# ECP-WarpX/WarpX

Measured on AMD Instinct MI355X. Metric: particle_steps_per_s, higher is better.
Workload: dtype f64; 1 GPU; 3D uniform_plasma 256x256x256, 8 ppc, Yee FDTD, order-3 shape, esirkepov, boris, filter on; cells_per_gpu=16777216, particles_per_gpu=134217728, n_ranks=1, ranks_per_gpu=1, sort_interval=2, single_precision_comms=False, preroll_steps=40, overlap_halo=False, momentum_synchronisation=outside the timed region (the K steps are consecutive steps of one longer run)

## Files before the change

### include/warpx_amd.h

```cpp
#ifndef WARPX_AMD_H_
#define WARPX_AMD_H_

#include <stdint.h>

#ifdef __cplusplus
extern "C" {
#endif

typedef enum wxa_status {
    WXA_OK = 0,
    WXA_ERR_INVALID_ARG = -1,
    WXA_ERR_HIP = -2,
    WXA_ERR_UNSUPPORTED = -3,
    WXA_ERR_NOMEM = -4,
    WXA_ERR_COMM = -5
} wxa_status;

enum { WXA_PUSHER_BORIS = 0, WXA_PUSHER_VAY = 1, WXA_PUSHER_HC = 2,
       WXA_PUSHER_BORIS_RR = 3 };
enum { WXA_DEPOSIT_ESIRKEPOV = 0, WXA_DEPOSIT_DIRECT = 1 };
enum { WXA_DT_FULL = 0, WXA_DT_FIRST_HALF = 1, WXA_DT_SECOND_HALF = 2 };

typedef struct wxa_field_view {
    double* p;
    int32_t lo[3];
    int32_t n[3];
    int32_t ng[3];
    int32_t stag[3];
    int64_t jstride;
    int64_t kstride;
} wxa_field_view;

typedef struct wxa_particle_view {
    double* x; double* y; double* z; double* w;
    double* ux; double* uy; double* uz;
    uint64_t* idcpu;
    int64_t np;
} wxa_particle_view;

typedef struct wxa_grid_geom {
    double xyzmin[3];
    double dinv[3];
    int32_t lo[3];
} wxa_grid_geom;

typedef struct wxa_workspace wxa_workspace;

wxa_status wxa_workspace_create(wxa_workspace** ws);
void       wxa_workspace_destroy(wxa_workspace* ws);
wxa_status wxa_workspace_set_external_particle_fields(wxa_workspace* ws, const double E[3], const double B[3]);
typedef struct wxa_repeated_plasma_lens {
    int32_t n_lenses;
    double  period;
    const double* starts;
    const double* lengths;
    const double* strengths_E;
    const double* strengths_B;
    double  gamma_boost;
    double  dt;
} wxa_repeated_plasma_lens;
wxa_status wxa_workspace_set_repeated_plasma_lens(wxa_workspace* ws, const wxa_repeated_plasma_lens* lens);
wxa_status wxa_workspace_set_time(wxa_workspace* ws, double t);
#define WXA_ACC_FP64 0
#define WXA_ACC_FP32 1
wxa_status wxa_workspace_set_deposit_accumulator(wxa_workspace* ws, int32_t accumulator);
wxa_status wxa_workspace_set_streaming_plasma(wxa_workspace* ws, int32_t on);

const char* wxa_version(void);
const char* wxa_last_error(void);


wxa_status wxa_evolve_b(const wxa_field_view E[3], const wxa_field_view B[3],
                        double dt, const double dinv[3], void* stream);

wxa_status wxa_evolve_e(const wxa_field_view E[3], const wxa_field_view B[3],
                        const wxa_field_view J[3],
                        double dt, const double dinv[3], void* stream);

wxa_status wxa_evolve_b_guard_layer(const wxa_field_view E[3], const wxa_field_view B[3], double dt,
                                    const double inv_dx[3], const int32_t grow[3], void* stream);

void wxa_ckc_stencil_coefficients(const double cell_size[3], double coefs_x[5], double coefs_y[5], double coefs_z[5]);
double wxa_ckc_max_dt(const double cell_size[3]);
wxa_status wxa_evolve_b_ckc(const wxa_field_view E[3], const wxa_field_view B[3], double dt,
                            const double coefs_x[5], const double coefs_y[5], const double coefs_z[5], void* stream);


wxa_status wxa_gather_push(const wxa_particle_view* p,
                           const wxa_field_view E[3], const wxa_field_view B[3],
                           const wxa_grid_geom* geom,
                           double q, double m, double dt,
                           int order, int galerkin, int pusher, void* stream);

wxa_status wxa_push_p(const wxa_particle_view* p,
                      const wxa_field_view E[3], const wxa_field_view B[3],
                      const wxa_grid_geom* geom,
                      double q, double m, double dt,
                      int order, int galerkin, int pusher, void* stream);

wxa_status wxa_gather_push_ws(const wxa_particle_view* p,
                              const wxa_field_view E[3], const wxa_field_view B[3],
                              const wxa_grid_geom* geom,
                              double q, double m, double dt,
                              int order, int galerkin, int pusher, int move,
                              wxa_workspace* ws, void* stream);

enum { WXA_PART_INTERIOR = 1, WXA_PART_REST = 2 };
wxa_status wxa_gather_push_part(const wxa_particle_view* p,
                                const wxa_field_view E[3], const wxa_field_view B[3],
                                const wxa_grid_geom* geom,
                                double q, double m, double dt,
                                int order, int galerkin, int pusher,
                                wxa_workspace* ws, int part, void* stream);

wxa_status wxa_deposit_current(const wxa_particle_view* p,
                               const wxa_field_view J[3],
                               const wxa_grid_geom* geom,
                               double q, double dt, double relative_time,
                               int order, int algo,
                               wxa_workspace* ws, void* stream);

wxa_status wxa_deposit_charge(const wxa_particle_view* p,
                              const wxa_field_view* rho,
                              const wxa_grid_geom* geom,
                              double q, int order, void* stream);

wxa_status wxa_enforce_periodic(const wxa_particle_view* p,
                                const double plo[3], const double phi[3],
                                const int periodic[3], void* stream);
wxa_status wxa_enforce_periodic_sorted(const wxa_particle_view* p, const double plo[3], const double phi[3],
                                       const int periodic[3], wxa_workspace* ws, int32_t steps_since_sort,
                                       void* stream);

wxa_status wxa_sort_particles_by_cell(const wxa_particle_view* src,
                                      const wxa_particle_view* dst,
                                      const double plo[3], const double dinv[3],
                                      const int32_t cell_lo[3], const int32_t ncell[3],
                                      wxa_workspace* ws, void* stream);

enum { WXA_PUSH_SORT_COUNT = 1, WXA_PUSH_SORT_SCATTER = 2 };
wxa_status wxa_push_sort_begin(wxa_workspace* ws, int32_t mode, const wxa_particle_view* p,
                               const wxa_particle_view* dst, const double plo[3], const double dinv[3],
                               const int32_t cell_lo[3], const int32_t ncell[3], const int32_t wrap[3],
                               int32_t check_retired, double predict_dt, void* stream);
wxa_status wxa_push_sort_end(wxa_workspace* ws, int32_t read_live, int64_t* live, int64_t* appended,
                             void* stream);
int32_t wxa_push_sort_pending(const wxa_workspace* ws, const wxa_particle_view* p);

wxa_status wxa_partition_particles(const wxa_particle_view* src, const wxa_particle_view* dst,
                                   int dim, double lo, double hi, int64_t counts[3],
                                   wxa_workspace* ws, void* stream);

#define WXA_IDCPU_RETIRED 0xFFFFFFFFFFFFFFFFull

wxa_status wxa_wrap_and_classify(const wxa_particle_view* p, int64_t first, int64_t count,
                                 const double prob_lo[3], const double prob_hi[3],
                                 const int periodic[3], const double brick_lo[3],
                                 const double brick_hi[3], const int split[3], int32_t* lists,
                                 int64_t capacity, int64_t counts[6], wxa_workspace* ws,
                                 void* stream);

wxa_status wxa_wrap_and_classify_dest(const wxa_particle_view* p, int64_t first, int64_t count,
                                      const double prob_lo[3], const double prob_hi[3],
                                      const int periodic[3], const double brick_lo[3],
                                      const double brick_hi[3], const int split[3], int32_t* lists,
                                      int64_t capacity, int64_t counts[27], wxa_workspace* ws,
                                      void* stream);

wxa_status wxa_pack_leavers(const wxa_particle_view* p, const int32_t* list, int64_t n, void* msg,
                            int64_t row_len, int64_t offset, int retire, const double brick_lo[3],
                            const double brick_hi[3], void* stream);

wxa_status wxa_sort_live_count(wxa_workspace* ws, int64_t* n, void* stream);


#define WXA_BOUNDARY_PERIODIC 0
#define WXA_BOUNDARY_PEC      1

wxa_status wxa_apply_pec_e(const wxa_field_view E[3], const int32_t dom_lo[3],
                           const int32_t dom_hi[3], const int32_t pec_lo[3],
                           const int32_t pec_hi[3], const int32_t ng[3], void* stream);
wxa_status wxa_apply_pec_b(const wxa_field_view B[3], const int32_t dom_lo[3],
                           const int32_t dom_hi[3], const int32_t pec_lo[3],
                           const int32_t pec_hi[3], const int32_t ng[3], void* stream);

#define WXA_PBOUNDARY_DEFAULT    0
#define WXA_PBOUNDARY_ABSORBING  1
#define WXA_PBOUNDARY_REFLECTING 2
#define WXA_PBOUNDARY_PERIODIC   3

wxa_status wxa_apply_particle_boundaries(const wxa_particle_view* p, const double prob_lo[3],
                                         const double prob_hi[3], const int32_t bc_lo[3],
                                         const int32_t bc_hi[3], int64_t* n_lost,
                                         wxa_workspace* ws, void* stream);

wxa_status wxa_apply_pec_j(const wxa_field_view J[3], const int32_t dom_lo[3],
                           const int32_t dom_hi[3], const int32_t pec_lo[3],
                           const int32_t pec_hi[3], void* stream);

wxa_status wxa_apply_pec_rho(const wxa_field_view* rho, const int32_t dom_lo[3],
                             const int32_t dom_hi[3], const int32_t pec_lo[3],
                             const int32_t pec_hi[3], void* stream);


wxa_status wxa_filter_bilinear(const wxa_field_view* src, const wxa_field_view* dst,
                               void* stream);

wxa_status wxa_filter_stencil(const wxa_field_view* src, const wxa_field_view* dst, const double* s0, int32_t n0,
                              const double* s1, int32_t n1, const double* s2, int32_t n2, void* stream);

#define WXA_NCI_EX_EY_BZ 0
#define WXA_NCI_BX_BY_EZ 1
wxa_status wxa_nci_godfrey_stencil(double cdtodz, int32_t nodal_gather, int32_t coeff_set, double stencil_z[5]);

wxa_status wxa_fill_boundary_periodic(const wxa_field_view* f, const int ng[3],
                                      const int periodic[3], void* stream);

wxa_status wxa_fill_boundary_periodic_multi(const wxa_field_view* f, int32_t nf, const int ng[3],
                                            const int periodic[3], void* stream);

wxa_status wxa_sync_nodal_periodic(const wxa_field_view* f, const int periodic[3], void* stream);

wxa_status wxa_sum_boundary_periodic(const wxa_field_view* f, const int src_ng[3],
                                     const int periodic[3], void* stream);

wxa_status wxa_sum_boundary_periodic_multi(const wxa_field_view* f, int32_t nf, const int src_ng[3],
                                           const int periodic[3], void* stream);

wxa_status wxa_pack_box(const wxa_field_view* f, const int32_t blo[3], const int32_t bhi[3],
                        double* buf, void* stream);
wxa_status wxa_unpack_box(const wxa_field_view* f, const int32_t blo[3], const int32_t bhi[3],
                          const double* buf, int mode, void* stream);
wxa_status wxa_pack_box_f32(const wxa_field_view* f, const int32_t blo[3], const int32_t bhi[3],
                            float* buf, void* stream);
wxa_status wxa_unpack_box_f32(const wxa_field_view* f, const int32_t blo[3], const int32_t bhi[3],
                              const float* buf, int mode, void* stream);

wxa_status wxa_field_set_zero(const wxa_field_view* f, void* stream);
wxa_status wxa_field_set_zero_multi(const wxa_field_view* f, int32_t nf, void* stream);

wxa_status wxa_copy_to_host(void* dst_host, const void* src_dev, int64_t bytes);
wxa_status wxa_copy_to_device(void* dst_dev, const void* src_host, int64_t bytes);
wxa_status wxa_device_synchronize(void);


enum { WXA_GRID_STAGGERED = 0, WXA_GRID_COLLOCATED = 1 };
enum { WXA_SOLVER_YEE = 0, WXA_SOLVER_CKC = 1 };

typedef struct wxa_sim_config {
    int32_t n_cell[3];
    double  prob_lo[3];
    double  prob_hi[3];
    double  cfl;
    int32_t nox;
    int32_t galerkin;
    int32_t particle_pusher;
    int32_t current_deposition;
    int32_t use_filter;
    int32_t sort_interval;
    int32_t nbricks[3];
    int32_t coord[3];
    int32_t field_boundary_lo[3];
    int32_t field_boundary_hi[3];
    int32_t particle_boundary_lo[3];
    int32_t particle_boundary_hi[3];
    int32_t overlap_halo;
    int32_t grid_type;
    int32_t maxwell_solver;
    double  gamma_boost;
    int32_t use_fdtd_nci_corr;
} wxa_sim_config;


typedef struct wxa_moving_window {
    int32_t dir;
    double  v;
} wxa_moving_window;

typedef struct wxa_plasma_injector {
    double  density;
    int32_t ppc[3];
    double  lo[3], hi[3];
    double  gamma_boost;
    double  t;
} wxa_plasma_injector;

typedef struct wxa_injected_momentum {
    double   u_mean[3];
    double   u_th[3];
    uint64_t seed;
    double   origin[3];
} wxa_injected_momentum;
wxa_status wxa_add_plasma(const wxa_particle_view* dst, const wxa_plasma_injector* inj,
                          const double corner[3], const int32_t ncells[3], const double dx[3],
                          const double brick_lo[3], const double brick_hi[3],
                          const wxa_injected_momentum* momentum,
                          int64_t* n_added, wxa_workspace* ws, void* stream);

typedef struct wxa_laser_antenna {
    double position[3], direction[3], polarization[3];
    double e_max, wavelength;
    double waist, duration, t_peak, focal_distance;
} wxa_laser_antenna;

#define WXA_WINDOW_KEEP_GUARDS 2
wxa_status wxa_shift_field_window(const wxa_field_view* f, double* tmp, int32_t dir, int32_t num_shift,
                                  const int periodic[3], void* stream);

typedef struct wxa_laser_push_params {
    double position[3], p_X[3], p_Y[3];
    double mobility;
    double e_max, wavelength, waist, duration, t_peak, focal_distance;
    double nvec[3];
    double gamma_boost;
} wxa_laser_push_params;
wxa_status wxa_laser_push(const wxa_particle_view* p, const wxa_laser_push_params* par, double t,
                          double dt, void* stream);

typedef struct wxa_comm {
    void* ctx;
    int32_t rank, nranks;
    int (*exchange)(void* ctx, int nmsg,
                    const int32_t* send_peer, void* const* send_buf, const int64_t* send_bytes,
                    const int32_t* recv_peer, void* const* recv_buf, const int64_t* recv_bytes,
                    void* stream);
    int (*exchange_counts)(void* ctx, int nmsg,
                           const int32_t* send_peer, const int64_t* send_val,
                           const int32_t* recv_peer, int64_t* recv_val);
} wxa_comm;

#define WXA_RCCL_ID_BYTES 128
#define WXA_RCCL_LOOPBACK 1
#define WXA_RCCL_TIMING   2
typedef struct wxa_rccl_stats {
    int64_t n_exchanges, n_messages, bytes_sent, n_count_exchanges, timed_exchanges;
    double timed_ms;
} wxa_rccl_stats;
wxa_status wxa_rccl_unique_id(char id[WXA_RCCL_ID_BYTES]);
wxa_status wxa_rccl_comm_set_timing(wxa_comm* comm, int32_t on);
wxa_status wxa_rccl_comm_create(const char id[WXA_RCCL_ID_BYTES], int32_t rank, int32_t nranks, int32_t flags,
                                wxa_comm* out);
void       wxa_rccl_comm_destroy(wxa_comm* comm);
wxa_status wxa_rccl_comm_stats(wxa_comm* comm, wxa_rccl_stats* out, int32_t reset);

typedef struct wxa_sim wxa_sim;

wxa_status wxa_sim_create(const wxa_sim_config* cfg, const wxa_comm* comm, wxa_sim** out);
void       wxa_sim_destroy(wxa_sim* s);
wxa_status wxa_sim_add_species(wxa_sim* s, double charge, double mass,
                               const wxa_particle_view* init, int32_t* species_id);
wxa_status wxa_sim_evolve(wxa_sim* s, int32_t numsteps);
wxa_status wxa_sim_set_synchronize_at_end(wxa_sim* s, int32_t on);
wxa_status wxa_sim_synchronize(wxa_sim* s);
wxa_status wxa_sim_set_safe_guard_cells(wxa_sim* s, int32_t on);
wxa_status wxa_sim_set_single_precision_comms(wxa_sim* s, int32_t on);
wxa_status wxa_sim_set_external_particle_fields(wxa_sim* s, int32_t id, const double E[3], const double B[3]);
wxa_status wxa_sim_set_deposit_accumulator(wxa_sim* s, int32_t id, int32_t accumulator);
wxa_status wxa_sim_set_radiation_reaction(wxa_sim* s, int32_t id, int32_t on);
wxa_status wxa_sim_create_from_inputs(const char* inputs_path, int32_t n_overrides,
                                      const char* const* overrides, const wxa_comm* comm,
                                      const int32_t* nbricks, const int32_t* coord, wxa_sim** out);
int32_t     wxa_sim_max_step(const wxa_sim* s);
int32_t     wxa_sim_num_species(const wxa_sim* s);
const char* wxa_sim_species_name(const wxa_sim* s, int32_t id);
int64_t     wxa_sim_checksum_json(wxa_sim* s, char* buf, int64_t capacity);
wxa_status  wxa_sim_write_plotfile(wxa_sim* s, const char* dir);
wxa_status  wxa_sim_add_full_diag(wxa_sim* s, const char* name, const char* intervals, const char* file_prefix,
                                  int32_t file_min_digits, const char* fields, int32_t write_species,
                                  int32_t dump_last_timestep);
wxa_status  wxa_sim_flush_diags_last_timestep(wxa_sim* s);
wxa_status  wxa_sim_btd_write_plotfile(wxa_sim* s, int32_t i, const char* dir);
wxa_status  wxa_sim_btd_set_flush(wxa_sim* s, const char* file_prefix, int32_t file_min_digits);
wxa_status  wxa_sim_btd_flush(wxa_sim* s);
wxa_status  wxa_sim_btd_box(wxa_sim* s, int32_t i, int32_t lo[3], int32_t hi[3]);
wxa_status  wxa_parser_eval(const char* expr, int32_t nvars, const char* const* names,
                            const double* values, double* out);

int32_t wxa_sim_halo_overlap(const wxa_sim* s);

wxa_status wxa_sim_compute_rho(wxa_sim* s);
double     wxa_sim_dt(const wxa_sim* s);
int64_t    wxa_sim_istep(const wxa_sim* s);
wxa_status wxa_sim_get_field(wxa_sim* s, const char* name, wxa_field_view* out);
wxa_status wxa_sim_get_particles(wxa_sim* s, int32_t species_id, wxa_particle_view* out);
wxa_status wxa_btd_select_particles(const wxa_particle_view* p, const double* const old6[6], double z_boost,
                                    double z_boost_old, double t_boost, double dt, double t_lab, double gamma_boost,
                                    double* out, int64_t capacity, int64_t* n_selected, void* stream);
wxa_status wxa_sim_add_btd(wxa_sim* s, int32_t num_snapshots, double dt_snapshots_lab, int32_t buffer_size,
                           int32_t write_species);
wxa_status wxa_sim_btd_num_particles(wxa_sim* s, int32_t i, int32_t id, int64_t* n);
wxa_status wxa_sim_btd_particles(wxa_sim* s, int32_t i, int32_t id, double* out);
wxa_status wxa_sim_btd_info(wxa_sim* s, int32_t i, int32_t n[3], double z_lab[2], double* t_lab, int32_t* slices,
                            int32_t* full);
wxa_status wxa_sim_btd_data(wxa_sim* s, int32_t i, int32_t comp, double* out);

wxa_status wxa_sim_get_timers(wxa_sim* s, double ms[8], int64_t counts[8], int reset);
wxa_status wxa_sim_dry_comm(wxa_sim* s, int32_t reps, double ms[4]);
wxa_status wxa_sim_enable_timers(wxa_sim* s, int enable);

wxa_status wxa_reduce_field(const wxa_field_view* f, const int32_t lo[3], const int32_t hi[3], double* sum_sq,
                            double* max_abs, void* stream);
wxa_status wxa_reduce_particles(const wxa_particle_view* p, double mass, int32_t photon, double out[6], void* stream);
wxa_status wxa_sim_add_reduced_diag(wxa_sim* s, const char* name, const char* type, const char* intervals,
                                    const char* path);
wxa_status wxa_sim_reduced_diag_data(wxa_sim* s, const char* name, int32_t compute_now, double* out, int32_t capacity,
                                     int32_t* n);

#ifdef __cplusplus
}
#endif
#endif
```

### warpx_amd/_capi.py

```python
from __future__ import annotations

import ctypes as C
import os

_HERE = os.path.dirname(os.path.abspath(__file__))
PRODUCT_LIB = os.path.join(_HERE, "libwarpx_amd.so")


class FieldView(C.Structure):
    _fields_ = [
        ("p", C.c_void_p),
        ("lo", C.c_int32 * 3),
        ("n", C.c_int32 * 3),
        ("ng", C.c_int32 * 3),
        ("stag", C.c_int32 * 3),
        ("jstride", C.c_int64),
        ("kstride", C.c_int64),
    ]


class ParticleView(C.Structure):
    _fields_ = [
        ("x", C.c_void_p), ("y", C.c_void_p), ("z", C.c_void_p), ("w", C.c_void_p),
        ("ux", C.c_void_p), ("uy", C.c_void_p), ("uz", C.c_void_p),
# ... 14 lines not shown
SOLVER_YEE, SOLVER_CKC = 0, 1
PART_INTERIOR, PART_REST = 1, 2


class SimConfig(C.Structure):
    _fields_ = [
        ("n_cell", C.c_int32 * 3),
        ("prob_lo", C.c_double * 3),
        ("prob_hi", C.c_double * 3),
        ("cfl", C.c_double),
        ("nox", C.c_int32),
        ("galerkin", C.c_int32),
        ("particle_pusher", C.c_int32),
        ("current_deposition", C.c_int32),
        ("use_filter", C.c_int32),
        ("sort_interval", C.c_int32),
        ("nbricks", C.c_int32 * 3),
        ("coord", C.c_int32 * 3),
        ("field_boundary_lo", C.c_int32 * 3),
        ("field_boundary_hi", C.c_int32 * 3),
        ("particle_boundary_lo", C.c_int32 * 3),
        ("particle_boundary_hi", C.c_int32 * 3),
        ("overlap_halo", C.c_int32),
        ("grid_type", C.c_int32),
        ("maxwell_solver", C.c_int32),
        ("gamma_boost", C.c_double),
        ("use_fdtd_nci_corr", C.c_int32),
    ]


class MovingWindow(C.Structure):
    _fields_ = [("dir", C.c_int32), ("v", C.c_double)]


class PlasmaInjector(C.Structure):
    _fields_ = [("density", C.c_double), ("ppc", C.c_int32 * 3), ("lo", C.c_double * 3), ("hi", C.c_double * 3),
                ("gamma_boost", C.c_double), ("t", C.c_double)]


class RepeatedPlasmaLens(C.Structure):
    _fields_ = [("n_lenses", C.c_int32), ("period", C.c_double), ("starts", C.POINTER(C.c_double)),
                ("lengths", C.POINTER(C.c_double)), ("strengths_E", C.POINTER(C.c_double)),
                ("strengths_B", C.POINTER(C.c_double)), ("gamma_boost", C.c_double), ("dt", C.c_double)]

    @classmethod
    def make(cls, period, starts, lengths, strengths_E, strengths_B, gamma_boost, dt):
        n = len(starts)
        arrays = [(C.c_double * n)(*map(float, a)) for a in (starts, lengths, strengths_E, strengths_B)]
        lens = cls(n, float(period), *[C.cast(a, C.POINTER(C.c_double)) for a in arrays], float(gamma_boost), float(dt))
        lens._keep = arrays
        return lens


class InjectedMomentum(C.Structure):
    _fields_ = [("u_mean", C.c_double * 3), ("u_th", C.c_double * 3), ("seed", C.c_uint64), ("origin", C.c_double * 3)]


class LaserAntenna(C.Structure):
    _fields_ = [("position", C.c_double * 3), ("direction", C.c_double * 3), ("polarization", C.c_double * 3),
                ("e_max", C.c_double), ("wavelength", C.c_double), ("waist", C.c_double), ("duration", C.c_double),
                ("t_peak", C.c_double), ("focal_distance", C.c_double)]


class LaserPushParams(C.Structure):
    _fields_ = [("position", C.c_double * 3), ("p_X", C.c_double * 3), ("p_Y", C.c_double * 3),
                ("mobility", C.c_double), ("e_max", C.c_double), ("wavelength", C.c_double), ("waist", C.c_double),
                ("duration", C.c_double), ("t_peak", C.c_double), ("focal_distance", C.c_double),
                ("nvec", C.c_double * 3), ("gamma_boost", C.c_double)]


EXCHANGE_FN = C.CFUNCTYPE(
    C.c_int, C.c_void_p, C.c_int,
    C.POINTER(C.c_int32), C.POINTER(C.c_void_p), C.POINTER(C.c_int64),
    C.POINTER(C.c_int32), C.POINTER(C.c_void_p), C.POINTER(C.c_int64),
    C.c_void_p)
EXCHANGE_COUNTS_FN = C.CFUNCTYPE(
    C.c_int, C.c_void_p, C.c_int,
    C.POINTER(C.c_int32), C.POINTER(C.c_int64),
    C.POINTER(C.c_int32), C.POINTER(C.c_int64))


class Comm(C.Structure):
    _fields_ = [
        ("ctx", C.c_void_p),
        ("rank", C.c_int32),
        ("nranks", C.c_int32),
        ("exchange", EXCHANGE_FN),
        ("exchange_counts", EXCHANGE_COUNTS_FN),
    ]


class RcclStats(C.Structure):
    _fields_ = [("n_exchanges", C.c_int64), ("n_messages", C.c_int64), ("bytes_sent", C.c_int64),
                ("n_count_exchanges", C.c_int64), ("timed_exchanges", C.c_int64), ("timed_ms", C.c_double)]


RCCL_LOOPBACK, RCCL_TIMING = 1, 2
PUSHER_BORIS, PUSHER_VAY, PUSHER_HC, PUSHER_BORIS_RR = 0, 1, 2, 3
DEPOSIT_ESIRKEPOV, DEPOSIT_DIRECT = 0, 1
BOUNDARY_PERIODIC, BOUNDARY_PEC = 0, 1
PBOUNDARY_DEFAULT, PBOUNDARY_ABSORBING, PBOUNDARY_REFLECTING, PBOUNDARY_PERIODIC = 0, 1, 2, 3

_FV3 = FieldView * 3
_D3 = C.c_double * 3
_I3 = C.c_int * 3
_I32_3 = C.c_int32 * 3
_PFV = C.POINTER(FieldView)
_PPV = C.POINTER(ParticleView)
_PGG = C.POINTER(GridGeom)

_KERNEL_SIGS = {
    "evolve_b": (C.c_int, [_FV3, _FV3, C.c_double, _D3, C.c_void_p]),
    "evolve_e": (C.c_int, [_FV3, _FV3, _FV3, C.c_double, _D3, C.c_void_p]),
    "gather_push": (C.c_int, [_PPV, _FV3, _FV3, _PGG, C.c_double, C.c_double, C.c_double,
                              C.c_int, C.c_int, C.c_int, C.c_void_p]),
    "push_p": (C.c_int, [_PPV, _FV3, _FV3, _PGG, C.c_double, C.c_double, C.c_double,
                         C.c_int, C.c_int, C.c_int, C.c_void_p]),
    "deposit_current": (C.c_int, [_PPV, _FV3, _PGG, C.c_double, C.c_double, C.c_double,
                                  C.c_int, C.c_int, C.c_void_p, C.c_void_p]),
    "deposit_charge": (C.c_int, [_PPV, _PFV, _PGG, C.c_double, C.c_int, C.c_void_p]),
    "btd_select_particles": (C.c_int, [_PPV, C.POINTER(C.c_void_p), C.c_double, C.c_double, C.c_double, C.c_double,
                                       C.c_double, C.c_double, C.c_void_p, C.c_int64, C.POINTER(C.c_int64), C.c_void_p]),
    "reduce_field": (C.c_int, [_PFV, _I32_3, _I32_3, C.POINTER(C.c_double), C.POINTER(C.c_double), C.c_void_p]),
    "reduce_particles": (C.c_int, [_PPV, C.c_double, C.c_int32, C.c_double * 6, C.c_void_p]),
    "enforce_periodic": (C.c_int, [_PPV, _D3, _D3, _I3, C.c_void_p]),
    "apply_pec_e": (C.c_int, [_FV3, _I32_3, _I32_3, _I32_3, _I32_3, _I32_3, C.c_void_p]),
    "apply_pec_b": (C.c_int, [_FV3, _I32_3, _I32_3, _I32_3, _I32_3, _I32_3, C.c_void_p]),
    "apply_pec_j": (C.c_int, [_FV3, _I32_3, _I32_3, _I32_3, _I32_3, C.c_void_p]),
    "apply_particle_boundaries": (C.c_int, [_PPV, _D3, _D3, _I32_3, _I32_3, C.POINTER(C.c_int64), C.c_void_p,
                                            C.c_void_p]),
    "evolve_b_guard_layer": (C.c_int, [_FV3, _FV3, C.c_double, _D3, _I32_3, C.c_void_p]),
    "evolve_b_ckc": (C.c_int, [_FV3, _FV3, C.c_double, C.c_double * 5, C.c_double * 5, C.c_double * 5, C.c_void_p]),
    "ckc_stencil_coefficients": (None, [_D3, C.c_double * 5, C.c_double * 5, C.c_double * 5]),
    "ckc_max_dt": (C.c_double, [_D3]),
    "apply_pec_rho": (C.c_int, [_PFV, _I32_3, _I32_3, _I32_3, _I32_3, C.c_void_p]),
    "shift_field_window": (C.c_int, [_PFV, C.c_void_p, C.c_int32, C.c_int32, _I3, C.c_void_p]),
    "laser_push": (C.c_int, [_PPV, C.POINTER(LaserPushParams), C.c_double, C.c_double, C.c_void_p]),
    "filter_bilinear": (C.c_int, [_PFV, _PFV, C.c_void_p]),
    "filter_stencil": (C.c_int, [_PFV, _PFV, C.POINTER(C.c_double), C.c_int32, C.POINTER(C.c_double), C.c_int32,
                                 C.POINTER(C.c_double), C.c_int32, C.c_void_p]),
    "nci_godfrey_stencil": (C.c_int, [C.c_double, C.c_int32, C.c_int32, C.POINTER(C.c_double)]),
    "fill_boundary_periodic": (C.c_int, [_PFV, _I3, _I3, C.c_void_p]),
    "sum_boundary_periodic": (C.c_int, [_PFV, _I3, _I3, C.c_void_p]),
    "sync_nodal_periodic": (C.c_int, [_PFV, _I3, C.c_void_p]),
    "field_set_zero": (C.c_int, [_PFV, C.c_void_p]),
    "version": (C.c_char_p, []),
}

_INPUTS_SIGS = {
    "sim_dry_comm": (C.c_int, [C.c_void_p, C.c_int32, C.c_double * 4]),
    "sim_create_from_inputs": (C.c_int, [C.c_char_p, C.c_int32, C.POINTER(C.c_char_p), C.POINTER(Comm),
                                        C.POINTER(C.c_int32), C.POINTER(C.c_int32), C.POINTER(C.c_void_p)]),
    "sim_max_step": (C.c_int32, [C.c_void_p]),
    "sim_num_species": (C.c_int32, [C.c_void_p]),
    "sim_species_name": (C.c_char_p, [C.c_void_p, C.c_int32]),
    "sim_checksum_json": (C.c_int64, [C.c_void_p, C.c_char_p, C.c_int64]),
    "sim_write_plotfile": (C.c_int, [C.c_void_p, C.c_char_p]),
    "sim_add_full_diag": (C.c_int, [C.c_void_p, C.c_char_p, C.c_char_p, C.c_char_p, C.c_int32, C.c_char_p, C.c_int32,
                                   C.c_int32]),
    "sim_flush_diags_last_timestep": (C.c_int, [C.c_void_p]),
    "sim_btd_write_plotfile": (C.c_int, [C.c_void_p, C.c_int32, C.c_char_p]),
    "sim_btd_set_flush": (C.c_int, [C.c_void_p, C.c_char_p, C.c_int32]),
    "sim_btd_flush": (C.c_int, [C.c_void_p]),
    "sim_btd_box": (C.c_int, [C.c_void_p, C.c_int32, C.POINTER(C.c_int32), C.POINTER(C.c_int32)]),
    "sim_set_synchronize_at_end": (C.c_int, [C.c_void_p, C.c_int32]),
    "sim_synchronize": (C.c_int, [C.c_void_p]),
    "sim_set_safe_guard_cells": (C.c_int, [C.c_void_p, C.c_int32]),
    "sim_set_single_precision_comms": (C.c_int, [C.c_void_p, C.c_int32]),
    "parser_eval": (C.c_int, [C.c_char_p, C.c_int32, C.POINTER(C.c_char_p), C.POINTER(C.c_double),
                              C.POINTER(C.c_double)]),
    "last_error": (C.c_char_p, []),
}

_SIM_SIGS = {
    "sim_create": (C.c_int, [C.POINTER(SimConfig), C.c_void_p, C.POINTER(C.c_void_p)]),
    "sim_destroy": (None, [C.c_void_p]),
    "sim_add_species": (C.c_int, [C.c_void_p, C.c_double, C.c_double, _PPV, C.POINTER(C.c_int32)]),
    "sim_evolve": (C.c_int, [C.c_void_p, C.c_int32]),
    "sim_dt": (C.c_double, [C.c_void_p]),
    "sim_istep": (C.c_int64, [C.c_void_p]),
    "sim_get_field": (C.c_int, [C.c_void_p, C.c_char_p, _PFV]),
    "sim_get_particles": (C.c_int, [C.c_void_p, C.c_int32, _PPV]),
    "sim_get_timers": (C.c_int, [C.c_void_p, C.c_double * 8, C.c_int64 * 8, C.c_int]),
    "sim_enable_timers": (C.c_int, [C.c_void_p, C.c_int]),
    "sim_compute_rho": (C.c_int, [C.c_void_p]),
    "sim_halo_overlap": (C.c_int32, [C.c_void_p]),
    "sim_set_moving_window": (C.c_int, [C.c_void_p, C.POINTER(MovingWindow)]),
    "sim_set_injection": (C.c_int, [C.c_void_p, C.c_int32, C.POINTER(PlasmaInjector), C.c_int, C.c_int]),
    "sim_set_external_particle_fields": (C.c_int, [C.c_void_p, C.c_int32, _D3, _D3]),
    "sim_set_radiation_reaction": (C.c_int, [C.c_void_p, C.c_int32, C.c_int32]),
    "sim_add_laser": (C.c_int, [C.c_void_p, C.POINTER(LaserAntenna)]),
    "sim_add_btd": (C.c_int, [C.c_void_p, C.c_int32, C.c_double, C.c_int32, C.c_int32]),
    "sim_btd_num_particles": (C.c_int, [C.c_void_p, C.c_int32, C.c_int32, C.POINTER(C.c_int64)]),
    "sim_btd_particles": (C.c_int, [C.c_void_p, C.c_int32, C.c_int32, C.POINTER(C.c_double)]),
    "sim_btd_info": (C.c_int, [C.c_void_p, C.c_int32, C.POINTER(C.c_int32), C.POINTER(C.c_double), C.POINTER(C.c_double),
                              C.POINTER(C.c_int32), C.POINTER(C.c_int32)]),
    "sim_btd_data": (C.c_int, [C.c_void_p, C.c_int32, C.c_int32, C.POINTER(C.c_double)]),
    "sim_add_reduced_diag": (C.c_int, [C.c_void_p, C.c_char_p, C.c_char_p, C.c_char_p, C.c_char_p]),
    "sim_reduced_diag_data": (C.c_int, [C.c_void_p, C.c_char_p, C.c_int32, C.POINTER(C.c_double), C.c_int32,
                                       C.POINTER(C.c_int32)]),
}

_PRODUCT_SIGS = {
    "fill_boundary_periodic_multi": (C.c_int, [_PFV, C.c_int32, _I3, _I3, C.c_void_p]),
    "sum_boundary_periodic_multi": (C.c_int, [_PFV, C.c_int32, _I3, _I3, C.c_void_p]),
    "workspace_set_external_particle_fields": (C.c_int, [C.c_void_p, _D3, _D3]),
    "workspace_set_repeated_plasma_lens": (C.c_int, [C.c_void_p, C.POINTER(RepeatedPlasmaLens)]),
    "workspace_set_time": (C.c_int, [C.c_void_p, C.c_double]),
    "workspace_create": (C.c_int, [C.POINTER(C.c_void_p)]),
    "workspace_destroy": (None, [C.c_void_p]),
    "last_error": (C.c_char_p, []),
    "sort_particles_by_cell": (C.c_int, [_PPV, _PPV, _D3, _D3, _I32_3, _I32_3, C.c_void_p, C.c_void_p]),
    "gather_push_ws": (C.c_int, [_PPV, _FV3, _FV3, _PGG, C.c_double, C.c_double, C.c_double,
                                 C.c_int, C.c_int, C.c_int, C.c_int, C.c_void_p, C.c_void_p]),
    "add_plasma": (C.c_int, [_PPV, C.POINTER(PlasmaInjector), _D3, _I32_3, _D3, _D3, _D3,
                             C.POINTER(InjectedMomentum), C.POINTER(C.c_int64), C.c_void_p, C.c_void_p]),
    "gather_push_part": (C.c_int, [_PPV, _FV3, _FV3, _PGG, C.c_double, C.c_double, C.c_double, C.c_int, C.c_int,
                                   C.c_int, C.c_void_p, C.c_int, C.c_void_p]),
    "partition_particles": (C.c_int, [_PPV, _PPV, C.c_int, C.c_double, C.c_double,
                                      C.POINTER(C.c_int64), C.c_void_p, C.c_void_p]),
    "wrap_and_classify": (C.c_int, [_PPV, C.c_int64, C.c_int64, _D3, _D3, _I3, _D3, _D3, _I3, C.c_void_p,
                                    C.c_int64, C.POINTER(C.c_int64), C.c_void_p, C.c_void_p]),
    "wrap_and_classify_dest": (C.c_int, [_PPV, C.c_int64, C.c_int64, _D3, _D3, _I3, _D3, _D3, _I3, C.c_void_p,
                                         C.c_int64, C.POINTER(C.c_int64), C.c_void_p, C.c_void_p]),
    "pack_leavers": (C.c_int, [_PPV, C.c_void_p, C.c_int64, C.c_void_p, C.c_int64, C.c_int64, C.c_int, _D3, _D3,
                               C.c_void_p]),
    "sort_live_count": (C.c_int, [C.c_void_p, C.POINTER(C.c_int64), C.c_void_p]),
    "push_sort_begin": (C.c_int, [C.c_void_p, C.c_int32, _PPV, _PPV, _D3, _D3, _I32_3, _I32_3, _I32_3, C.c_int32, C.c_double, C.c_void_p]),
    "push_sort_end": (C.c_int, [C.c_void_p, C.c_int32, C.POINTER(C.c_int64), C.POINTER(C.c_int64), C.c_void_p]),
    "push_sort_pending": (C.c_int32, [C.c_void_p, _PPV]),
    "pack_box": (C.c_int, [_PFV, _I32_3, _I32_3, C.c_void_p, C.c_void_p]),
    "unpack_box": (C.c_int, [_PFV, _I32_3, _I32_3, C.c_void_p, C.c_int, C.c_void_p]),
    "pack_box_f32": (C.c_int, [_PFV, _I32_3, _I32_3, C.c_void_p, C.c_void_p]),
    "unpack_box_f32": (C.c_int, [_PFV, _I32_3, _I32_3, C.c_void_p, C.c_int, C.c_void_p]),
    "field_set_zero_multi": (C.c_int, [_PFV, C.c_int32, C.c_void_p]),
    "copy_to_host": (C.c_int, [C.c_void_p, C.c_void_p, C.c_int64]),
    "copy_to_device": (C.c_int, [C.c_void_p, C.c_void_p, C.c_int64]),
    "device_synchronize": (C.c_int, []),
    "enforce_periodic_sorted": (C.c_int, [_PPV, _D3, _D3, _I3, C.c_void_p, C.c_int32, C.c_void_p]),
    "workspace_set_deposit_accumulator": (C.c_int, [C.c_void_p, C.c_int32]),
    "workspace_set_streaming_plasma": (C.c_int, [C.c_void_p, C.c_int32]),
    "sim_set_deposit_accumulator": (C.c_int, [C.c_void_p, C.c_int32, C.c_int32]),
}
ACC_FP64, ACC_FP32 = 0, 1
PUSH_SORT_COUNT, PUSH_SORT_SCATTER = 1, 2

_TRANSPORT_SIGS = {
    "rccl_unique_id": (C.c_int, [C.c_char * 128]),
    "rccl_comm_create": (C.c_int, [C.c_char * 128, C.c_int32, C.c_int32, C.c_int32, C.POINTER(Comm)]),
    "rccl_comm_destroy": (None, [C.POINTER(Comm)]),
    "rccl_comm_stats": (C.c_int, [C.POINTER(Comm), C.POINTER(RcclStats), C.c_int32]),
    "rccl_comm_set_timing": (C.c_int, [C.POINTER(Comm), C.c_int32]),
}

_ORACLE_SIGS = {
    "sum_sq_unique": (C.c_double, [_PFV]),
    "field_energy": (None, [_FV3, _FV3, _D3, C.c_double * 3]),
    "particle_energy": (C.c_double, [_PPV, C.c_double]),
    "particle_momentum": (None, [_PPV, C.c_double, C.c_double * 3]),
    "cell_centered_abs_sum": (C.c_double, [_PFV]),
    "abs_sum": (C.c_double, [C.c_void_p, C.c_int64, C.c_double]),

    "pack_box_f32": (C.c_int, [_PFV, _I32_3, _I32_3, C.c_void_p, C.c_void_p]),
    "unpack_box_f32": (C.c_int, [_PFV, _I32_3, _I32_3, C.c_void_p, C.c_int, C.c_void_p]),
    "num_threads": (C.c_int, []),
    "set_num_threads": (C.c_int, [C.c_int]),
    "add_plasma": (C.c_int, [_PPV, C.POINTER(PlasmaInjector), _D3, _I32_3, _D3, _D3, _D3,
                             C.POINTER(InjectedMomentum), C.POINTER(C.c_int64), C.c_void_p, C.c_void_p]),
    "sort_particles_by_cell": (C.c_int, [_PPV, _PPV, _D3, _D3, _I32_3, _I32_3, C.c_void_p, C.c_void_p]),
    "wrap_and_classify": (C.c_int, [_PPV, C.c_int64, C.c_int64, _D3, _D3, _I3, _D3, _D3, _I3, C.c_void_p,
                                    C.c_int64, C.POINTER(C.c_int64), C.c_void_p, C.c_void_p]),
    "wrap_and_classify_dest": (C.c_int, [_PPV, C.c_int64, C.c_int64, _D3, _D3, _I3, _D3, _D3, _I3, C.c_void_p,
                                         C.c_int64, C.POINTER(C.c_int64), C.c_void_p, C.c_void_p]),
    "pack_leavers": (C.c_int, [_PPV, C.c_void_p, C.c_int64, C.c_void_p, C.c_int64, C.c_int64, C.c_int, _D3, _D3,
                               C.c_void_p]),
}


class WxaError(RuntimeError):
    pass


_RETURNS_A_VALUE = {"sim_max_step", "sim_num_species", "num_threads", "set_num_threads", "sim_halo_overlap", "push_sort_pending"}


class CLib:

    def __init__(self, path: str, prefix: str, extra_sigs: dict | None = None, kernels: bool = True,
                 memory: str | None = None):
        self.memory = memory or ("cuda" if prefix == "wxa_" else "cpu")
        if not os.path.exists(path):
            raise WxaError(
                f"{path} not found: build it first (python -c 'import __graft_entry__ as g; g.build()')")
        self.path = path
        self.prefix = prefix
        self._dll = C.CDLL(path, mode=C.RTLD_GLOBAL if prefix == "wxa_" else C.RTLD_LOCAL)
        sigs = dict(_KERNEL_SIGS) if kernels else {}
        sigs.update(_SIM_SIGS)
        if extra_sigs:
            sigs.update(extra_sigs)
        self.names = []
        for name, (res, args) in sigs.items():
            fn = getattr(self._dll, prefix + name)
            fn.restype = res
            fn.argtypes = args
            setattr(self, "_" + name, fn)
            self.names.append(prefix + name)

    def __getattr__(self, name):
        raw = object.__getattribute__(self, "_" + name)
        if raw.restype is C.c_int and name not in _RETURNS_A_VALUE:
            def checked(*a):
                rc = raw(*a)
                if rc != 0:
                    msg = ""
                    if hasattr(self, "_last_error"):
                        try:
                            msg = (self._last_error() or b"").decode()
                        except Exception:
                            pass
                    raise WxaError(f"{self.prefix}{name} failed with status {rc} {msg}")
                return rc
            return checked
        return raw


_product = None


def load_product() -> CLib:
    global _product
    if _product is None:
        _product = CLib(os.environ.get("WXA_PRODUCT_LIB", PRODUCT_LIB), "wxa_",
                       {**_PRODUCT_SIGS, **_INPUTS_SIGS, **_TRANSPORT_SIGS})
    return _product


def declared_symbols(header_path: str) -> list[str]:
    import re
    text = open(header_path).read()
    text = re.sub(r"/\*.*?\*/", "", text, flags=re.S)
    return sorted(set(re.findall(r"\b(wxa_[a-z0-9_]+)\s*\(", text)))
```

### warpx_amd/csrc/fields.hip

```cpp
#include "common.hpp"

#include <algorithm>
#include <climits>
#include <cstdlib>

namespace wxa {

template <int TW_, int TJ_, int KC_, int NT_, int BATCH_ = 0>
struct StencilCfg {
    static constexpr int TW = TW_, TI = 64 * TW_, TJ = TJ_, KC = KC_, NT = NT_, BATCH = BATCH_;
};

struct TileGrid {
    int nti, ntj, ntk;
    long ntiles;
};

template <class CFG>
static TileGrid make_tiles_cfg(const Box3& ub) {
    TileGrid t;
    t.nti = (ub.hi[0] - ub.lo[0] + CFG::TI - 1) / CFG::TI;
    t.ntj = (ub.hi[1] - ub.lo[1] + CFG::TJ - 1) / CFG::TJ;
    t.ntk = (ub.hi[2] - ub.lo[2] + CFG::KC - 1) / CFG::KC;
    t.ntiles = (long)t.nti * t.ntj * t.ntk;
    return t;
}

__device__ inline bool in_ij(const Box3& b, int i, int j) {
    return i >= b.lo[0] && i < b.hi[0] && j >= b.lo[1] && j < b.hi[1];
}

template <int NT>
__device__ __forceinline__ double ld_shared(const double* p) {
    if constexpr (NT >= 2) return __builtin_nontemporal_load(p);
    else return *p;
}
template <int NT>
__device__ __forceinline__ double ld_once(const double* p) {
    if constexpr (NT) return __builtin_nontemporal_load(p);
    else return *p;
}
template <int NT>
__device__ __forceinline__ void st_once(double* p, double v) {
    if constexpr (NT) __builtin_nontemporal_store(v, p);
    else *p = v;
}

template <class CFG>
__global__ void __launch_bounds__(CFG::TI* CFG::TJ)
evolve_b_kernel(DevF Ex, DevF Ey, DevF Ez, DevF Bx, DevF By, DevF Bz, Box3 ub, Box3 bbx, Box3 bby,
                Box3 bbz, TileGrid tg, double dt, double idx, double idy, double idz) {
    constexpr int KC = CFG::KC, NT = CFG::NT;
    const long tile = xcd_tile_id(blockIdx.x, tg.ntiles);
    if (tile >= tg.ntiles) return;
    const int ti = (int)(tile % tg.nti);
    const int tj = (int)((tile / tg.nti) % tg.ntj);
    const int tk = (int)(tile / ((long)tg.nti * tg.ntj));
    const int i = ub.lo[0] + ti * CFG::TI + (int)threadIdx.x;
    const int j = ub.lo[1] + tj * CFG::TJ + (int)threadIdx.y;
    if (i >= ub.hi[0] || j >= ub.hi[1]) return;
    const int k0 = ub.lo[2] + tk * KC;
    const int k1 = min(k0 + KC, ub.hi[2]);
    const bool px = in_ij(bbx, i, j), py = in_ij(bby, i, j), pz = in_ij(bbz, i, j);

    const double* __restrict__ ex = Ex.p + Ex.off(i, j, k0);
    const double* __restrict__ ey = Ey.p + Ey.off(i, j, k0);
    const double* __restrict__ ez = Ez.p + Ez.off(i, j, k0);
    double* __restrict__ bx = Bx.p + Bx.off(i, j, k0);
    double* __restrict__ by = By.p + By.off(i, j, k0);
    double* __restrict__ bz = Bz.p + Bz.off(i, j, k0);

    if constexpr (CFG::BATCH != 0) {
        double exv[KC + 1], eyv[KC + 1], ezc[KC], ezj[KC], ezi[KC], exj[KC], eyi[KC], b0[KC], b1[KC], b2[KC];
        bool d0[KC], d1[KC], d2[KC];
        exv[0] = ld_shared<NT>(ex); eyv[0] = ld_shared<NT>(ey);
#pragma unroll
        for (int n = 0; n < KC; ++n) {
            const int k = k0 + n;
            const bool in = k < k1;
            d0[n] = in && px && k >= bbx.lo[2] && k < bbx.hi[2];
            d1[n] = in && py && k >= bby.lo[2] && k < bby.hi[2];
            d2[n] = in && pz && k >= bbz.lo[2] && k < bbz.hi[2];
            exv[n + 1] = eyv[n + 1] = ezc[n] = ezj[n] = ezi[n] = exj[n] = eyi[n] = b0[n] = b1[n] = b2[n] = 0.0;
            if (in) {
                exv[n + 1] = ld_shared<NT>(ex + (n + 1) * Ex.ks); eyv[n + 1] = ld_shared<NT>(ey + (n + 1) * Ey.ks);
                ezc[n] = ld_shared<NT>(ez + n * Ez.ks); ezj[n] = ld_shared<NT>(ez + n * Ez.ks + Ez.js);
                ezi[n] = ld_shared<NT>(ez + n * Ez.ks + 1);
                exj[n] = ld_shared<NT>(ex + n * Ex.ks + Ex.js); eyi[n] = ld_shared<NT>(ey + n * Ey.ks + 1);
            }
            if (d0[n]) b0[n] = ld_once<NT>(bx + n * Bx.ks);
            if (d1[n]) b1[n] = ld_once<NT>(by + n * By.ks);
            if (d2[n]) b2[n] = ld_once<NT>(bz + n * Bz.ks);
        }
        asm volatile("" : "+v"(exv[0]), "+v"(eyv[0]));
#pragma unroll
        for (int n = 0; n < KC; ++n)
            asm volatile("" : "+v"(exv[n + 1]), "+v"(eyv[n + 1]), "+v"(ezc[n]), "+v"(ezj[n]), "+v"(ezi[n]), "+v"(exj[n]),
                              "+v"(eyi[n]), "+v"(b0[n]), "+v"(b1[n]), "+v"(b2[n]));
#pragma unroll
        for (int n = 0; n < KC; ++n) {
            if (d0[n]) st_once<NT>(bx + n * Bx.ks, b0[n] + (dt * (idz * (eyv[n + 1] - eyv[n])) - dt * (idy * (ezj[n] - ezc[n]))));
            if (d1[n]) st_once<NT>(by + n * By.ks, b1[n] + (dt * (idx * (ezi[n] - ezc[n])) - dt * (idz * (exv[n + 1] - exv[n]))));
            if (d2[n]) st_once<NT>(bz + n * Bz.ks, b2[n] + (dt * (idy * (exj[n] - exv[n])) - dt * (idx * (eyi[n] - eyv[n]))));
        }
        return;
    }
    double ex_k = ld_shared<NT>(ex), ey_k = ld_shared<NT>(ey);
#pragma unroll 4
    for (int k = k0; k < k1; ++k) {
        const double ex_k1 = ld_shared<NT>(ex + Ex.ks), ey_k1 = ld_shared<NT>(ey + Ey.ks);
        const double ez_c = ld_shared<NT>(ez), ez_j1 = ld_shared<NT>(ez + Ez.js), ez_i1 = ld_shared<NT>(ez + 1);
        const double ex_j1 = ld_shared<NT>(ex + Ex.js), ey_i1 = ld_shared<NT>(ey + 1);
        if (px && k >= bbx.lo[2] && k < bbx.hi[2])
            st_once<NT>(bx, ld_once<NT>(bx) + (dt * (idz * (ey_k1 - ey_k)) - dt * (idy * (ez_j1 - ez_c))));
        if (py && k >= bby.lo[2] && k < bby.hi[2])
            st_once<NT>(by, ld_once<NT>(by) + (dt * (idx * (ez_i1 - ez_c)) - dt * (idz * (ex_k1 - ex_k))));
        if (pz && k >= bbz.lo[2] && k < bbz.hi[2])
            st_once<NT>(bz, ld_once<NT>(bz) + (dt * (idy * (ex_j1 - ex_k)) - dt * (idx * (ey_i1 - ey_k))));
        ex_k = ex_k1; ey_k = ey_k1;
        ex += Ex.ks; ey += Ey.ks; ez += Ez.ks; bx += Bx.ks; by += By.ks; bz += Bz.ks;
    }
}

template <class CFG>
__global__ void __launch_bounds__(CFG::TI* CFG::TJ)
evolve_e_kernel(DevF Ex, DevF Ey, DevF Ez, DevF Bx, DevF By, DevF Bz, DevF Jx, DevF Jy, DevF Jz,
                Box3 ub, Box3 bex, Box3 bey, Box3 bez, TileGrid tg, double dt, double idx, double idy,
                double idz) {
    constexpr int KC = CFG::KC, NT = CFG::NT;
    const long tile = xcd_tile_id(blockIdx.x, tg.ntiles);
    if (tile >= tg.ntiles) return;
    const int ti = (int)(tile % tg.nti);
    const int tj = (int)((tile / tg.nti) % tg.ntj);
    const int tk = (int)(tile / ((long)tg.nti * tg.ntj));
    const int i = ub.lo[0] + ti * CFG::TI + (int)threadIdx.x;
    const int j = ub.lo[1] + tj * CFG::TJ + (int)threadIdx.y;
    if (i >= ub.hi[0] || j >= ub.hi[1]) return;
    const int k0 = ub.lo[2] + tk * KC;
    const int k1 = min(k0 + KC, ub.hi[2]);
    const bool px = in_ij(bex, i, j), py = in_ij(bey, i, j), pz = in_ij(bez, i, j);
    constexpr double c2 = PhysConst::c * PhysConst::c;
    constexpr double mu0 = PhysConst::mu0;

    double* __restrict__ ex = Ex.p + Ex.off(i, j, k0);
    double* __restrict__ ey = Ey.p + Ey.off(i, j, k0);
    double* __restrict__ ez = Ez.p + Ez.off(i, j, k0);
    const double* __restrict__ bx = Bx.p + Bx.off(i, j, k0);
    const double* __restrict__ by = By.p + By.off(i, j, k0);
    const double* __restrict__ bz = Bz.p + Bz.off(i, j, k0);
    const double* __restrict__ jx = Jx.p + Jx.off(i, j, k0);
    const double* __restrict__ jy = Jy.p + Jy.off(i, j, k0);
    const double* __restrict__ jz = Jz.p + Jz.off(i, j, k0);

    if constexpr (CFG::BATCH != 0) {
        double bxv[KC + 1], byv[KC + 1], bzc[KC], bzj[KC], bzi[KC], bxj[KC], byi[KC], e0[KC], e1[KC], e2[KC], j0[KC], j1[KC], j2[KC];
        bool d0[KC], d1[KC], d2[KC];
        bxv[0] = ld_shared<NT>(bx - Bx.ks); byv[0] = ld_shared<NT>(by - By.ks);
#pragma unroll
        for (int n = 0; n < KC; ++n) {
            const int k = k0 + n;
            const bool in = k < k1;
            d0[n] = in && px && k >= bex.lo[2] && k < bex.hi[2];
            d1[n] = in && py && k >= bey.lo[2] && k < bey.hi[2];
            d2[n] = in && pz && k >= bez.lo[2] && k < bez.hi[2];
            bxv[n + 1] = byv[n + 1] = bzc[n] = bzj[n] = bzi[n] = bxj[n] = byi[n] = 0.0;
            e0[n] = e1[n] = e2[n] = j0[n] = j1[n] = j2[n] = 0.0;
            if (in) {
                bxv[n + 1] = ld_shared<NT>(bx + n * Bx.ks); byv[n + 1] = ld_shared<NT>(by + n * By.ks);
                bzc[n] = ld_shared<NT>(bz + n * Bz.ks);
                bzj[n] = ld_shared<NT>(bz + n * Bz.ks - Bz.js); bzi[n] = ld_shared<NT>(bz + n * Bz.ks - 1);
                bxj[n] = ld_shared<NT>(bx + n * Bx.ks - Bx.js); byi[n] = ld_shared<NT>(by + n * By.ks - 1);
            }
            if (d0[n]) { e0[n] = ld_once<NT>(ex + n * Ex.ks); j0[n] = ld_once<NT>(jx + n * Jx.ks); }
            if (d1[n]) { e1[n] = ld_once<NT>(ey + n * Ey.ks); j1[n] = ld_once<NT>(jy + n * Jy.ks); }
            if (d2[n]) { e2[n] = ld_once<NT>(ez + n * Ez.ks); j2[n] = ld_once<NT>(jz + n * Jz.ks); }
        }
        asm volatile("" : "+v"(bxv[0]), "+v"(byv[0]));
#pragma unroll
        for (int n = 0; n < KC; ++n)
            asm volatile("" : "+v"(bxv[n + 1]), "+v"(byv[n + 1]), "+v"(bzc[n]), "+v"(bzj[n]), "+v"(bzi[n]), "+v"(bxj[n]),
                              "+v"(byi[n]), "+v"(e0[n]), "+v"(e1[n]), "+v"(e2[n]), "+v"(j0[n]), "+v"(j1[n]), "+v"(j2[n]));
#pragma unroll
        for (int n = 0; n < KC; ++n) {
            if (d0[n]) st_once<NT>(ex + n * Ex.ks, e0[n] + c2 * dt * (-(idz * (byv[n + 1] - byv[n])) + (idy * (bzc[n] - bzj[n])) - mu0 * j0[n]));
            if (d1[n]) st_once<NT>(ey + n * Ey.ks, e1[n] + c2 * dt * (-(idx * (bzc[n] - bzi[n])) + (idz * (bxv[n + 1] - bxv[n])) - mu0 * j1[n]));
            if (d2[n]) st_once<NT>(ez + n * Ez.ks, e2[n] + c2 * dt * (-(idy * (bxv[n + 1] - bxj[n])) + (idx * (byv[n + 1] - byi[n])) - mu0 * j2[n]));
        }
        return;
    }
    double bx_km = ld_shared<NT>(bx - Bx.ks), by_km = ld_shared<NT>(by - By.ks);
#pragma unroll 4
    for (int k = k0; k < k1; ++k) {
        const double bx_c = ld_shared<NT>(bx), by_c = ld_shared<NT>(by), bz_c = ld_shared<NT>(bz);
        const double bz_jm = ld_shared<NT>(bz - Bz.js), bz_im = ld_shared<NT>(bz - 1);
        const double bx_jm = ld_shared<NT>(bx - Bx.js), by_im = ld_shared<NT>(by - 1);
        if (px && k >= bex.lo[2] && k < bex.hi[2])
            st_once<NT>(ex, ld_once<NT>(ex) + c2 * dt * (-(idz * (by_c - by_km)) + (idy * (bz_c - bz_jm)) - mu0 * ld_once<NT>(jx)));
        if (py && k >= bey.lo[2] && k < bey.hi[2])
            st_once<NT>(ey, ld_once<NT>(ey) + c2 * dt * (-(idx * (bz_c - bz_im)) + (idz * (bx_c - bx_km)) - mu0 * ld_once<NT>(jy)));
        if (pz && k >= bez.lo[2] && k < bez.hi[2])
            st_once<NT>(ez, ld_once<NT>(ez) + c2 * dt * (-(idy * (bx_c - bx_jm)) + (idx * (by_c - by_im)) - mu0 * ld_once<NT>(jz)));
        bx_km = bx_c; by_km = by_c;
        ex += Ex.ks; ey += Ey.ks; ez += Ez.ks; bx += Bx.ks; by += By.ks; bz += Bz.ks;
        jx += Jx.ks; jy += Jy.ks; jz += Jz.ks;
    }
}

using StProduction = StencilCfg<1, 1, 3, 1, 1>;

struct FaceBoxes {
    int n;
    Box3 b[12];
    int comp[12];
    long first[13];
};
__global__ void __launch_bounds__(256)
evolve_b_faces_kernel(DevF Ex, DevF Ey, DevF Ez, DevF Bx, DevF By, DevF Bz, FaceBoxes fb, double dt, double idx, double idy,
                      double idz) {
    long t = (long)blockIdx.x * 256 + threadIdx.x;
    if (t >= fb.first[fb.n]) return;
    int f = 0;
    while (t >= fb.first[f + 1]) ++f;
    t -= fb.first[f];
    const Box3 b = fb.b[f];
    const int n0 = b.hi[0] - b.lo[0], n1 = b.hi[1] - b.lo[1];
    const int i = b.lo[0] + (int)(t % n0), j = b.lo[1] + (int)((t / n0) % n1), k = b.lo[2] + (int)(t / ((long)n0 * n1));
    const int c = fb.comp[f];
    if (c == 0) {
        const double* ey = Ey.p + Ey.off(i, j, k);
        const double* ez = Ez.p + Ez.off(i, j, k);
        double* bx = Bx.p + Bx.off(i, j, k);
        *bx = *bx + (dt * (idz * (ey[Ey.ks] - ey[0])) - dt * (idy * (ez[Ez.js] - ez[0])));
    } else if (c == 1) {
        const double* ex = Ex.p + Ex.off(i, j, k);
        const double* ez = Ez.p + Ez.off(i, j, k);
        double* by = By.p + By.off(i, j, k);
        *by = *by + (dt * (idx * (ez[1] - ez[0])) - dt * (idz * (ex[Ex.ks] - ex[0])));
    } else {
        const double* ex = Ex.p + Ex.off(i, j, k);
        const double* ey = Ey.p + Ey.off(i, j, k);
        double* bz = Bz.p + Bz.off(i, j, k);
        *bz = *bz + (dt * (idy * (ex[Ex.js] - ex[0])) - dt * (idx * (ey[1] - ey[0])));
    }
}

struct BoxN {
    int lo[3];
    int n[3];
};

__global__ void __launch_bounds__(256)
shift_copy_kernel(DevF f, BoxN box, int s0, int s1, int s2) {
    const long total = (long)box.n[0] * box.n[1] * box.n[2];
    for (long t = (long)blockIdx.x * blockDim.x + threadIdx.x; t < total; t += (long)gridDim.x * blockDim.x) {
        const int a = (int)(t % box.n[0]);
        const int b = (int)((t / box.n[0]) % box.n[1]);
        const int c = (int)(t / ((long)box.n[0] * box.n[1]));
        const int i = box.lo[0] + a, j = box.lo[1] + b, k = box.lo[2] + c;
        f.p[f.off(i, j, k)] = f.p[f.off(i + s0, j + s1, k + s2)];
    }
}

struct PecGeom {
    int dom_lo[3], dom_hi[3];
    int pec_lo[3], pec_hi[3];
    int nodal[3];
};

template <bool IS_E>
__global__ void __launch_bounds__(256)
apply_pec_kernel(DevF f, int icomp, BoxN box, PecGeom pg) {
    const long total = (long)box.n[0] * box.n[1] * box.n[2];
    for (long t = (long)blockIdx.x * blockDim.x + threadIdx.x; t < total; t += (long)gridDim.x * blockDim.x) {
        int ijk[3];
        ijk[0] = box.lo[0] + (int)(t % box.n[0]);
        ijk[1] = box.lo[1] + (int)((t / box.n[0]) % box.n[1]);
        ijk[2] = box.lo[2] + (int)(t / ((long)box.n[0] * box.n[1]));
        int mirror[3] = {ijk[0], ijk[1], ijk[2]};
        bool on_face = false, guard = false;
        double sign = 1.0;
#pragma unroll
        for (int idim = 0; idim < 3; ++idim) {
#pragma unroll
            for (int iside = 0; iside < 2; ++iside) {
                if (!(iside == 0 ? pg.pec_lo[idim] : pg.pec_hi[idim])) continue;
                const bool flagged = IS_E ? (icomp != idim) : (icomp == idim);
                const int ig = iside == 0 ? pg.dom_lo[idim] - ijk[idim]
                                          : ijk[idim] - (pg.dom_hi[idim] + pg.nodal[idim]);
                if (ig == 0) {
                    if (flagged && pg.nodal[idim] == 1) on_face = true;
                } else if (ig > 0) {
                    mirror[idim] = iside == 0 ? pg.dom_lo[idim] + ig - (1 - pg.nodal[idim]) : pg.dom_hi[idim] + 1 - ig;
                    guard = true;
                    if (flagged) sign = -sign;
                }
            }
        }
        if (on_face) f(ijk[0], ijk[1], ijk[2]) = 0.0;
        else if (guard) f(ijk[0], ijk[1], ijk[2]) = sign * f(mirror[0], mirror[1], mirror[2]);
    }
}

__global__ void __launch_bounds__(256)
apply_pec_j_kernel(DevF f, int icomp, Box3 vb, PecGeom pg) {
    const int n0 = vb.hi[0] - vb.lo[0], n1 = vb.hi[1] - vb.lo[1], n2 = vb.hi[2] - vb.lo[2];
    const long total = (long)n0 * n1 * n2;
    for (long t = (long)blockIdx.x * blockDim.x + threadIdx.x; t < total; t += (long)gridDim.x * blockDim.x) {
        int ijk[3];
        ijk[0] = vb.lo[0] + (int)(t % n0);
        ijk[1] = vb.lo[1] + (int)((t / n0) % n1);
        ijk[2] = vb.lo[2] + (int)(t / ((long)n0 * n1));
        const int flo[3] = {f.lo0, f.lo1, f.lo2}, fn[3] = {f.n0, f.n1, f.n2};
        int mir[3][2];
        bool any = false;
#pragma unroll
        for (int d = 0; d < 3; ++d) {
#pragma unroll
            for (int s = 0; s < 2; ++s) {
                mir[d][s] = INT_MIN;
                if (!(s == 0 ? pg.pec_lo[d] : pg.pec_hi[d])) continue;
                const int fac = (s == 0 ? 2 * pg.dom_lo[d] : 2 * (pg.dom_hi[d] + 1)) - (1 - pg.nodal[d]);
                const int m = fac - ijk[d];
                if (m == ijk[d] || (m >= flo[d] && m < flo[d] + fn[d])) { mir[d][s] = m; any = true; }
            }
        }
        if (!any) continue;
        double v = f(ijk[0], ijk[1], ijk[2]);
#pragma unroll
        for (int d = 0; d < 3; ++d) {
#pragma unroll
            for (int s = 0; s < 2; ++s) {
                const int m = mir[d][s];
                if (m == INT_MIN) continue;
                if (m == ijk[d]) { v = 0.0; continue; }
                int q[3] = {ijk[0], ijk[1], ijk[2]};
                q[d] = m;
                v += (icomp != d ? -1.0 : 1.0) * f(q[0], q[1], q[2]);
            }
        }
        f(ijk[0], ijk[1], ijk[2]) = v;
#pragma unroll
        for (int d = 0; d < 3; ++d) {
#pragma unroll
            for (int s = 0; s < 2; ++s) {
                const int m = mir[d][s];
                if (m == INT_MIN || m == ijk[d]) continue;
                int q[3] = {ijk[0], ijk[1], ijk[2]};
                q[d] = m;
                f(q[0], q[1], q[2]) = icomp != d ? -v : v;
            }
        }
    }
}

__global__ void __launch_bounds__(256)
set_box_kernel(DevF f, BoxN box, double value) {
    const long total = (long)box.n[0] * box.n[1] * box.n[2];
    for (long t = (long)blockIdx.x * blockDim.x + threadIdx.x; t < total; t += (long)gridDim.x * blockDim.x) {
        const int i = box.lo[0] + (int)(t % box.n[0]);
        const int j = box.lo[1] + (int)((t / box.n[0]) % box.n[1]);
        const int k = box.lo[2] + (int)(t / ((long)box.n[0] * box.n[1]));
        f.p[f.off(i, j, k)] = value;
    }
}

__global__ void __launch_bounds__(256)
shifted_copy_kernel(DevF dst, DevF src, BoxN box, int s0, int s1, int s2) {
    const long total = (long)box.n[0] * box.n[1] * box.n[2];
    for (long t = (long)blockIdx.x * blockDim.x + threadIdx.x; t < total; t += (long)gridDim.x * blockDim.x) {
        const int i = box.lo[0] + (int)(t % box.n[0]);
        const int j = box.lo[1] + (int)((t / box.n[0]) % box.n[1]);
        const int k = box.lo[2] + (int)(t / ((long)box.n[0] * box.n[1]));
        dst.p[dst.off(i, j, k)] = src.p[src.off(i + s0, j + s1, k + s2)];
    }
}

__global__ void __launch_bounds__(256)
shift_copy_sides_kernel(DevF f, BoxN box_lo, BoxN box_hi, int s0, int s1, int s2) {
    const long half = (long)box_lo.n[0] * box_lo.n[1] * box_lo.n[2];
    for (long t = (long)blockIdx.x * blockDim.x + threadIdx.x; t < 2 * half; t += (long)gridDim.x * blockDim.x) {
        const bool hi = t >= half;
        const long u = hi ? t - half : t;
        const BoxN& box = hi ? box_hi : box_lo;
        const int sg = hi ? -1 : 1;
        const int a = (int)(u % box.n[0]);
        const int b = (int)((u / box.n[0]) % box.n[1]);
        const int c = (int)(u / ((long)box.n[0] * box.n[1]));
        const int i = box.lo[0] + a, j = box.lo[1] + b, k = box.lo[2] + c;
        f.p[f.off(i, j, k)] = f.p[f.off(i + sg * s0, j + sg * s1, k + sg * s2)];
    }
}

__global__ void __launch_bounds__(256)
sum_periodic_kernel(DevF f, int d, int nc, int s0, int s1) {
    const int lo[3] = {f.lo0, f.lo1, f.lo2};
// ... 269 lines not shown
using CkcProduction = CkcCfg<4, 16, 2>;
using FilterCfg = CkcCfg<8, 16, 1>;

struct FilterStencils {
    static constexpr int MAXLEN = 8;
    double s[3][MAXLEN];
    int n[3];
};
__global__ void __launch_bounds__(256)
filter_stencil_kernel(DevF src, DevF dst, FilterStencils fs) {
    const long total = (long)src.n0 * src.n1 * src.n2;
    for (long t = (long)blockIdx.x * blockDim.x + threadIdx.x; t < total; t += (long)gridDim.x * blockDim.x) {
        const int i = src.lo0 + (int)(t % src.n0);
        const int j = src.lo1 + (int)((t / src.n0) % src.n1);
        const int k = src.lo2 + (int)(t / ((long)src.n0 * src.n1));
        auto zp = [&](int ii, int jj, int kk) -> double {
            return (ii >= src.lo0 && ii < src.lo0 + src.n0 && jj >= src.lo1 && jj < src.lo1 + src.n1 && kk >= src.lo2 &&
                    kk < src.lo2 + src.n2) ? src.p[src.off(ii, jj, kk)] : 0.0;
        };
        double d = 0.0;
        for (int i2 = 0; i2 < fs.n[2]; ++i2)
            for (int i1 = 0; i1 < fs.n[1]; ++i1)
                for (int i0 = 0; i0 < fs.n[0]; ++i0) {
                    const double sss = fs.s[0][i0] * fs.s[1][i1] * fs.s[2][i2];
                    d += sss * (zp(i - i0, j - i1, k - i2) + zp(i + i0, j - i1, k - i2) + zp(i - i0, j + i1, k - i2) +
                                zp(i + i0, j + i1, k - i2) + zp(i - i0, j - i1, k + i2) + zp(i + i0, j - i1, k + i2) +
                                zp(i - i0, j + i1, k + i2) + zp(i + i0, j + i1, k + i2));
                }
        dst.p[dst.off(i, j, k)] = d;
    }
}

template <int N2, int KC>
__global__ void __launch_bounds__(256)
filter_stencil_z_kernel(DevF src, DevF dst, FilterStencils fs) {
    const long columns = (long)src.n0 * src.n1;
    const int nseg = (src.n2 + KC - 1) / KC;
    const long t = (long)blockIdx.x * blockDim.x + threadIdx.x;
    if (t >= columns * nseg) return;
    const int i = src.lo0 + (int)(t % src.n0);
    const int j = src.lo1 + (int)((t / src.n0) % src.n1);
    const int k0 = src.lo2 + (int)(t / columns) * KC, k1 = min(k0 + KC, src.lo2 + src.n2);
    auto zp = [&](int kk) -> double { return (kk >= src.lo2 && kk < src.lo2 + src.n2) ? src.p[src.off(i, j, kk)] : 0.0; };
    double w[2 * N2 - 1];
#pragma unroll
    for (int m = 0; m < 2 * N2 - 1; ++m) w[m] = zp(k0 - (N2 - 1) + m);
    double sss[N2];
#pragma unroll
    for (int i2 = 0; i2 < N2; ++i2) sss[i2] = fs.s[0][0] * fs.s[1][0] * fs.s[2][i2];
    for (int k = k0; k < k1; ++k) {
        const double next = zp(k + N2);
        double d = 0.0;
#pragma unroll
        for (int i2 = 0; i2 < N2; ++i2) {
            const double a = w[N2 - 1 - i2], b = w[N2 - 1 + i2];
            d += sss[i2] * (a + a + a + a + b + b + b + b);
        }
        dst.p[dst.off(i, j, k)] = d;
#pragma unroll
        for (int m = 0; m + 1 < 2 * N2 - 1; ++m) w[m] = w[m + 1];
        w[2 * N2 - 2] = next;
    }
}

template <class CFG>
__global__ void __launch_bounds__(CFG::NT)
filter_bilinear_kernel(DevF src, DevF dst, TileGrid tg) {
    constexpr int PLANE = CFG::PLANE;
    __shared__ double ring[4 * PLANE];
    const long tile = xcd_tile_id(blockIdx.x, tg.ntiles);
    if (tile >= tg.ntiles) return;
    const int ti = (int)(tile % tg.nti), tj = (int)((tile / tg.nti) % tg.ntj), tk = (int)(tile / ((long)tg.nti * tg.ntj));
    const int i0 = src.lo0 + ti * CFG::TI, j0 = src.lo1 + tj * CFG::TJ, k0 = src.lo2 + tk * CFG::KC;
    const int hi0 = src.lo0 + src.n0, hi1 = src.lo1 + src.n1, hi2 = src.lo2 + src.n2;
    const int k1 = min(k0 + CFG::KC, hi2);
    const int tid = (int)(threadIdx.y * CFG::TI + threadIdx.x);
    const int i = i0 + (int)threadIdx.x, j = j0 + (int)threadIdx.y;
    double r[CFG::PER];
    for (int k = k0 - 1; k <= k0 + 1; ++k) {
        ckc_fetch_plane<CFG>(r, src, i0, j0, k, tid);
        ckc_put_plane<CFG>(ring + (k & 3) * PLANE, r, tid);
    }
    const CkcRing<CFG> in{ring, i0, j0};
    const bool active = i < hi0 && j < hi1;
    for (int k = k0; k < k1; ++k) {
        __syncthreads();
        const bool more = k + 2 <= k1;
        if (more) ckc_fetch_plane<CFG>(r, src, i0, j0, k + 2, tid);
        if (active) {
            auto tap = [&](int di, int dj, int dk) -> double { return in(i + di, j + dj, k + dk); };
            double d = 0.0;
#pragma unroll
            for (int i2 = 0; i2 < 2; ++i2)
#pragma unroll
                for (int i1 = 0; i1 < 2; ++i1)
#pragma unroll
                    for (int i0_ = 0; i0_ < 2; ++i0_) {
                        const double sss = 0.25 * 0.25 * 0.25;
                        d += sss * (tap(-i0_, -i1, -i2) + tap(+i0_, -i1, -i2) + tap(-i0_, +i1, -i2) +
                                    tap(+i0_, +i1, -i2) + tap(-i0_, -i1, +i2) + tap(+i0_, -i1, +i2) +
                                    tap(-i0_, +i1, +i2) + tap(+i0_, +i1, +i2));
                    }
            dst.p[dst.off(i, j, k)] = d;
        }
        if (more) ckc_put_plane<CFG>(ring + ((k + 2) & 3) * PLANE, r, tid);
    }
}

static inline int grid_for(long total, int block = 256, int cap = 256 * 16) {
    long g = (total + block - 1) / block;
    if (g < 1) g = 1;
    if (g > cap) g = cap;
    return (int)g;
}

static bool box_inside(const wxa_field_view& v, const int32_t blo[3], const int32_t bhi[3]) {
    for (int d = 0; d < 3; ++d)
        if (blo[d] < v.lo[d] || bhi[d] > v.lo[d] + v.n[d] || bhi[d] < blo[d]) return false;
    return true;
}

}

using namespace wxa;

extern "C" {

wxa_status wxa_evolve_b(const wxa_field_view E[3], const wxa_field_view B[3], double dt,
                        const double dinv[3], void* stream) {
    WXA_REQUIRE(E && B && dinv, "null argument");
    for (int c = 0; c < 3; ++c) WXA_REQUIRE(view_ok(E[c]) && view_ok(B[c]), "bad field view");
    if (!yee_E(E) || !yee_B(B)) {
        set_last_error("wxa_evolve_b: only the Yee staggering is supported");
        return WXA_ERR_UNSUPPORTED;
    }
    for (int c = 0; c < 3; ++c)
        for (int d = 0; d < 3; ++d) WXA_REQUIRE(E[c].ng[d] >= 1, "EvolveB needs >= 1 guard point on E");
    const Box3 bx = valid_box(B[0]), by = valid_box(B[1]), bz = valid_box(B[2]);
    Box3 ub;
    for (int d = 0; d < 3; ++d) {
        ub.lo[d] = std::min(bx.lo[d], std::min(by.lo[d], bz.lo[d]));
        ub.hi[d] = std::max(bx.hi[d], std::max(by.hi[d], bz.hi[d]));
    }
    using CFG = StProduction;
    const TileGrid tg = make_tiles_cfg<CFG>(ub);
    if (tg.ntiles > 0)
        hipLaunchKernelGGL((evolve_b_kernel<CFG>), dim3((unsigned)xcd_grid_size(tg.ntiles)), dim3(CFG::TI, CFG::TJ), 0,
                           (hipStream_t)stream, make_devf(E[0]), make_devf(E[1]), make_devf(E[2]), make_devf(B[0]),
                           make_devf(B[1]), make_devf(B[2]), ub, bx, by, bz, tg, dt, dinv[0], dinv[1], dinv[2]);
    WXA_LAUNCH_CHECK();
    return WXA_OK;
}

wxa_status wxa_evolve_b_guard_layer(const wxa_field_view E[3], const wxa_field_view B[3], double dt,
                                    const double dinv[3], const int32_t grow[3], void* stream) {
    WXA_REQUIRE(E && B && dinv && grow, "null argument");
    for (int c = 0; c < 3; ++c) WXA_REQUIRE(view_ok(E[c]) && view_ok(B[c]), "bad field view");
    if (!yee_E(E) || !yee_B(B)) {
        set_last_error("wxa_evolve_b_guard_layer: only the Yee staggering is supported");
        return WXA_ERR_UNSUPPORTED;
    }
    for (int c = 0; c < 3; ++c)
        for (int d = 0; d < 3; ++d)
            WXA_REQUIRE(!grow[d] || (E[c].ng[d] >= 2 && B[c].ng[d] >= 1), "guard layer update needs 2 guard points on E, 1 on B");
    FaceBoxes fb;
    fb.n = 0;
    fb.first[0] = 0;
    for (int d = 0; d < 3; ++d) {
        if (!grow[d]) continue;
        for (int side = 0; side < 2; ++side)
            for (int c = 0; c < 3; ++c) {
                if (B[c].stag[d]) continue;
                Box3 b = valid_box(B[c]);
                const int layer = side == 0 ? b.lo[d] - 1 : b.hi[d];
                b.lo[d] = layer; b.hi[d] = layer + 1;
                const long pts = (long)(b.hi[0] - b.lo[0]) * (b.hi[1] - b.lo[1]) * (b.hi[2] - b.lo[2]);
                if (pts <= 0) continue;
                fb.b[fb.n] = b; fb.comp[fb.n] = c;
                fb.first[fb.n + 1] = fb.first[fb.n] + pts;
                ++fb.n;
            }
    }
    if (fb.n > 0 && fb.first[fb.n] > 0)
        hipLaunchKernelGGL(evolve_b_faces_kernel, dim3((unsigned)((fb.first[fb.n] + 255) / 256)), dim3(256), 0, (hipStream_t)stream,
                           make_devf(E[0]), make_devf(E[1]), make_devf(E[2]), make_devf(B[0]), make_devf(B[1]), make_devf(B[2]),
                           fb, dt, dinv[0], dinv[1], dinv[2]);
    WXA_LAUNCH_CHECK();
    return WXA_OK;
}

void wxa_ckc_stencil_coefficients(const double cell_size[3], double cx[5], double cy[5], double cz[5]) {
    const double inv_dx = 1. / cell_size[0], inv_dy = 1. / cell_size[1], inv_dz = 1. / cell_size[2];
    const double delta = std::max({inv_dx, inv_dy, inv_dz});
    const double rx = (inv_dx / delta) * (inv_dx / delta);
    const double ry = (inv_dy / delta) * (inv_dy / delta);
    const double rz = (inv_dz / delta) * (inv_dz / delta);
    const double beta = 0.125 * (1. - rx * ry * rz / (ry * rz + rz * rx + rx * ry));
    const double betaxy = ry * beta * inv_dx, betaxz = rz * beta * inv_dx;
    const double betayx = rx * beta * inv_dy, betayz = rz * beta * inv_dy;
    const double betazx = rx * beta * inv_dz, betazy = ry * beta * inv_dz;
    const double inv_r_fac = (1. / (ry * rz + rz * rx + rx * ry));
    const double gammax = ry * rz * (0.0625 - 0.125 * ry * rz * inv_r_fac);
    const double gammay = rx * rz * (0.0625 - 0.125 * rx * rz * inv_r_fac);
    const double gammaz = rx * ry * (0.0625 - 0.125 * rx * ry * inv_r_fac);
    const double alphax = (1. - 2. * ry * beta - 2. * rz * beta - 4. * gammax) * inv_dx;
    const double alphay = (1. - 2. * rx * beta - 2. * rz * beta - 4. * gammay) * inv_dy;
    const double alphaz = (1. - 2. * rx * beta - 2. * ry * beta - 4. * gammaz) * inv_dz;
    cx[0] = inv_dx; cx[1] = alphax; cx[2] = betaxy; cx[3] = betaxz; cx[4] = gammax * inv_dx;
    cy[0] = inv_dy; cy[1] = alphay; cy[2] = betayz; cy[3] = betayx; cy[4] = gammay * inv_dy;
    cz[0] = inv_dz; cz[1] = alphaz; cz[2] = betazx; cz[3] = betazy; cz[4] = gammaz * inv_dz;
}

double wxa_ckc_max_dt(const double cell_size[3]) {
    return std::min(cell_size[0], std::min(cell_size[1], cell_size[2])) / PhysConst::c;
}

wxa_status wxa_evolve_b_ckc(const wxa_field_view E[3], const wxa_field_view B[3], double dt, const double cx[5],
                            const double cy[5], const double cz[5], void* stream) {
    WXA_REQUIRE(E && B && cx && cy && cz, "null argument");
    for (int c = 0; c < 3; ++c) WXA_REQUIRE(view_ok(E[c]) && view_ok(B[c]), "bad field view");
    if (!yee_E(E) || !yee_B(B)) {
        set_last_error("wxa_evolve_b_ckc: only the Yee staggering is supported");
        return WXA_ERR_UNSUPPORTED;
    }
    for (int c = 0; c < 3; ++c)
        for (int d = 0; d < 3; ++d) WXA_REQUIRE(E[c].ng[d] >= 1, "the CKC update of B needs >= 1 guard point on E");
    const Box3 bx = valid_box(B[0]), by = valid_box(B[1]), bz = valid_box(B[2]);
    Box3 ub;
    for (int d = 0; d < 3; ++d) {
        ub.lo[d] = std::min(bx.lo[d], std::min(by.lo[d], bz.lo[d]));
        ub.hi[d] = std::max(bx.hi[d], std::max(by.hi[d], bz.hi[d]));
        if (ub.hi[d] <= ub.lo[d]) return WXA_OK;
    }
    CkcCoefs cc;
    for (int n = 0; n < 5; ++n) { cc.x[n] = cx[n]; cc.y[n] = cy[n]; cc.z[n] = cz[n]; }
    using CFG = CkcProduction;
    const TileGrid tg = make_tiles_cfg<StencilCfg<1, CFG::TJ, CFG::KC, 1>>(ub);
    hipLaunchKernelGGL(evolve_b_ckc_tiled_kernel<CFG>, dim3((unsigned)xcd_grid_size(tg.ntiles)), dim3(CFG::TI, CFG::TJ), 0,
                       (hipStream_t)stream, make_devf(E[0]), make_devf(E[1]), make_devf(E[2]), make_devf(B[0]), make_devf(B[1]),
                       make_devf(B[2]), ub, bx, by, bz, tg, dt, cc);
    WXA_LAUNCH_CHECK();
    return WXA_OK;
}

wxa_status wxa_evolve_e(const wxa_field_view E[3], const wxa_field_view B[3], const wxa_field_view J[3],
                        double dt, const double dinv[3], void* stream) {
    WXA_REQUIRE(E && B && J && dinv, "null argument");
    for (int c = 0; c < 3; ++c) WXA_REQUIRE(view_ok(E[c]) && view_ok(B[c]) && view_ok(J[c]), "bad field view");
    if (!yee_E(E) || !yee_B(B) || !yee_E(J)) {
        set_last_error("wxa_evolve_e: only the Yee staggering is supported");
        return WXA_ERR_UNSUPPORTED;
    }
    for (int c = 0; c < 3; ++c)
        for (int d = 0; d < 3; ++d) WXA_REQUIRE(B[c].ng[d] >= 1, "EvolveE needs >= 1 guard point on B");
    const Box3 bx = valid_box(E[0]), by = valid_box(E[1]), bz = valid_box(E[2]);
    for (int c = 0; c < 3; ++c) {
        const Box3 bj = valid_box(J[c]);
        const Box3 be = valid_box(E[c]);
        for (int d = 0; d < 3; ++d)
            WXA_REQUIRE(bj.lo[d] == be.lo[d] && bj.hi[d] == be.hi[d], "J and E valid boxes differ");
    }
    Box3 ub;
    for (int d = 0; d < 3; ++d) {
        ub.lo[d] = std::min(bx.lo[d], std::min(by.lo[d], bz.lo[d]));
        ub.hi[d] = std::max(bx.hi[d], std::max(by.hi[d], bz.hi[d]));
    }
    using CFG = StProduction;
    const TileGrid tg = make_tiles_cfg<CFG>(ub);
    if (tg.ntiles > 0)
        hipLaunchKernelGGL((evolve_e_kernel<CFG>), dim3((unsigned)xcd_grid_size(tg.ntiles)), dim3(CFG::TI, CFG::TJ), 0,
                           (hipStream_t)stream, make_devf(E[0]), make_devf(E[1]), make_devf(E[2]), make_devf(B[0]),
                           make_devf(B[1]), make_devf(B[2]), make_devf(J[0]), make_devf(J[1]), make_devf(J[2]), ub, bx, by, bz,
                           tg, dt, dinv[0], dinv[1], dinv[2]);
    WXA_LAUNCH_CHECK();
    return WXA_OK;
}

wxa_status wxa_filter_bilinear(const wxa_field_view* src, const wxa_field_view* dst, void* stream) {
    WXA_REQUIRE(src && dst && view_ok(*src) && view_ok(*dst), "bad field view");
    WXA_REQUIRE(src->p != dst->p, "src and dst must not alias");
    for (int d = 0; d < 3; ++d)
        WXA_REQUIRE(src->lo[d] == dst->lo[d] && src->n[d] == dst->n[d], "src/dst boxes differ");
    TileGrid tg;
    tg.nti = (src->n[0] + FilterCfg::TI - 1) / FilterCfg::TI;
    tg.ntj = (src->n[1] + FilterCfg::TJ - 1) / FilterCfg::TJ;
    tg.ntk = (src->n[2] + FilterCfg::KC - 1) / FilterCfg::KC;
    tg.ntiles = (long)tg.nti * tg.ntj * tg.ntk;
    hipLaunchKernelGGL(filter_bilinear_kernel<FilterCfg>, dim3((unsigned)xcd_grid_size(tg.ntiles)),
                       dim3(FilterCfg::TI, FilterCfg::TJ), 0, (hipStream_t)stream, make_devf(*src), make_devf(*dst), tg);
    WXA_LAUNCH_CHECK();
    return WXA_OK;
}

wxa_status wxa_filter_stencil(const wxa_field_view* src, const wxa_field_view* dst, const double* s0, int32_t n0,
                              const double* s1, int32_t n1, const double* s2, int32_t n2, void* stream) {
    WXA_REQUIRE(src && dst && view_ok(*src) && view_ok(*dst) && s0 && s1 && s2, "bad argument");
    WXA_REQUIRE(src->p != dst->p, "src and dst must not alias");
    WXA_REQUIRE(n0 >= 1 && n0 <= FilterStencils::MAXLEN && n1 >= 1 && n1 <= FilterStencils::MAXLEN && n2 >= 1 &&
                n2 <= FilterStencils::MAXLEN, "stencil length");
    for (int d = 0; d < 3; ++d)
        WXA_REQUIRE(src->lo[d] == dst->lo[d] && src->n[d] == dst->n[d], "src/dst boxes differ");
    FilterStencils fs;
    fs.n[0] = n0; fs.n[1] = n1; fs.n[2] = n2;
    for (int a = 0; a < FilterStencils::MAXLEN; ++a) {
        fs.s[0][a] = a < n0 ? s0[a] : 0.0; fs.s[1][a] = a < n1 ? s1[a] : 0.0; fs.s[2][a] = a < n2 ? s2[a] : 0.0;
    }
    const long total = (long)src->n[0] * src->n[1] * src->n[2];
    if (total == 0) return WXA_OK;
    if (n0 == 1 && n1 == 1 && n2 == 5) {
        constexpr int KC = 32;
        const long lanes = (long)src->n[0] * src->n[1] * ((src->n[2] + KC - 1) / KC);
        hipLaunchKernelGGL((filter_stencil_z_kernel<5, KC>), dim3((unsigned)((lanes + 255) / 256)), dim3(256), 0,
                           (hipStream_t)stream, make_devf(*src), make_devf(*dst), fs);
        WXA_LAUNCH_CHECK();
        return WXA_OK;
    }
    hipLaunchKernelGGL(filter_stencil_kernel, dim3(grid_for(total)), dim3(256), 0, (hipStream_t)stream, make_devf(*src),
                       make_devf(*dst), fs);
    WXA_LAUNCH_CHECK();
    return WXA_OK;
}

wxa_status wxa_fill_boundary_periodic(const wxa_field_view* f, const int ng[3], const int periodic[3],
                                      void* stream) {
    WXA_REQUIRE(f && view_ok(*f) && ng && periodic, "bad argument");
    const DevF df = make_devf(*f);
    int lo[3], hi[3];
    for (int d = 0; d < 3; ++d) {
        WXA_REQUIRE(ng[d] <= f->ng[d], "ng exceeds allocated guards");
        lo[d] = f->lo[d] + f->ng[d];
        hi[d] = f->lo[d] + f->n[d] - f->ng[d];
    }
    for (int d = 0; d < 3; ++d) {
        if (!periodic[d] || ng[d] <= 0) continue;
        const int nc = f->n[d] - 2 * f->ng[d] - f->stag[d];
        WXA_REQUIRE(ng[d] <= nc, "guard depth exceeds the period");
        const int v0 = f->lo[d] + f->ng[d], v1 = f->lo[d] + f->n[d] - f->ng[d];
        BoxN blo, bhi;
        for (int e = 0; e < 3; ++e) { blo.lo[e] = bhi.lo[e] = lo[e]; blo.n[e] = bhi.n[e] = hi[e] - lo[e]; }
// ... 353 lines not shown
```

### warpx_amd/csrc/host/WarpX.hpp

```cpp
#ifndef WXA_HOST_WARPX_HPP_
#define WXA_HOST_WARPX_HPP_

#include <chrono>
#include <functional>

#include "BTDiagnostics.hpp"
#include "NCIGodfreyFilter.hpp"
#include "ReducedDiags.hpp"
#include "WarpXParticleContainer.hpp"

namespace wxa::host {

struct guardCellManager {
    amrex::IntVect ng_alloc_EB, ng_alloc_J, ng_depos_J, ng_FieldSolver, ng_FieldGather, ng_UpdateAux;

    void Init(const amrex::Real dt, const std::array<amrex::Real, 3>& dx, const int nox, const bool use_filter,
              const amrex::IntVect& bilinear_filter_stencil_length, const bool do_fdtd_nci_corr = false,
              const int nci_corr_stencil = 0, const bool safe_guard_cells = false) {
        constexpr double c = 299'792'458.;
        for (int d = 0; d < 3; ++d) {
            const int ng_tmp = nox;
            ng_alloc_EB[d] = (ng_tmp % 2) ? ng_tmp + 1 : ng_tmp;
            if (d == 2 && do_fdtd_nci_corr) {
                const int ng = ng_tmp + nci_corr_stencil;
                ng_alloc_EB[d] = (ng % 2) ? ng + 1 : ng;
            }
            int ngJ = ng_tmp;
            ngJ += static_cast<int>(std::ceil(c * 0.5 * dt / dx[d]));
            ng_depos_J[d] = ngJ;
            ng_alloc_J[d] = ngJ + (use_filter ? bilinear_filter_stencil_length[d] - 1 : 0);
            ng_FieldSolver[d] = 1;
            ng_FieldGather[d] = (nox + 1) / 2;
            ng_UpdateAux[d] = 0;
        }
        {
            const amrex::IntVect no_nci(std::min(ng_FieldGather[0], nox % 2 ? nox + 1 : nox),
                                        std::min(ng_FieldGather[1], nox % 2 ? nox + 1 : nox),
                                        std::min(ng_FieldGather[2], nox % 2 ? nox + 1 : nox));
            ng_FieldGather = no_nci;
            if (do_fdtd_nci_corr) ng_FieldGather[2] += nci_corr_stencil;
        }
        ng_FieldGather = amrex::min(ng_FieldGather, ng_alloc_EB);
        for (int d = 0; d < 3; ++d) ng_FieldGather[d] = std::max(ng_FieldGather[d], ng_FieldSolver[d]);
        if (safe_guard_cells) {
            ng_FieldSolver = ng_alloc_EB;
            ng_FieldGather = ng_alloc_EB;
            ng_UpdateAux = ng_alloc_EB;
        }
    }
};

class FiniteDifferenceSolver {
public:
    FiniteDifferenceSolver(WarpXContext* ctx, int fdtd_algo, const std::array<amrex::Real, 3>& cell_size)
        : m_ctx(ctx), m_fdtd_algo(fdtd_algo) {
        for (int d = 0; d < 3; ++d) m_stencil_coefs[d] = 1.0 / cell_size[d];
        if (m_fdtd_algo == WXA_SOLVER_CKC) {
            if (!ctx->be->evolve_b_ckc) throw std::runtime_error("algo.maxwell_solver = ckc: not in this backend");
            ctx->be->ckc_stencil_coefficients(cell_size.data(), m_ckc_x.data(), m_ckc_y.data(), m_ckc_z.data());
        } else if (m_fdtd_algo != WXA_SOLVER_YEE) {
            throw std::runtime_error("algo.maxwell_solver: yee or ckc");
        }
    }
    void EvolveB(ablastr::fields::MultiFabRegister& fields, int lev, PatchType patch_type, amrex::Real dt) {
        using warpx::fields::FieldType;
        if (patch_type != PatchType::fine) throw std::runtime_error("single level: fine patch only");
        auto E = fields.get_alldirs(FieldType::Efield_fp, lev);
        auto B = fields.get_alldirs(FieldType::Bfield_fp, lev);
        const wxa_field_view Ev[3] = {E[0]->view(), E[1]->view(), E[2]->view()};
        const wxa_field_view Bv[3] = {B[0]->view(), B[1]->view(), B[2]->view()};
        if (m_fdtd_algo == WXA_SOLVER_CKC)
            check(m_ctx->be->evolve_b_ckc(Ev, Bv, dt, m_ckc_x.data(), m_ckc_y.data(), m_ckc_z.data(), m_ctx->stream),
                  "evolve_b_ckc");
        else
            check(m_ctx->be->evolve_b(Ev, Bv, dt, m_stencil_coefs.data(), m_ctx->stream), "evolve_b");
    }
    void EvolveE(ablastr::fields::MultiFabRegister& fields, int lev, PatchType patch_type,
                 const ablastr::fields::VectorField& Efield, amrex::Real dt) {
        using warpx::fields::FieldType;
        if (patch_type != PatchType::fine) throw std::runtime_error("single level: fine patch only");
        auto B = fields.get_alldirs(FieldType::Bfield_fp, lev);
        auto J = fields.get_alldirs(FieldType::current_fp, lev);
        const wxa_field_view Ev[3] = {Efield[0]->view(), Efield[1]->view(), Efield[2]->view()};
        const wxa_field_view Bv[3] = {B[0]->view(), B[1]->view(), B[2]->view()};
        const wxa_field_view Jv[3] = {J[0]->view(), J[1]->view(), J[2]->view()};
        check(m_ctx->be->evolve_e(Ev, Bv, Jv, dt, m_stencil_coefs.data(), m_ctx->stream), "evolve_e");
    }
    void EvolveBGuardLayer(ablastr::fields::MultiFabRegister& fields, int lev, amrex::Real dt, const int32_t grow[3]) {
        using warpx::fields::FieldType;
        auto E = fields.get_alldirs(FieldType::Efield_fp, lev);
        auto B = fields.get_alldirs(FieldType::Bfield_fp, lev);
        const wxa_field_view Ev[3] = {E[0]->view(), E[1]->view(), E[2]->view()};
        const wxa_field_view Bv[3] = {B[0]->view(), B[1]->view(), B[2]->view()};
        check(m_ctx->be->evolve_b_guard_layer(Ev, Bv, dt, m_stencil_coefs.data(), grow, m_ctx->stream), "evolve_b_guard_layer");
    }

private:
    WarpXContext* m_ctx;
    int m_fdtd_algo = WXA_SOLVER_YEE;
    std::array<amrex::Real, 3> m_stencil_coefs{};
    std::array<amrex::Real, 5> m_ckc_x{}, m_ckc_y{}, m_ckc_z{};
};

class WarpX {
public:
    static constexpr bool sync_nodal_points = true;

    WarpX(const Backend* be, const wxa_sim_config& cfg, const wxa_comm* comm)
        : m_be(be), m_cfg(cfg), m_fields(be), mypc(std::make_unique<MultiParticleContainer>(&m_ctx)) {
        using warpx::fields::FieldType;
        using ablastr::fields::Direction;
        if (cfg.nox < 1 || cfg.nox > 4) throw std::runtime_error("algo.particle_shape must be 1..4");
        m_env_no_guard_layer = std::getenv("WXA_NO_GUARD_LAYER") != nullptr;
        if (const char* e = std::getenv("WXA_PEC_RHO_FOLD_GUARD_COLUMNS")) m_env_fold_rho_guard_columns = std::atoi(e) != 0;
        m_ctx.be = be;
        m_ctx.nox = cfg.nox;
        m_ctx.galerkin_interpolation = cfg.galerkin != 0;
        m_ctx.particle_pusher_algo = (ParticlePusherAlgo)cfg.particle_pusher;
        m_ctx.current_deposition_algo = (CurrentDepositionAlgo)cfg.current_deposition;
        if (cfg.gamma_boost > 1.0) {
            m_ctx.gamma_boost = cfg.gamma_boost;
            m_ctx.beta_boost = std::sqrt(1.0 - 1.0 / std::pow(cfg.gamma_boost, 2.0));
        }
        amrex::IntVect blo, bhi;
        for (int d = 0; d < 3; ++d) {
            if (cfg.nbricks[d] < 1 || cfg.coord[d] < 0 || cfg.coord[d] >= cfg.nbricks[d])
                throw std::runtime_error("bad brick decomposition");
            if (cfg.n_cell[d] % cfg.nbricks[d] != 0) throw std::runtime_error("n_cell must divide evenly into bricks");
            m_ctx.prob_lo[d] = cfg.prob_lo[d];
            m_ctx.prob_hi[d] = cfg.prob_hi[d];
            m_ctx.dx[d] = (cfg.prob_hi[d] - cfg.prob_lo[d]) / cfg.n_cell[d];
            m_ctx.dinv[d] = 1.0 / m_ctx.dx[d];
            const int nb = cfg.n_cell[d] / cfg.nbricks[d];
            blo[d] = cfg.coord[d] * nb;
            bhi[d] = blo[d] + nb - 1;
            m_ctx.brick_plo[d] = cfg.prob_lo[d] + blo[d] * m_ctx.dx[d];
            m_ctx.brick_phi[d] = (cfg.coord[d] == cfg.nbricks[d] - 1) ? cfg.prob_hi[d]
                                                                       : cfg.prob_lo[d] + (bhi[d] + 1) * m_ctx.dx[d];
        }
        m_ctx.brick_box = amrex::Box(blo, bhi);
        if (cfg.grid_type != WXA_GRID_STAGGERED)
            throw std::runtime_error("warpx.grid_type: only the staggered (Yee) grid is on this path");
        ComputeDt();
        use_filter = cfg.use_filter != 0;
        guard_cells.Init(dt[0], m_ctx.dx, cfg.nox, use_filter, amrex::IntVect(2), cfg.use_fdtd_nci_corr != 0,
                         NCIGodfreyFilter::m_stencil_width);
        m_ctx.ng_alloc_EB = guard_cells.ng_alloc_EB;
        m_ctx.ng_depos_J = guard_cells.ng_depos_J;
        for (int d = 0; d < 3; ++d)
            if (m_ctx.brick_box.length(d) < guard_cells.ng_alloc_J[d] + 1)
                throw std::runtime_error("brick thinner than the guard depth");
        m_comm = std::make_unique<BrickComm>(be, comm, cfg.nbricks, cfg.coord);
        int periodic[3];
        for (int d = 0; d < 3; ++d) {
            const int lo = cfg.field_boundary_lo[d], hi = cfg.field_boundary_hi[d];
            const bool ok = (lo == WXA_BOUNDARY_PERIODIC || lo == WXA_BOUNDARY_PEC) &&
                            (hi == WXA_BOUNDARY_PERIODIC || hi == WXA_BOUNDARY_PEC) &&
                            ((lo == WXA_BOUNDARY_PERIODIC) == (hi == WXA_BOUNDARY_PERIODIC));
            if (!ok) throw std::runtime_error("field boundary: a direction is periodic on both sides or on neither");
            periodic[d] = lo == WXA_BOUNDARY_PERIODIC;
            m_pec_lo[d] = lo == WXA_BOUNDARY_PEC && cfg.coord[d] == 0;
            m_pec_hi[d] = hi == WXA_BOUNDARY_PEC && cfg.coord[d] == cfg.nbricks[d] - 1;
            m_any_pec = m_any_pec || lo == WXA_BOUNDARY_PEC || hi == WXA_BOUNDARY_PEC;
            m_pec_here = m_pec_here || m_pec_lo[d] || m_pec_hi[d];
            m_dom_lo[d] = 0;
            m_dom_hi[d] = cfg.n_cell[d] - 1;
        }
        m_comm->set_periodic(periodic);
        SetUpHaloOverlap(cfg.overlap_halo != 0);
        for (int d = 0; d < 3; ++d)
            for (int side = 0; side < 2; ++side) {
                int32_t want = side == 0 ? cfg.particle_boundary_lo[d] : cfg.particle_boundary_hi[d];
                const bool fper = periodic[d] != 0;
                if (want == WXA_PBOUNDARY_DEFAULT) want = fper ? WXA_PBOUNDARY_PERIODIC : WXA_PBOUNDARY_ABSORBING;
                const bool ok = (want == WXA_PBOUNDARY_PERIODIC) == fper &&
                                (want == WXA_PBOUNDARY_PERIODIC || want == WXA_PBOUNDARY_ABSORBING ||
                                 want == WXA_PBOUNDARY_REFLECTING);
                if (!ok) throw std::runtime_error("particle boundary: periodic if and only if the field boundary is");
                (side == 0 ? m_ctx.particle_bc_lo[d] : m_ctx.particle_bc_hi[d]) = want;
                m_ctx.any_particle_wall = m_ctx.any_particle_wall || want != WXA_PBOUNDARY_PERIODIC;
                m_any_reflecting_wall = m_any_reflecting_wall || want == WXA_PBOUNDARY_REFLECTING;
            }

        const amrex::IntVect Etype[3] = {{0, 1, 1}, {1, 0, 1}, {1, 1, 0}};
        const amrex::IntVect Btype[3] = {{1, 0, 0}, {0, 1, 0}, {0, 0, 1}};
        for (int d = 0; d < 3; ++d) {
            m_fields.alloc_init(FieldType::Efield_fp, Direction{d}, 0, m_ctx.brick_box, Etype[d], guard_cells.ng_alloc_EB);
            m_fields.alloc_init(FieldType::Bfield_fp, Direction{d}, 0, m_ctx.brick_box, Btype[d], guard_cells.ng_alloc_EB);
            m_fields.alloc_init(FieldType::current_fp, Direction{d}, 0, m_ctx.brick_box, Etype[d], guard_cells.ng_alloc_J);
            m_fields.alias_init(FieldType::Efield_aux, FieldType::Efield_fp, Direction{d}, 0);
            m_fields.alias_init(FieldType::Bfield_aux, FieldType::Bfield_fp, Direction{d}, 0);
        }
        if (use_filter)
            for (int d = 0; d < 3; ++d)
                m_filter_tmp[d] = std::make_unique<amrex::MultiFab>(be, m_ctx.brick_box, Etype[d], guard_cells.ng_alloc_J);
        for (int d = 0; d < 3; ++d)
            if (cfg.nbricks[d] == 1 && m_comm->periodic(d) &&
                m_ctx.brick_box.length(d) < 2 * guard_cells.ng_alloc_J[d] + 1)
                throw std::runtime_error("periodic direction shorter than twice the guard depth");
        if (cfg.use_fdtd_nci_corr) InitNCICorrector(Etype, Btype);
        {
            std::vector<amrex::MultiFab*> eb, jj;
            for (int d = 0; d < 3; ++d) {
                eb.push_back(m_fields.get(FieldType::Efield_fp, Direction{d}, 0));
                eb.push_back(m_fields.get(FieldType::Bfield_fp, Direction{d}, 0));
                jj.push_back(m_fields.get(FieldType::current_fp, Direction{d}, 0));
            }
            m_comm->presize(eb, guard_cells.ng_alloc_EB);
            m_comm->presize(jj, guard_cells.ng_alloc_J);
        }
        m_fdtd_solver_fp = std::make_unique<FiniteDifferenceSolver>(&m_ctx, cfg.maxwell_solver, m_ctx.dx);
        sort_intervals = cfg.sort_interval;
        m_ctx.sort_intervals_on = sort_intervals > 0;
        const char* fold = std::getenv("WXA_SORT_IN_PUSH");
        m_ctx.sort_in_push = sort_intervals > 0 && !(fold && std::atoi(fold) == 0);
        if (const char* e = std::getenv("WXA_SORT_BEHIND_SHIFT")) m_ctx.skip_sort_behind_a_window_shift = std::atoi(e) == 0;
        for (int d = 0; d < 3; ++d) m_ctx.sort_wrap[d] = m_comm->periodic(d) && m_comm->self_periodic(d) ? 1 : 0;
        const char* predict = std::getenv("WXA_SORT_PREDICT");
        m_ctx.sort_predict_dt = predict && std::atoi(predict) == 0 ? 0.0 : dt[0];
        const char* merged = std::getenv("WXA_SORT_MERGED");
        m_ctx.sort_merged = m_ctx.sort_in_push && !(merged && std::atoi(merged) == 0);
        m_ctx.sort_interval_steps = (int32_t)sort_intervals;
        m_ctx.step_dt = dt[0];
    }

    void InitNCICorrector(const amrex::IntVect (&Etype)[3], const amrex::IntVect (&Btype)[3]) {
        constexpr double c = 299'792'458.;
        const double cdtodz = c * dt[0] / m_ctx.dx[2];
        const bool nodal_gather = !m_ctx.galerkin_interpolation;
        nci_godfrey_filter_exeybz = std::make_unique<NCIGodfreyFilter>(godfrey_coeff_set::Ex_Ey_Bz, cdtodz, nodal_gather);
        nci_godfrey_filter_bxbyez = std::make_unique<NCIGodfreyFilter>(godfrey_coeff_set::Bx_By_Ez, cdtodz, nodal_gather);
        nci_godfrey_filter_exeybz->ComputeStencils();
        nci_godfrey_filter_bxbyez->ComputeStencils();
        for (int i = 0; i < 5; ++i) {
            m_ctx.nci_stencil_exeybz[i] = nci_godfrey_filter_exeybz->stencil_z[i];
            m_ctx.nci_stencil_bxbyez[i] = nci_godfrey_filter_bxbyez->stencil_z[i];
        }
        for (int d = 0; d < 3; ++d) {
            m_nci_E[d] = std::make_unique<amrex::MultiFab>(m_be, m_ctx.brick_box, Etype[d], guard_cells.ng_alloc_EB);
            m_nci_B[d] = std::make_unique<amrex::MultiFab>(m_be, m_ctx.brick_box, Btype[d], guard_cells.ng_alloc_EB);
            m_ctx.nci_E[d] = m_nci_E[d].get();
            m_ctx.nci_B[d] = m_nci_B[d].get();
        }
        m_ctx.use_fdtd_nci_corr = true;
    }

    void ComputeDt() {
        constexpr double c = 299'792'458.;
        const auto& dx = m_ctx.dx;
        amrex::Real deltat;
        if (m_cfg.maxwell_solver == WXA_SOLVER_CKC) {
            if (!m_be->ckc_max_dt) throw std::runtime_error("algo.maxwell_solver = ckc: not in this backend");
            deltat = m_cfg.cfl * m_be->ckc_max_dt(dx.data());
        } else {
            deltat = m_cfg.cfl * 1.0 / (std::sqrt(1.0 / (dx[0] * dx[0]) + 1.0 / (dx[1] * dx[1]) + 1.0 / (dx[2] * dx[2])) * c);
        }
        dt.assign(1, deltat);
    }

    void Evolve(int numsteps) {
        const int numsteps_max = numsteps;
        if (!m_switches_verified) {
            m_switches_verified = true;
            m_comm->VerifySwitchesAgree((safe_guard_cells ? 1 : 0) | (m_env_no_guard_layer ? 2 : 0) |
                                        (m_env_fold_rho_guard_columns ? 4 : 0) | (m_overlap ? 8 : 0));
        }
        if (!m_reduced_diags_started) {
            m_reduced_diags_started = true;
            if (diag_hook) diag_hook((int)istep - 1, kDiagFlush);
            reduced_diags.ComputeAndWrite(*this, (int)istep - 1);
        }
        for (int step = 0; step < numsteps_max; ++step) {
            if (diag_hook) diag_hook((int)istep, kDiagNewIteration);
            ExplicitFillBoundaryEBUpdateAux();
            m_ctx.sort_now = sort_intervals > 0 && (istep % sort_intervals == 0);
            m_ctx.count_now = sort_intervals > 0 && ((istep + 1) % sort_intervals == 0);
            m_ctx.steps_to_next_sort = sort_intervals > 0 ? (int32_t)(sort_intervals - istep % sort_intervals) : 0;
            OneStep_nosub(cur_time);
            if (step == numsteps_max - 1 && synchronize_at_end) Synchronize();
            ++istep;
            cur_time += dt[0];
            m_ctx.t_new = cur_time;
            if (m_btd) m_btd->ComputeAndPack(*this);
            const bool move_j = is_synchronized;
            const int num_moved = MoveWindow(istep, move_j);
            HandleParticlesAtBoundaries(step, cur_time, num_moved);
            reduced_diags.ComputeAndWrite(*this, (int)istep - 1);
            if (diag_hook) diag_hook((int)istep - 1, kDiagFlush);
        }
        m_be->stream_sync(m_ctx.stream);
        if (max_step >= 0 && istep == max_step) FlushDiagsLastTimestep();
    }
    void FlushDiagsLastTimestep() {
        if (diag_hook) diag_hook((int)istep, kDiagLastTimestep);
        if (m_btd) m_btd->FlushLast(*this);
    }
    static constexpr int kDiagNewIteration = 0, kDiagFlush = 1, kDiagLastTimestep = 2;
    std::function<void(int step, int what)> diag_hook;
    int64_t max_step = -1;

    void AddBTDiagnostics(int num_snapshots, amrex::Real dt_snapshots_lab, int buffer_size, bool write_species) {
        m_btd = std::make_unique<BTDiagnostics>(num_snapshots, dt_snapshots_lab, buffer_size);
        m_btd->Init(*this);
        m_btd_write_species = write_species;
        HookBTDSpecies();
    }
    void HookBTDSpecies() {
        if (!m_btd || !m_btd_write_species) return;
        m_ctx.btd = m_btd.get();
        for (int i = 0; i < mypc->nSpecies(); ++i) mypc->GetParticleContainer(i).btd_species_id = i;
    }
    BTDiagnostics* btd() const { return m_btd.get(); }

    MultiReducedDiags reduced_diags;
    void owned_points(const wxa_field_view& f, int32_t lo[3], int32_t hi[3]) const {
        for (int d = 0; d < 3; ++d) {
            lo[d] = f.lo[d] + f.ng[d];
            hi[d] = f.lo[d] + f.n[d] - f.ng[d];
            const bool top_wall = !m_comm->periodic(d) && m_comm->coord()[d] == m_comm->nbricks()[d] - 1;
            if (f.stag[d] && !top_wall) hi[d] -= 1;
        }
    }
    amrex::Real getdt() const { return dt[0]; }
    void sync_stream() { m_be->stream_sync(m_ctx.stream); }

    void SetMovingWindow(int dir, amrex::Real v_over_c) {
        if (dir < 0 || dir > 2 || !(v_over_c > 0.0)) throw std::runtime_error("moving window: direction 0..2, v > 0");
        if (m_comm->periodic(dir)) throw std::runtime_error("the moving window direction cannot be periodic");
        do_moving_window = true;
        moving_window_dir = dir;
        moving_window_v = v_over_c * 299'792'458.;
        moving_window_x = m_ctx.prob_lo[dir];
        const char* merged = std::getenv("WXA_SORT_MERGED");
        if (!(merged && std::atoi(merged) != 0)) m_ctx.sort_merged = false;
    }

    int MoveWindow(int , bool move_j) {
        if (!do_moving_window) return 0;
        using warpx::fields::FieldType;
        using ablastr::fields::Direction;
        for (int i = 0; i < mypc->nContainers(); ++i) {
            WarpXParticleContainer& pc = mypc->GetParticleContainer(i);
            if (std::isnan(pc.m_current_injection_position)) pc.m_current_injection_position = m_ctx.prob_hi[moving_window_dir];
        }
        const amrex::Real c = 299'792'458.;
        moving_window_x += (moving_window_v - m_ctx.beta_boost * c) / (1 - moving_window_v * m_ctx.beta_boost / c) * dt[0];
        const int dir = moving_window_dir;
        UpdateInjectionPosition(dt[0]);
        const amrex::Real cdx = m_ctx.dx[dir];
        const int num_shift_base = static_cast<int>((moving_window_x - m_ctx.prob_lo[dir]) / cdx);
        if (num_shift_base == 0) return 0;
        m_ctx.prob_lo[dir] += num_shift_base * cdx;
        m_ctx.prob_hi[dir] += num_shift_base * cdx;
        m_ctx.brick_plo[dir] = m_ctx.prob_lo[dir] + (m_ctx.brick_box.lo[dir] - m_dom_lo[dir]) * cdx;
        m_ctx.brick_phi[dir] = m_ctx.prob_lo[dir] + (m_ctx.brick_box.lo[dir] - m_dom_lo[dir] + m_ctx.brick_box.length(dir)) * cdx;
        for (int dim = 0; dim < 3; ++dim) {
            shiftMF(*m_fields.get(FieldType::Bfield_fp, Direction{dim}, 0), num_shift_base, dir);
            shiftMF(*m_fields.get(FieldType::Efield_fp, Direction{dim}, 0), num_shift_base, dir);
            if (move_j) shiftMF(*m_fields.get(FieldType::current_fp, Direction{dim}, 0), num_shift_base, dir);
        }
        for (int i = 0; i < mypc->nContainers(); ++i) {
            WarpXParticleContainer& pc = mypc->GetParticleContainer(i);
            if (!pc.doContinuousInjection()) continue;
            const amrex::Real new_injection_position =
                pc.m_current_injection_position + std::floor((m_ctx.prob_hi[dir] - pc.m_current_injection_position) / cdx) * cdx;
            double blo[3] = {m_ctx.prob_lo[0], m_ctx.prob_lo[1], m_ctx.prob_lo[2]};
            double bhi[3] = {m_ctx.prob_hi[0], m_ctx.prob_hi[1], m_ctx.prob_hi[2]};
            blo[dir] = pc.m_current_injection_position;
            bhi[dir] = new_injection_position;
            if (bhi[dir] > blo[dir] && pc.m_current_injection_position != new_injection_position) {
                pc.ContinuousInjection(blo, bhi);
                pc.m_current_injection_position = new_injection_position;
            }
        }
        if (sort_intervals > 0) {
            mypc->SortParticlesByBin(amrex::IntVect(1));
            for (int i = 0; i < mypc->nContainers(); ++i) mypc->GetParticleContainer(i).m_sorted_by_window_shift = true;
        }
        return num_shift_base;
    }

    void UpdateInjectionPosition(amrex::Real a_dt) {
        const amrex::Real c = 299'792'458.;
        const int dir = moving_window_dir;
        for (int i = 0; i < mypc->nContainers(); ++i) {
            WarpXParticleContainer& pc = mypc->GetParticleContainer(i);
            if (!pc.doContinuousInjection()) continue;
            const amrex::Real u_bulk = pc.BulkMomentum(dir);
            amrex::Real v_shift = c * u_bulk / std::sqrt(1.0 + u_bulk * u_bulk);
            if (m_ctx.gamma_boost > 1.0) {
                v_shift = (v_shift - c * m_ctx.beta_boost) / (1.0 - v_shift * m_ctx.beta_boost / c);
                v_shift *= (dir == 2) ? 1.0 : 0.0;
            }
            pc.m_current_injection_position += v_shift * a_dt;
        }
    }

    void shiftMF(amrex::MultiFab& mf, int num_shift, int dir) {
        const wxa_field_view& v = mf.view();
        if (num_shift > v.ng[dir]) throw std::runtime_error("shiftMF: shift exceeds the guard depth");
        m_shift_tmp.be = m_be;
        m_shift_tmp.reserve(sizeof(double) * (size_t)v.kstride * (size_t)v.n[2]);
        int periodic[3] = {m_comm->periodic(0) ? 1 : 0, m_comm->periodic(1) ? 1 : 0, m_comm->periodic(2) ? 1 : 0};
        if (m_comm->exchanges(dir)) {
            amrex::IntVect ng(0);
            ng[dir] = num_shift;
            m_comm->FillBoundary(mf, ng, false, m_ctx.stream);
            if (m_comm->has_neighbor(dir, 1)) periodic[dir] = WXA_WINDOW_KEEP_GUARDS;
        }
        if (m_be->shift_field_window(&v, static_cast<double*>(m_shift_tmp.p), dir, num_shift, periodic, m_ctx.stream) != 0)
            throw std::runtime_error("shift_field_window failed");
    }

    void OneStep_nosub(amrex::Real a_cur_time) {
        PushParticlesandDeposit(a_cur_time);
        SyncCurrentAndRho();
        EvolveB(0.5 * dt[0], DtType::FirstHalf);
        if (!m_grown_b) FillBoundaryB(guard_cells.ng_FieldSolver, WarpX::sync_nodal_points);
        if (m_overlap) order_streams(m_ctx.stream, 1, m_comm_stream);
        EvolveE(dt[0]);
        if (m_cfg.maxwell_solver == WXA_SOLVER_CKC || safe_guard_cells)
            FillBoundaryE(guard_cells.ng_FieldSolver, WarpX::sync_nodal_points);
        EvolveB(0.5 * dt[0], DtType::SecondHalf);
        if (safe_guard_cells) FillBoundaryB(guard_cells.ng_alloc_EB);
    }

    void SetSafeGuardCells(bool on) {
        if (istep != 0 && on != safe_guard_cells) throw std::runtime_error("warpx.safe_guard_cells: before the first step");
        safe_guard_cells = on;
        guard_cells.Init(dt[0], m_ctx.dx, m_cfg.nox, use_filter, amrex::IntVect(2), m_cfg.use_fdtd_nci_corr != 0,
                         NCIGodfreyFilter::m_stencil_width, safe_guard_cells);
        if (on && m_overlap) throw std::runtime_error("warpx.safe_guard_cells with overlap_halo: the overlapped schedule relies on the "
                                                      "guard-layer update the safe mode switches off");
        if (on) m_grown_b = false;
    }
    void SetSinglePrecisionComms(bool on) { m_comm->set_single_precision_comms(on); }
    bool do_single_precision_comms() const { return m_comm->single_precision_comms(); }

    void SetUpHaloOverlap(bool want) {
        m_grown_b = !m_any_pec && m_be->evolve_b_guard_layer != nullptr && m_cfg.maxwell_solver == WXA_SOLVER_YEE &&
                    !m_env_no_guard_layer;
        m_overlap = false;
        bool any_split = false;
        for (int d = 0; d < 3; ++d) any_split = any_split || !m_comm->self_periodic(d);
        if (want && !(m_cfg.sort_interval > 0 && m_cfg.sort_interval <= 4))
            throw std::runtime_error("overlap_halo needs 0 < warpx.sort_intervals <= 4 (interior tiles must stay clear of the guards)");
        if (!want || !m_grown_b || !any_split || !m_be->stream_create || m_cfg.use_fdtd_nci_corr) return;
        m_comm_stream = m_be->stream_create();
        if (!m_comm_stream) return;
        if (m_be->event_create)
            for (auto& e : m_halo_events) e = m_be->event_create();
        m_overlap = true;
    }
    bool halo_overlap() const { return m_overlap; }
    void order_streams(void* waiting_stream, int ev, void* recorded_stream) {
        if (!m_halo_events[ev]) return;
        m_be->event_record(m_halo_events[ev], recorded_stream);
        m_be->stream_wait_event(waiting_stream, m_halo_events[ev]);
    }

    void PushParticlesandDeposit(amrex::Real a_cur_time, bool skip_current = false,
                                 PushType push_type = PushType::Explicit) {
        if (m_eb_fill_in_flight) {
            mypc->PushInterior(m_fields, dt[0]);
            order_streams(m_ctx.stream, 3, m_comm_stream);
            m_eb_fill_in_flight = false;
        }
        mypc->Evolve(m_fields, 0, "current_fp", a_cur_time, dt[0], DtType::Full, skip_current, push_type);
    }

    void SyncCurrentAndRho() {
        PhaseTimer t(&m_ctx, kSyncCurrent);
        using warpx::fields::FieldType;
        auto J = m_fields.get_alldirs(FieldType::current_fp, 0);
        if (use_filter)
            for (int idim = 0; idim < 3; ++idim) ApplyFilterJ(J, 0, idim);
        if (m_overlap) {
            order_streams(m_comm_stream, 0, m_ctx.stream);
            SumBoundaryJ(J, 0, m_comm_stream);
            return;
        }
        SumBoundaryJ(J, 0);
        ApplyJfieldBoundary(0, J[0], J[1], J[2], PatchType::fine);
    }

    void ApplyJfieldBoundary(int , amrex::MultiFab* Jx, amrex::MultiFab* Jy, amrex::MultiFab* Jz,
                             PatchType ) {
        if (!m_pec_here) return;
        const wxa_field_view Jv[3] = {Jx->view(), Jy->view(), Jz->view()};
        if (m_be->apply_pec_j(Jv, m_dom_lo, m_dom_hi, m_pec_lo, m_pec_hi, m_ctx.stream) != 0)
            throw std::runtime_error("apply_pec_j failed");
    }

    amrex::MultiFab& ComputeRho() {
        if (!m_rho) {
            amrex::IntVect ng_rho;
            for (int d = 0; d < 3; ++d)
                ng_rho[d] = m_ctx.nox + 1 + static_cast<int>(std::ceil(299'792'458. * dt[0] / m_ctx.dx[d]));
            m_rho = std::make_unique<amrex::MultiFab>(m_be, m_ctx.brick_box, amrex::IntVect(1), ng_rho);
            if (use_filter) m_rho_tmp = std::make_unique<amrex::MultiFab>(m_be, m_ctx.brick_box, amrex::IntVect(1), ng_rho);
        }
        amrex::MultiFab& rho = *m_rho;
        rho.setVal(0.0, m_ctx.stream);
        for (int i = 0; i < mypc->nContainers(); ++i) mypc->GetParticleContainer(i).DepositCharge(&rho);
        if (m_pec_here) ApplyRhofieldBoundary(rho);
        if (use_filter) {
            check(m_be->filter_bilinear(&rho.view(), &m_rho_tmp->view(), m_ctx.stream), "filter_bilinear");
            rho.swap_storage(*m_rho_tmp);
        }
        m_comm->SumBoundary(rho, rho.nGrowVect(), false, m_ctx.stream);
        m_be->stream_sync(m_ctx.stream);
        return rho;
    }
    amrex::MultiFab* rho() { return m_rho.get(); }

    void ApplyRhofieldBoundary(amrex::MultiFab& rho) {
        const wxa_field_view& v = rho.view();
        const bool fold_columns = m_env_fold_rho_guard_columns;
        struct Slab { int32_t lo[3], hi[3]; size_t at; };
        std::vector<Slab> slabs;
        size_t total = 0;
        if (!fold_columns) {
            for (int d = 0; d < 3; ++d) {
                if (m_pec_lo[d] || m_pec_hi[d] || v.ng[d] == 0) continue;
                for (int side = 0; side < 2; ++side) {
                    if (!m_comm->domain_face(d, side)) continue;
                    Slab sl;
                    for (int e = 0; e < 3; ++e) { sl.lo[e] = v.lo[e]; sl.hi[e] = v.lo[e] + v.n[e]; }
                    if (side == 0) sl.hi[d] = v.lo[d] + v.ng[d];
                    else sl.lo[d] = v.lo[d] + v.n[d] - v.ng[d];
                    sl.at = total;
                    total += (size_t)(sl.hi[0] - sl.lo[0]) * (size_t)(sl.hi[1] - sl.lo[1]) * (size_t)(sl.hi[2] - sl.lo[2]);
                    slabs.push_back(sl);
                }
            }
        }
        if (total) {
            m_pec_rho_keep.be = m_be;
            m_pec_rho_keep.reserve(sizeof(double) * total);
            for (const Slab& sl : slabs)
                check(m_be->pack_box(&v, sl.lo, sl.hi, static_cast<double*>(m_pec_rho_keep.p) + sl.at, m_ctx.stream), "pack_box");
        }
        if (m_be->apply_pec_rho(&v, m_dom_lo, m_dom_hi, m_pec_lo, m_pec_hi, m_ctx.stream) != 0)
            throw std::runtime_error("apply_pec_rho failed");
        for (const Slab& sl : slabs)
            check(m_be->unpack_box(&v, sl.lo, sl.hi, static_cast<const double*>(m_pec_rho_keep.p) + sl.at,  0,
                                   m_ctx.stream), "unpack_box");
    }

    void ApplyFilterJ(const ablastr::fields::VectorField& current, int , int idim) {
        amrex::MultiFab& J = *current[idim];
        amrex::MultiFab& tmp = *m_filter_tmp[idim];
        check(m_be->filter_bilinear(&J.view(), &tmp.view(), m_ctx.stream), "filter_bilinear");
        J.swap_storage(tmp);
    }

    void SumBoundaryJ(const ablastr::fields::VectorField& current, int lev) { SumBoundaryJ(current, lev, m_ctx.stream); }
    void SumBoundaryJ(const ablastr::fields::VectorField& current, int , void* stream) {
        amrex::IntVect ng_depos_J = guard_cells.ng_depos_J;
        if (use_filter) ng_depos_J = ng_depos_J + amrex::IntVect(2) - amrex::IntVect(1);
        ng_depos_J = amrex::min(ng_depos_J, current[0]->nGrowVect());
        m_comm->SumBoundary({current[0], current[1], current[2]}, ng_depos_J, safe_guard_cells,
                            stream);
    }

    void DryComm(int reps, double ms[4]) {
        using warpx::fields::FieldType;
        reps = std::min(std::max(reps, 1), 64);
        auto J = m_fields.get_alldirs(FieldType::current_fp, 0);
        DeviceBuffer saved[3];
        for (int c = 0; c < 3; ++c) {
            const wxa_field_view v = J[c]->view();
            const size_t bytes = sizeof(double) * (size_t)v.kstride * (size_t)v.n[2];
            saved[c].be = m_be;
            saved[c].reserve(bytes);
            m_be->memcpy_async(saved[c].p, v.p, bytes, m_ctx.stream);
        }
        auto timed = [&](auto&& f) {
// ... 18 lines not shown
    }

    void EvolveB(amrex::Real a_dt, DtType a_dt_type) {
        {
            PhaseTimer t(&m_ctx, kEvolveB);
            m_fdtd_solver_fp->EvolveB(m_fields, 0, PatchType::fine, a_dt);
        }
        if (a_dt_type == DtType::FirstHalf && m_grown_b) {
            PhaseTimer t(&m_ctx, kFillBoundary);
            const int32_t grow[3] = {1, 1, 1};
            m_fdtd_solver_fp->EvolveBGuardLayer(m_fields, 0, a_dt, grow);
        }
        ApplyBfieldBoundary(0, PatchType::fine);
    }
    void EvolveE(amrex::Real a_dt) {
        PhaseTimer t(&m_ctx, kEvolveE);
        using warpx::fields::FieldType;
        m_fdtd_solver_fp->EvolveE(m_fields, 0, PatchType::fine, m_fields.get_alldirs(FieldType::Efield_fp, 0), a_dt);
        ApplyEfieldBoundary(0, PatchType::fine);
    }

    void ApplyEfieldBoundary(int , PatchType ) {
        if (!m_pec_here) return;
        auto E = m_fields.get_alldirs(warpx::fields::FieldType::Efield_fp, 0);
        const wxa_field_view Ev[3] = {E[0]->view(), E[1]->view(), E[2]->view()};
        const int32_t ng[3] = {guard_cells.ng_FieldGather[0], guard_cells.ng_FieldGather[1], guard_cells.ng_FieldGather[2]};
        if (m_be->apply_pec_e(Ev, m_dom_lo, m_dom_hi, m_pec_lo, m_pec_hi, ng, m_ctx.stream) != 0)
            throw std::runtime_error("apply_pec_e failed");
    }
    void ApplyBfieldBoundary(int , PatchType ) {
        if (!m_pec_here) return;
        auto B = m_fields.get_alldirs(warpx::fields::FieldType::Bfield_fp, 0);
        const wxa_field_view Bv[3] = {B[0]->view(), B[1]->view(), B[2]->view()};
        const int32_t ng[3] = {guard_cells.ng_FieldGather[0], guard_cells.ng_FieldGather[1], guard_cells.ng_FieldGather[2]};
        if (m_be->apply_pec_b(Bv, m_dom_lo, m_dom_hi, m_pec_lo, m_pec_hi, ng, m_ctx.stream) != 0)
            throw std::runtime_error("apply_pec_b failed");
    }

    void FillBoundaryE(const amrex::IntVect& ng, std::optional<bool> nodal_sync = std::nullopt) {
        FillBoundaryVector(warpx::fields::FieldType::Efield_fp, ng, nodal_sync.value_or(false));
    }
    void FillBoundaryB(const amrex::IntVect& ng, std::optional<bool> nodal_sync = std::nullopt) {
        FillBoundaryVector(warpx::fields::FieldType::Bfield_fp, ng, nodal_sync.value_or(false));
    }
    void FillBoundaryAux(const amrex::IntVect& ) {}
    void UpdateAuxilaryData() {}

    void ExplicitFillBoundaryEBUpdateAux() {
        using warpx::fields::FieldType;
        if (is_synchronized) {
            FillBoundaryEB(guard_cells.ng_alloc_EB);
            UpdateAuxilaryData();
            FillBoundaryAux(guard_cells.ng_UpdateAux);
            auto E = m_fields.get_alldirs(FieldType::Efield_aux, 0);
            auto B = m_fields.get_alldirs(FieldType::Bfield_aux, 0);
            mypc->PushP(0, -0.5 * dt[0], *E[0], *E[1], *E[2], *B[0], *B[1], *B[2]);
            is_synchronized = false;
        } else {
            if (m_overlap) {
                order_streams(m_comm_stream, 2, m_ctx.stream);
                FillBoundaryEB(guard_cells.ng_FieldGather, m_comm_stream);
                m_eb_fill_in_flight = true;
            } else {
                FillBoundaryEB(guard_cells.ng_FieldGather);
            }
            UpdateAuxilaryData();
            FillBoundaryAux(guard_cells.ng_UpdateAux);
        }
    }

    void Synchronize() {
        using warpx::fields::FieldType;
        FillBoundaryEB(guard_cells.ng_FieldGather);
        UpdateAuxilaryData();
        FillBoundaryAux(guard_cells.ng_UpdateAux);
        auto E = m_fields.get_alldirs(FieldType::Efield_aux, 0);
        auto B = m_fields.get_alldirs(FieldType::Bfield_aux, 0);
        mypc->PushP(0, 0.5 * dt[0], *E[0], *E[1], *E[2], *B[0], *B[1], *B[2]);
        is_synchronized = true;
    }

    void HandleParticlesAtBoundaries(int step, amrex::Real , int num_moved) {
        PhaseTimer t(&m_ctx, kRedistribute);
        mypc->ApplyBoundaryConditions();
        mypc->RedistributeLocal(num_moved + 1, *m_comm);
        (void)step;
    }

    ablastr::fields::MultiFabRegister& fields() { return m_fields; }
    MultiParticleContainer& GetPartContainer() { return *mypc; }
    WarpXContext& context() { return m_ctx; }
    amrex::Real getdt(int lev) const { return dt[lev]; }
    int64_t getistep() const { return istep; }
    amrex::Real gett_new() const { return cur_time; }
    BrickComm& comm() { return *m_comm; }
    bool any_reflecting_wall() const { return m_any_reflecting_wall; }

    guardCellManager guard_cells;
    bool use_filter = true;
    bool safe_guard_cells = false;
    bool is_synchronized = true;
    bool synchronize_at_end = true;
    void SynchronizeNow() {
        if (!is_synchronized) Synchronize();
        m_be->stream_sync(m_ctx.stream);
    }
    int sort_intervals = -1;
    int32_t m_pec_lo[3] = {0, 0, 0}, m_pec_hi[3] = {0, 0, 0}, m_dom_lo[3] = {0, 0, 0}, m_dom_hi[3] = {0, 0, 0};
    bool m_any_pec = false;
    bool m_pec_here = false;
    bool m_any_reflecting_wall = false;
    bool do_moving_window = false;
    int moving_window_dir = 2;
    amrex::Real moving_window_v = 0.0, moving_window_x = 0.0;
    DeviceBuffer m_shift_tmp;

private:
    void FillBoundaryVector(warpx::fields::FieldType ft, const amrex::IntVect& ng, bool nodal_sync, void* stream) {
        auto F = m_fields.get_alldirs(ft, 0);
        m_comm->FillBoundary({F[0], F[1], F[2]}, ng, nodal_sync, stream);
    }
    void FillBoundaryVector(warpx::fields::FieldType ft, const amrex::IntVect& ng, bool nodal_sync) {
        PhaseTimer t(&m_ctx, kFillBoundary);
        auto F = m_fields.get_alldirs(ft, 0);
        for (int d = 0; d < 3; ++d)
            if (!ng.allLE(F[d]->nGrowVect()))
                throw std::runtime_error("Error: in FillBoundary, requested more guard cells than allocated");
        m_comm->FillBoundary({F[0], F[1], F[2]}, ng, nodal_sync, m_ctx.stream);
    }
    void FillBoundaryEB(const amrex::IntVect& ng) {
        PhaseTimer t(&m_ctx, kFillBoundary);
        FillBoundaryEB(ng, m_ctx.stream);
    }
    void FillBoundaryEB(const amrex::IntVect& ng, void* stream) {
        using warpx::fields::FieldType;
        auto E = m_fields.get_alldirs(FieldType::Efield_fp, 0);
        auto B = m_fields.get_alldirs(FieldType::Bfield_fp, 0);
        for (int d = 0; d < 3; ++d)
            if (!ng.allLE(E[d]->nGrowVect()) || !ng.allLE(B[d]->nGrowVect()))
                throw std::runtime_error("Error: in FillBoundary, requested more guard cells than allocated");
        m_comm->FillBoundary({E[0], E[1], E[2], B[0], B[1], B[2]}, ng, false, stream);
    }

    const Backend* m_be;
    wxa_sim_config m_cfg;
    WarpXContext m_ctx;
    ablastr::fields::MultiFabRegister m_fields;
    std::unique_ptr<MultiParticleContainer> mypc;
    std::unique_ptr<FiniteDifferenceSolver> m_fdtd_solver_fp;
    std::unique_ptr<BrickComm> m_comm;
    std::unique_ptr<NCIGodfreyFilter> nci_godfrey_filter_exeybz, nci_godfrey_filter_bxbyez;
    std::unique_ptr<amrex::MultiFab> m_nci_E[3], m_nci_B[3];
    std::unique_ptr<amrex::MultiFab> m_filter_tmp[3];
    std::unique_ptr<amrex::MultiFab> m_rho, m_rho_tmp;
    DeviceBuffer m_pec_rho_keep;
    std::unique_ptr<BTDiagnostics> m_btd;
    bool m_btd_write_species = false;
    bool m_reduced_diags_started = false;
    bool m_grown_b = false, m_overlap = false;
    bool m_env_no_guard_layer = false, m_env_fold_rho_guard_columns = false, m_switches_verified = false;
    void* m_comm_stream = nullptr;
    void* m_halo_events[4] = {nullptr, nullptr, nullptr, nullptr};
    bool m_eb_fill_in_flight = false;
    std::vector<amrex::Real> dt;
    amrex::Real cur_time = 0.0;
    int64_t istep = 0;
};

}
#endif
```

### warpx_amd/csrc/host/backend.hpp

```cpp
#ifndef WXA_HOST_BACKEND_HPP_
#define WXA_HOST_BACKEND_HPP_

#include <cstddef>
#include <cstdint>

#include "../../../include/warpx_amd.h"

namespace wxa::host {

struct Backend {
    const char* name;
    int (*evolve_b)(const wxa_field_view*, const wxa_field_view*, double, const double*, void*);
    int (*evolve_e)(const wxa_field_view*, const wxa_field_view*, const wxa_field_view*, double,
                    const double*, void*);
    int (*evolve_b_guard_layer)(const wxa_field_view*, const wxa_field_view*, double, const double*, const int32_t* grow,
                                void*);
    void (*ckc_stencil_coefficients)(const double* cell_size, double* cx, double* cy, double* cz);
    double (*ckc_max_dt)(const double* cell_size);
    int (*evolve_b_ckc)(const wxa_field_view*, const wxa_field_view*, double, const double* cx, const double* cy,
                        const double* cz, void*);
    int (*ws_set_external_eb)(void* ws, const double* E, const double* B);
    int (*ws_set_repeated_plasma_lens)(void* ws, const wxa_repeated_plasma_lens*) = nullptr;
    int (*ws_set_time)(void* ws, double t) = nullptr;
    int (*ws_set_deposit_accumulator)(void* ws, int32_t acc) = nullptr;
    int (*ws_set_streaming_plasma)(void* ws, int32_t on) = nullptr;
    int (*gather_push)(const wxa_particle_view*, const wxa_field_view*, const wxa_field_view*,
                       const wxa_grid_geom*, double, double, double, int, int, int, int move, void* ws, void*);
    int (*gather_push_part)(const wxa_particle_view*, const wxa_field_view*, const wxa_field_view*,
                            const wxa_grid_geom*, double, double, double, int, int, int, void* ws, int part, void*);
    int (*deposit_current)(const wxa_particle_view*, const wxa_field_view*, const wxa_grid_geom*, double,
                           double, double, int, int, void* ws, void*);
    int (*add_plasma)(const wxa_particle_view* dst, const wxa_plasma_injector*, const double* corner, const int32_t* ncells,
                      const double* dx, const double* brick_lo, const double* brick_hi, const wxa_injected_momentum* momentum,
                      int64_t* n_added,
                      void* ws, void*);
    int (*deposit_charge)(const wxa_particle_view*, const wxa_field_view*, const wxa_grid_geom*, double, int, void*);
    int (*apply_pec_e)(const wxa_field_view*, const int32_t* dom_lo, const int32_t* dom_hi, const int32_t* pec_lo,
                       const int32_t* pec_hi, const int32_t* ng, void*);
    int (*apply_pec_b)(const wxa_field_view*, const int32_t* dom_lo, const int32_t* dom_hi, const int32_t* pec_lo,
                       const int32_t* pec_hi, const int32_t* ng, void*);
    int (*apply_pec_j)(const wxa_field_view*, const int32_t* dom_lo, const int32_t* dom_hi, const int32_t* pec_lo,
                       const int32_t* pec_hi, void*);
    int (*apply_pec_rho)(const wxa_field_view*, const int32_t* dom_lo, const int32_t* dom_hi, const int32_t* pec_lo,
                         const int32_t* pec_hi, void*);
    int (*shift_field_window)(const wxa_field_view*, double* tmp, int32_t dir, int32_t num_shift, const int* periodic,
                              void*);
    int (*laser_push)(const wxa_particle_view*, const wxa_laser_push_params*, double t, double dt, void*);
    int (*filter_bilinear)(const wxa_field_view*, const wxa_field_view*, void*);
    int (*btd_select_particles)(const wxa_particle_view*, const double* const old6[6], double z_boost, double z_boost_old,
                                double t_boost, double dt, double t_lab, double gamma_boost, double* out, int64_t capacity,
                                int64_t* n_selected, void* stream) = nullptr;
    int (*reduce_field)(const wxa_field_view*, const int32_t* lo, const int32_t* hi, double* sum_sq, double* max_abs,
                        void* stream) = nullptr;
    int (*reduce_particles)(const wxa_particle_view*, double mass, int32_t photon, double* out6, void* stream) = nullptr;
    int (*filter_stencil)(const wxa_field_view*, const wxa_field_view*, const double* s0, int32_t n0, const double* s1,
                          int32_t n1, const double* s2, int32_t n2, void*) = nullptr;
    int (*fill_boundary_periodic)(const wxa_field_view*, const int*, const int*, void*);
    int (*sync_nodal_periodic)(const wxa_field_view*, const int*, void*);
    int (*sum_boundary_periodic)(const wxa_field_view*, const int*, const int*, void*);
    int (*fill_boundary_periodic_multi)(const wxa_field_view*, int32_t, const int*, const int*, void*) = nullptr;
    int (*sum_boundary_periodic_multi)(const wxa_field_view*, int32_t, const int*, const int*, void*) = nullptr;
    int (*pack_box)(const wxa_field_view*, const int32_t*, const int32_t*, double*, void*);
    int (*unpack_box)(const wxa_field_view*, const int32_t*, const int32_t*, const double*, int, void*);
    int (*pack_box_f32)(const wxa_field_view*, const int32_t*, const int32_t*, float*, void*) = nullptr;
    int (*unpack_box_f32)(const wxa_field_view*, const int32_t*, const int32_t*, const float*, int, void*) = nullptr;
    int (*field_set_zero)(const wxa_field_view*, void*);
    int (*field_set_zero_multi)(const wxa_field_view*, int32_t, void*) = nullptr;
    int (*enforce_periodic)(const wxa_particle_view*, const double*, const double*, const int*, void*);
    int (*enforce_periodic_sorted)(const wxa_particle_view*, const double*, const double*, const int*, void* ws, int32_t,
                                   void*) = nullptr;
    int (*sort_particles_by_cell)(const wxa_particle_view*, const wxa_particle_view*, const double*,
                                  const double*, const int32_t*, const int32_t*, void* ws, void*);
    int (*partition_particles)(const wxa_particle_view*, const wxa_particle_view*, int dim, double lo,
                               double hi, int64_t* counts, void* ws, void*);
    int (*wrap_and_classify)(const wxa_particle_view*, int64_t first, int64_t count, const double* prob_lo,
                             const double* prob_hi, const int* periodic, const double* brick_lo,
                             const double* brick_hi, const int* split, int32_t* lists, int64_t capacity,
                             int64_t* counts, void* ws, void*);
    int (*wrap_and_classify_dest)(const wxa_particle_view*, int64_t first, int64_t count, const double* prob_lo,
                                  const double* prob_hi, const int* periodic, const double* brick_lo,
                                  const double* brick_hi, const int* split, int32_t* lists, int64_t capacity,
                                  int64_t* counts27, void* ws, void*);
    int (*pack_leavers)(const wxa_particle_view*, const int32_t* list, int64_t n, void* msg, int64_t row_len,
                        int64_t offset, int retire, const double* brick_lo, const double* brick_hi, void*);
    int (*sort_live_count)(void* ws, int64_t* n, void*);
    int (*push_sort_begin)(void* ws, int32_t mode, const wxa_particle_view* p, const wxa_particle_view* dst, const double* plo,
                           const double* dinv, const int32_t* cell_lo, const int32_t* ncell, const int32_t* wrap,
                           int32_t check_retired, double predict_dt, void*) = nullptr;
    int (*push_sort_end)(void* ws, int32_t read_live, int64_t* live, int64_t* appended, void*) = nullptr;
    int (*push_sort_pending)(const void* ws, const wxa_particle_view* p) = nullptr;
    int (*apply_particle_boundaries)(const wxa_particle_view*, const double* prob_lo, const double* prob_hi,
                                     const int32_t* bc_lo, const int32_t* bc_hi, int64_t* n_lost, void* ws, void*);
    int (*workspace_create)(void** ws);
    void (*workspace_destroy)(void* ws);
    void* (*dmalloc)(size_t bytes);
    void (*dfree)(void* p);
    int (*memset_async)(void* p, int value, size_t bytes, void* stream);
    int (*memcpy_async)(void* dst, const void* src, size_t bytes, void* stream);
    int (*memcpy_h2d)(void* dst, const void* src, size_t bytes);
    int (*memcpy_d2h)(void* dst, const void* src, size_t bytes);
    int (*stream_sync)(void* stream);
    void* (*stream_create)();
    void (*stream_destroy)(void* stream);
    void (*stream_wait_event)(void* stream, void* ev);
    void* (*event_create)();
    void (*event_destroy)(void* ev);
    void (*event_record)(void* ev, void* stream);
    float (*event_elapsed_ms)(void* start, void* stop);
};

}
#endif
```

### warpx_amd/csrc/host/sim_capi.hpp

```cpp
#ifndef WXA_HOST_SIM_CAPI_HPP_
#define WXA_HOST_SIM_CAPI_HPP_

#include <cstring>

#include "WarpX.hpp"

namespace wxa::host {

struct SimHandle {
    std::unique_ptr<WarpX> warpx;
    std::string error;
    int max_step = -1;
    std::vector<std::string> species_names;
    std::shared_ptr<void> multi_diags;
};

inline int sim_create(const Backend* be, const wxa_sim_config* cfg, const wxa_comm* comm, SimHandle** out,
                      std::string& err) {
    if (!cfg || !out) return WXA_ERR_INVALID_ARG;
    try {
        auto h = std::make_unique<SimHandle>();
        h->warpx = std::make_unique<WarpX>(be, *cfg, comm);
        *out = h.release();
        return WXA_OK;
// ... 136 lines not shown
    return WXA_OK;
}

inline int sim_compute_rho(SimHandle* h) {
    if (!h) return WXA_ERR_INVALID_ARG;
    try {
        h->warpx->ComputeRho();
        return WXA_OK;
    } catch (const std::exception& e) {
        h->error = e.what();
        return WXA_ERR_HIP;
    }
}

inline int sim_add_btd(SimHandle* h, int32_t num_snapshots, double dt_snapshots_lab, int32_t buffer_size,
                       int32_t write_species) {
    if (!h) return WXA_ERR_INVALID_ARG;
    try {
        h->warpx->AddBTDiagnostics(num_snapshots, dt_snapshots_lab, buffer_size, write_species != 0);
        return WXA_OK;
    } catch (const std::exception& e) {
        h->error = e.what();
        return WXA_ERR_INVALID_ARG;
    }
}

inline int sim_btd_info(SimHandle* h, int32_t i, int32_t n[3], double z_lab[2], double* t_lab, int32_t* filled,
                        int32_t* full) {
    if (!h || !h->warpx->btd() || i < 0 || i >= h->warpx->btd()->num_snapshots()) return WXA_ERR_INVALID_ARG;
    const auto& s = h->warpx->btd()->snapshot(i);
    if (n) for (int d = 0; d < 3; ++d) n[d] = s.n[d];
    if (z_lab) { z_lab[0] = s.zlo_lab; z_lab[1] = s.zhi_lab; }
    if (t_lab) *t_lab = s.t_lab;
    if (filled) *filled = s.counter;
    if (full) *full = s.full;
    return WXA_OK;
}

inline int sim_btd_data(SimHandle* h, int32_t i, int32_t comp, double* out) {
    if (!h || !out || !h->warpx->btd() || i < 0 || i >= h->warpx->btd()->num_snapshots() || comp < 0 ||
        comp >= BTDiagnostics::NCOMP)
        return WXA_ERR_INVALID_ARG;
    const auto& s = h->warpx->btd()->snapshot(i);
    const size_t n = (size_t)s.n[0] * s.n[1] * s.n[2];
    if (s.data.size() != (size_t)BTDiagnostics::NCOMP * n) return WXA_ERR_INVALID_ARG;
    std::memcpy(out, s.data.data() + (size_t)comp * n, sizeof(double) * n);
    return WXA_OK;
}

inline int sim_btd_num_particles(SimHandle* h, int32_t i, int32_t id, int64_t* n) {
    if (!h || !n || !h->warpx->btd() || i < 0 || i >= h->warpx->btd()->num_snapshots() || id < 0) return WXA_ERR_INVALID_ARG;
    const auto& s = h->warpx->btd()->snapshot(i);
    *n = id < (int32_t)s.particles.size() ? (int64_t)s.particles[(size_t)id][0].size() : 0;
    return WXA_OK;
}
inline int sim_btd_particles(SimHandle* h, int32_t i, int32_t id, double* out) {
    int64_t n = 0;
    const int rc = sim_btd_num_particles(h, i, id, &n);
    if (rc != WXA_OK || !out) return rc != WXA_OK ? rc : WXA_ERR_INVALID_ARG;
    if (n == 0) return WXA_OK;
    const auto& rows = h->warpx->btd()->snapshot(i).particles[(size_t)id];
    for (int c = 0; c < 7; ++c) std::memcpy(out + (size_t)c * (size_t)n, rows[(size_t)c].data(), sizeof(double) * (size_t)n);
    return WXA_OK;
}

inline int sim_add_reduced_diag(SimHandle* h, const char* name, const char* type, const char* intervals, const char* path) {
    if (!h || !name || !*name || !type) return WXA_ERR_INVALID_ARG;
    try {
        h->warpx->reduced_diags.Add(name, type, intervals ? intervals : "", path);
        h->warpx->reduced_diags.SetSpeciesNames(h->species_names);
        return WXA_OK;
    } catch (const std::exception& e) {
        h->error = e.what();
        return WXA_ERR_INVALID_ARG;
    }
}
inline int sim_reduced_diag_data(SimHandle* h, const char* name, int32_t compute_now, double* out, int32_t capacity,
                                 int32_t* n) {
    if (!h || !name || !n || capacity < 0 || (capacity > 0 && !out)) return WXA_ERR_INVALID_ARG;
    try {
        const std::vector<double>& d = h->warpx->reduced_diags.Data(*h->warpx, name, compute_now != 0);
        *n = (int32_t)d.size();
        for (int32_t i = 0; i < std::min(*n, capacity); ++i) out[i] = d[(size_t)i];
        return WXA_OK;
    } catch (const std::exception& e) {
        h->error = e.what();
        return WXA_ERR_INVALID_ARG;
    }
}

inline int sim_get_particles(SimHandle* h, int32_t id, wxa_particle_view* out) {
    if (!h || !out || id < 0 || id >= h->warpx->GetPartContainer().nSpecies()) return WXA_ERR_INVALID_ARG;
    *out = h->warpx->GetPartContainer().GetParticleContainer(id).tile().view();
    return WXA_OK;
}

inline int sim_dry_comm(SimHandle* h, int32_t reps, double ms[4]) {
    if (!h || !ms) return WXA_ERR_INVALID_ARG;
    try {
        h->warpx->DryComm(reps, ms);
        return WXA_OK;
    } catch (const std::exception& e) {
        h->error = e.what();
        return WXA_ERR_HIP;
    }
}

inline int sim_get_timers(SimHandle* h, double ms[8], int64_t counts[8], int reset) {
    if (!h) return WXA_ERR_INVALID_ARG;
    WarpXContext& c = h->warpx->context();
    c.resolve_timers();
    for (int i = 0; i < 8; ++i) { ms[i] = c.ms[i]; counts[i] = c.counts[i]; }
    if (reset) for (int i = 0; i < 8; ++i) { c.ms[i] = 0; c.counts[i] = 0; }
    return WXA_OK;
}

}

#define WXA_SIM_CAPI(PFX, RET, SIMTYPE, BACKEND_GETTER, SET_ERROR)                                          \
    extern "C" {                                                                                       \
    RET PFX##sim_create(const wxa_sim_config* cfg, const wxa_comm* comm, SIMTYPE** out) {              \
        std::string err;                                                                               \
        wxa::host::SimHandle* h = nullptr;                                                             \
        int rc = wxa::host::sim_create(BACKEND_GETTER(), cfg, comm, &h, err);                          \
        if (rc != 0) { SET_ERROR(err.c_str()); return (RET)rc; }                                            \
        *out = reinterpret_cast<SIMTYPE*>(h);                                                          \
        return (RET)0;                                                                                   \
    }                                                                                                  \
    void PFX##sim_destroy(SIMTYPE* s) { delete reinterpret_cast<wxa::host::SimHandle*>(s); }           \
    RET PFX##sim_add_species(SIMTYPE* s, double q, double m, const wxa_particle_view* init, int32_t* id) { \
        auto* h = reinterpret_cast<wxa::host::SimHandle*>(s);                                          \
        int rc = wxa::host::sim_add_species(h, q, m, init, id);                                        \
        if (rc != 0 && h) SET_ERROR(h->error.c_str());                                                 \
        return (RET)rc;                                                                                     \
    }                                                                                                  \
    RET PFX##sim_evolve(SIMTYPE* s, int32_t n) {                                                       \
        auto* h = reinterpret_cast<wxa::host::SimHandle*>(s);                                          \
        int rc = wxa::host::sim_evolve(h, n);                                                          \
        if (rc != 0 && h) SET_ERROR(h->error.c_str());                                                 \
        return (RET)rc;                                                                                     \
    }                                                                                                  \
    double PFX##sim_dt(const SIMTYPE* s) {                                                             \
        return reinterpret_cast<const wxa::host::SimHandle*>(s)->warpx->getdt(0);                      \
    }                                                                                                  \
    int64_t PFX##sim_istep(const SIMTYPE* s) {                                                         \
        return reinterpret_cast<const wxa::host::SimHandle*>(s)->warpx->getistep();                    \
    }                                                                                                  \
    RET PFX##sim_get_field(SIMTYPE* s, const char* name, wxa_field_view* out) {                        \
        return (RET)wxa::host::sim_get_field(reinterpret_cast<wxa::host::SimHandle*>(s), name, out);        \
    }                                                                                                  \
    int32_t PFX##sim_halo_overlap(const SIMTYPE* s) {                                                  \
        return s && reinterpret_cast<const wxa::host::SimHandle*>(s)->warpx->halo_overlap() ? 1 : 0;     \
    }                                                                                                  \
    RET PFX##sim_compute_rho(SIMTYPE* s) {                                                             \
        auto* h = reinterpret_cast<wxa::host::SimHandle*>(s);                                          \
        int rc = wxa::host::sim_compute_rho(h);                                                        \
        if (rc != 0 && h) SET_ERROR(h->error.c_str());                                                 \
        return (RET)rc;                                                                                \
    }                                                                                                  \
    RET PFX##sim_set_moving_window(SIMTYPE* s, const wxa_moving_window* mw) {                          \
        return (RET)wxa::host::sim_set_moving_window(reinterpret_cast<wxa::host::SimHandle*>(s), mw);    \
    }                                                                                                  \
    RET PFX##sim_set_injection(SIMTYPE* s, int32_t id, const wxa_plasma_injector* inj, int add_initial, \
                               int continuous) {                                                       \
        return (RET)wxa::host::sim_set_injection(reinterpret_cast<wxa::host::SimHandle*>(s), id, inj,    \
                                                 add_initial, continuous);                             \
    }                                                                                                  \
    RET PFX##sim_set_external_particle_fields(SIMTYPE* s, int32_t id, const double E[3], const double B[3]) { \
        return (RET)wxa::host::sim_set_external_particle_fields(reinterpret_cast<wxa::host::SimHandle*>(s), id, E, B); \
    }                                                                                                  \
    RET PFX##sim_set_deposit_accumulator(SIMTYPE* s, int32_t id, int32_t acc) {                        \
        return (RET)wxa::host::sim_set_deposit_accumulator(reinterpret_cast<wxa::host::SimHandle*>(s), id, acc); \
    }                                                                                                  \
    RET PFX##sim_set_radiation_reaction(SIMTYPE* s, int32_t id, int32_t on) {                          \
        return (RET)wxa::host::sim_set_radiation_reaction(reinterpret_cast<wxa::host::SimHandle*>(s), id, on); \
    }                                                                                                  \
    RET PFX##sim_add_laser(SIMTYPE* s, const wxa_laser_antenna* la) {                                  \
        return (RET)wxa::host::sim_add_laser(reinterpret_cast<wxa::host::SimHandle*>(s), la);            \
    }                                                                                                  \
    RET PFX##sim_add_btd(SIMTYPE* s, int32_t num_snapshots, double dt_snapshots_lab, int32_t buffer_size, \
                         int32_t write_species) {                                                      \
        auto* h = reinterpret_cast<wxa::host::SimHandle*>(s);                                          \
        int rc = wxa::host::sim_add_btd(h, num_snapshots, dt_snapshots_lab, buffer_size, write_species); \
        if (rc != 0 && h) SET_ERROR(h->error.c_str());                                                 \
        return (RET)rc;                                                                                \
    }                                                                                                  \
    RET PFX##sim_btd_info(SIMTYPE* s, int32_t i, int32_t n[3], double z_lab[2], double* t_lab, int32_t* filled, \
                          int32_t* full) {                                                             \
        return (RET)wxa::host::sim_btd_info(reinterpret_cast<wxa::host::SimHandle*>(s), i, n, z_lab, t_lab, filled, full); \
    }                                                                                                  \
    RET PFX##sim_btd_data(SIMTYPE* s, int32_t i, int32_t comp, double* out) {                          \
        return (RET)wxa::host::sim_btd_data(reinterpret_cast<wxa::host::SimHandle*>(s), i, comp, out); \
    }                                                                                                  \
    RET PFX##sim_btd_num_particles(SIMTYPE* s, int32_t i, int32_t id, int64_t* n) {                    \
        return (RET)wxa::host::sim_btd_num_particles(reinterpret_cast<wxa::host::SimHandle*>(s), i, id, n); \
    }                                                                                                  \
    RET PFX##sim_btd_particles(SIMTYPE* s, int32_t i, int32_t id, double* out) {                       \
        return (RET)wxa::host::sim_btd_particles(reinterpret_cast<wxa::host::SimHandle*>(s), i, id, out); \
    }                                                                                                  \
    RET PFX##sim_add_reduced_diag(SIMTYPE* s, const char* name, const char* type, const char* intervals, \
                                  const char* path) {                                                  \
        auto* h = reinterpret_cast<wxa::host::SimHandle*>(s);                                          \
        int rc = wxa::host::sim_add_reduced_diag(h, name, type, intervals, path);                      \
        if (rc != 0 && h) SET_ERROR(h->error.c_str());                                                 \
        return (RET)rc;                                                                                \
    }                                                                                                  \
    RET PFX##sim_reduced_diag_data(SIMTYPE* s, const char* name, int32_t compute_now, double* out,     \
                                   int32_t capacity, int32_t* n) {                                     \
        auto* h = reinterpret_cast<wxa::host::SimHandle*>(s);                                          \
        int rc = wxa::host::sim_reduced_diag_data(h, name, compute_now, out, capacity, n);             \
        if (rc != 0 && h) SET_ERROR(h->error.c_str());                                                 \
        return (RET)rc;                                                                                \
    }                                                                                                  \
    RET PFX##sim_get_particles(SIMTYPE* s, int32_t id, wxa_particle_view* out) {                       \
        return (RET)wxa::host::sim_get_particles(reinterpret_cast<wxa::host::SimHandle*>(s), id, out);      \
    }                                                                                                  \
    RET PFX##sim_get_timers(SIMTYPE* s, double ms[8], int64_t counts[8], int reset) {                  \
        return (RET)wxa::host::sim_get_timers(reinterpret_cast<wxa::host::SimHandle*>(s), ms, counts, reset); \
    }                                                                                                  \
    RET PFX##sim_dry_comm(SIMTYPE* s, int32_t reps, double ms[4]) {                                    \
        auto* h = reinterpret_cast<wxa::host::SimHandle*>(s);                                          \
        int rc = wxa::host::sim_dry_comm(h, reps, ms);                                                 \
        if (rc != 0 && h) SET_ERROR(h->error.c_str());                                                 \
        return (RET)rc;                                                                                \
    }                                                                                                  \
    RET PFX##sim_enable_timers(SIMTYPE* s, int enable) {                                               \
        if (!s) return (RET)-1;                                                                            \
        reinterpret_cast<wxa::host::SimHandle*>(s)->warpx->context().timers_on = enable != 0;          \
        return (RET)0;                                                                                   \
    }                                                                                                  \
    }
#endif
```

### warpx_amd/csrc/host/warpx_host.hip

```cpp
#include <hip/hip_runtime.h>

#include "../common.hpp"
#include "WarpXInputs.hpp"

namespace {

using wxa::host::Backend;

void* hip_dmalloc(size_t bytes) {
    void* p = nullptr;
    if (hipMalloc(&p, bytes ? bytes : 8) != hipSuccess) {
        wxa::set_last_error("hipMalloc of %zu bytes failed", bytes);
        return nullptr;
    }
    return p;
}
void hip_dfree(void* p) { if (p) (void)hipFree(p); }
int hip_memset_async(void* p, int v, size_t n, void* st) {
    return hipMemsetAsync(p, v, n, (hipStream_t)st) == hipSuccess ? 0 : WXA_ERR_HIP;
}
int hip_memcpy_async(void* d, const void* s, size_t n, void* st) {
    if (n == 0) return 0;
    return hipMemcpyAsync(d, s, n, hipMemcpyDeviceToDevice, (hipStream_t)st) == hipSuccess ? 0 : WXA_ERR_HIP;
}
// ... 23 lines not shown
    (void)hipEventElapsedTime(&ms, (hipEvent_t)a, (hipEvent_t)b);
    return ms;
}

int ws_create(void** ws) { return wxa_workspace_create(reinterpret_cast<wxa_workspace**>(ws)); }
void ws_destroy(void* ws) { wxa_workspace_destroy(static_cast<wxa_workspace*>(ws)); }
int k_deposit(const wxa_particle_view* p, const wxa_field_view* J, const wxa_grid_geom* g, double q, double dt,
              double rel, int order, int algo, void* ws, void* st) {
    return wxa_deposit_current(p, J, g, q, dt, rel, order, algo, static_cast<wxa_workspace*>(ws), st);
}
int k_sort(const wxa_particle_view* s, const wxa_particle_view* d, const double* plo, const double* dinv,
           const int32_t* lo, const int32_t* nc, void* ws, void* st) {
    return wxa_sort_particles_by_cell(s, d, plo, dinv, lo, nc, static_cast<wxa_workspace*>(ws), st);
}
int k_partition(const wxa_particle_view* s, const wxa_particle_view* d, int dim, double lo, double hi,
                int64_t* counts, void* ws, void* st) {
    return wxa_partition_particles(s, d, dim, lo, hi, counts, static_cast<wxa_workspace*>(ws), st);
}

const Backend* hip_backend() {
    static const Backend be = [] {
        Backend b{};
        b.name = "hip-gfx950";
        b.evolve_b = [](const wxa_field_view* E, const wxa_field_view* B, double dt, const double* di, void* st) -> int {
            return wxa_evolve_b(E, B, dt, di, st); };
        b.evolve_e = [](const wxa_field_view* E, const wxa_field_view* B, const wxa_field_view* J, double dt,
                        const double* di, void* st) -> int { return wxa_evolve_e(E, B, J, dt, di, st); };
        b.ws_set_external_eb = [](void* ws, const double* E, const double* B) -> int {
            return wxa_workspace_set_external_particle_fields(static_cast<wxa_workspace*>(ws), E, B); };
        b.ws_set_repeated_plasma_lens = [](void* ws, const wxa_repeated_plasma_lens* lens) -> int {
            return wxa_workspace_set_repeated_plasma_lens(static_cast<wxa_workspace*>(ws), lens); };
        b.ws_set_time = [](void* ws, double t) -> int { return wxa_workspace_set_time(static_cast<wxa_workspace*>(ws), t); };
        b.ws_set_deposit_accumulator = [](void* ws, int32_t acc) -> int {
            return wxa_workspace_set_deposit_accumulator(static_cast<wxa_workspace*>(ws), acc); };
        b.ws_set_streaming_plasma = [](void* ws, int32_t on) -> int {
            return wxa_workspace_set_streaming_plasma(static_cast<wxa_workspace*>(ws), on); };
        b.ckc_stencil_coefficients = wxa_ckc_stencil_coefficients;
        b.ckc_max_dt = wxa_ckc_max_dt;
        b.evolve_b_ckc = [](const wxa_field_view* E, const wxa_field_view* B, double dt, const double* cx, const double* cy,
                            const double* cz, void* st) -> int { return wxa_evolve_b_ckc(E, B, dt, cx, cy, cz, st); };
        b.gather_push = [](const wxa_particle_view* p, const wxa_field_view* E, const wxa_field_view* B,
                           const wxa_grid_geom* g, double q, double m, double dt, int o, int ga, int pu, int move,
                           void* ws, void* st) -> int {
            return wxa_gather_push_ws(p, E, B, g, q, m, dt, o, ga, pu, move, static_cast<wxa_workspace*>(ws), st); };
        b.gather_push_part = [](const wxa_particle_view* p, const wxa_field_view* E, const wxa_field_view* B,
                                const wxa_grid_geom* g, double q, double m, double dt, int o, int ga, int pu, void* ws,
                                int part, void* st) -> int {
            return wxa_gather_push_part(p, E, B, g, q, m, dt, o, ga, pu, static_cast<wxa_workspace*>(ws), part, st); };
        b.add_plasma = [](const wxa_particle_view* dst, const wxa_plasma_injector* inj, const double* corner,
                          const int32_t* nc, const double* dx, const double* blo, const double* bhi,
                          const wxa_injected_momentum* u, int64_t* n, void* ws, void* st) -> int {
            return wxa_add_plasma(dst, inj, corner, nc, dx, blo, bhi, u, n, static_cast<wxa_workspace*>(ws), st); };
        b.deposit_current = k_deposit;
        b.filter_bilinear = [](const wxa_field_view* s, const wxa_field_view* d, void* st) -> int {
            return wxa_filter_bilinear(s, d, st); };
        b.btd_select_particles = [](const wxa_particle_view* p, const double* const o[6], double zb, double zbo, double tb,
                                    double dt, double tl, double g, double* out, int64_t cap, int64_t* n, void* st) -> int {
            return wxa_btd_select_particles(p, o, zb, zbo, tb, dt, tl, g, out, cap, n, st); };
        b.reduce_field = [](const wxa_field_view* f, const int32_t* lo, const int32_t* hi, double* ss, double* mx,
                            void* st) -> int { return wxa_reduce_field(f, lo, hi, ss, mx, st); };
        b.reduce_particles = [](const wxa_particle_view* p, double m, int32_t photon, double* out, void* st) -> int {
            return wxa_reduce_particles(p, m, photon, out, st); };
        b.filter_stencil = [](const wxa_field_view* s, const wxa_field_view* d, const double* s0, int32_t n0,
                              const double* s1, int32_t n1, const double* s2, int32_t n2, void* st) -> int {
            return wxa_filter_stencil(s, d, s0, n0, s1, n1, s2, n2, st); };
        b.fill_boundary_periodic = [](const wxa_field_view* f, const int* ng, const int* per, void* st) -> int {
            return wxa_fill_boundary_periodic(f, ng, per, st); };
        b.sync_nodal_periodic = [](const wxa_field_view* f, const int* per, void* st) -> int {
            return wxa_sync_nodal_periodic(f, per, st); };
        b.sum_boundary_periodic = [](const wxa_field_view* f, const int* ng, const int* per, void* st) -> int {
            return wxa_sum_boundary_periodic(f, ng, per, st); };
        b.fill_boundary_periodic_multi = [](const wxa_field_view* f, int32_t nf, const int* ng, const int* per, void* st) -> int {
            return wxa_fill_boundary_periodic_multi(f, nf, ng, per, st); };
        b.sum_boundary_periodic_multi = [](const wxa_field_view* f, int32_t nf, const int* ng, const int* per, void* st) -> int {
            return wxa_sum_boundary_periodic_multi(f, nf, ng, per, st); };
        b.pack_box = [](const wxa_field_view* f, const int32_t* lo, const int32_t* hi, double* buf, void* st) -> int {
            return wxa_pack_box(f, lo, hi, buf, st); };
        b.unpack_box = [](const wxa_field_view* f, const int32_t* lo, const int32_t* hi, const double* buf, int mode,
                          void* st) -> int { return wxa_unpack_box(f, lo, hi, buf, mode, st); };
        b.pack_box_f32 = [](const wxa_field_view* f, const int32_t* lo, const int32_t* hi, float* buf, void* st) -> int {
            return wxa_pack_box_f32(f, lo, hi, buf, st); };
        b.unpack_box_f32 = [](const wxa_field_view* f, const int32_t* lo, const int32_t* hi, const float* buf, int mode,
                              void* st) -> int { return wxa_unpack_box_f32(f, lo, hi, buf, mode, st); };
        b.field_set_zero = [](const wxa_field_view* f, void* st) -> int { return wxa_field_set_zero(f, st); };
        b.field_set_zero_multi = [](const wxa_field_view* f, int32_t nf, void* st) -> int { return wxa_field_set_zero_multi(f, nf, st); };
        b.enforce_periodic = [](const wxa_particle_view* p, const double* lo, const double* hi, const int* per,
                                void* st) -> int { return wxa_enforce_periodic(p, lo, hi, per, st); };
        b.enforce_periodic_sorted = [](const wxa_particle_view* p, const double* lo, const double* hi, const int* per,
                                       void* ws, int32_t steps, void* st) -> int {
            return wxa_enforce_periodic_sorted(p, lo, hi, per, static_cast<wxa_workspace*>(ws), steps, st); };
        b.sort_particles_by_cell = k_sort;
        b.partition_particles = k_partition;
        b.wrap_and_classify = [](const wxa_particle_view* p, int64_t first, int64_t count, const double* plo,
                                 const double* phi, const int* per, const double* blo, const double* bhi,
                                 const int* split, int32_t* lists, int64_t cap, int64_t* counts, void* ws,
                                 void* st) -> int {
            return wxa_wrap_and_classify(p, first, count, plo, phi, per, blo, bhi, split, lists, cap, counts,
                                         static_cast<wxa_workspace*>(ws), st); };
        b.wrap_and_classify_dest = [](const wxa_particle_view* p, int64_t first, int64_t count, const double* plo,
                                      const double* phi, const int* per, const double* blo, const double* bhi,
                                      const int* split, int32_t* lists, int64_t cap, int64_t* counts, void* ws,
                                      void* st) -> int {
            return wxa_wrap_and_classify_dest(p, first, count, plo, phi, per, blo, bhi, split, lists, cap, counts,
                                              static_cast<wxa_workspace*>(ws), st); };
        b.pack_leavers = [](const wxa_particle_view* p, const int32_t* list, int64_t n, void* msg, int64_t row_len,
                            int64_t offset, int retire, const double* blo, const double* bhi, void* st) -> int {
            return wxa_pack_leavers(p, list, n, msg, row_len, offset, retire, blo, bhi, st); };
        b.apply_pec_e = [](const wxa_field_view* E, const int32_t* dlo, const int32_t* dhi, const int32_t* plo,
                           const int32_t* phi, const int32_t* ng, void* st) -> int {
            return wxa_apply_pec_e(E, dlo, dhi, plo, phi, ng, st); };
        b.apply_pec_b = [](const wxa_field_view* B, const int32_t* dlo, const int32_t* dhi, const int32_t* plo,
                           const int32_t* phi, const int32_t* ng, void* st) -> int {
            return wxa_apply_pec_b(B, dlo, dhi, plo, phi, ng, st); };
        b.apply_pec_j = [](const wxa_field_view* J, const int32_t* dlo, const int32_t* dhi, const int32_t* plo,
                           const int32_t* phi, void* st) -> int { return wxa_apply_pec_j(J, dlo, dhi, plo, phi, st); };
        b.apply_pec_rho = [](const wxa_field_view* r, const int32_t* dlo, const int32_t* dhi, const int32_t* plo,
                             const int32_t* phi, void* st) -> int { return wxa_apply_pec_rho(r, dlo, dhi, plo, phi, st); };
        b.deposit_charge = [](const wxa_particle_view* p, const wxa_field_view* r, const wxa_grid_geom* g, double q,
                              int order, void* st) -> int { return wxa_deposit_charge(p, r, g, q, order, st); };
        b.shift_field_window = [](const wxa_field_view* f, double* tmp, int32_t dir, int32_t n, const int* per,
                                  void* st) -> int { return wxa_shift_field_window(f, tmp, dir, n, per, st); };
        b.laser_push = [](const wxa_particle_view* p, const wxa_laser_push_params* par, double t, double dt,
                          void* st) -> int { return wxa_laser_push(p, par, t, dt, st); };
        b.apply_particle_boundaries = [](const wxa_particle_view* p, const double* plo, const double* phi,
                                         const int32_t* blo, const int32_t* bhi, int64_t* n_lost, void* ws,
                                         void* st) -> int {
            return wxa_apply_particle_boundaries(p, plo, phi, blo, bhi, n_lost, static_cast<wxa_workspace*>(ws), st); };
        b.sort_live_count = [](void* ws, int64_t* n, void* st) -> int {
            return wxa_sort_live_count(static_cast<wxa_workspace*>(ws), n, st); };
        b.push_sort_begin = [](void* ws, int32_t mode, const wxa_particle_view* p, const wxa_particle_view* dst,
                               const double* plo, const double* dinv, const int32_t* lo, const int32_t* nc,
                               const int32_t* wrap, int32_t check_retired, double predict_dt, void* st) -> int {
            return wxa_push_sort_begin(static_cast<wxa_workspace*>(ws), mode, p, dst, plo, dinv, lo, nc, wrap, check_retired,
                                       predict_dt, st); };
        b.push_sort_end = [](void* ws, int32_t read_live, int64_t* live, int64_t* appended, void* st) -> int {
            return wxa_push_sort_end(static_cast<wxa_workspace*>(ws), read_live, live, appended, st); };
        b.push_sort_pending = [](const void* ws, const wxa_particle_view* p) -> int {
            return wxa_push_sort_pending(static_cast<const wxa_workspace*>(ws), p); };
        b.workspace_create = ws_create;
        b.workspace_destroy = ws_destroy;
        b.dmalloc = hip_dmalloc;
        b.dfree = hip_dfree;
        b.memset_async = hip_memset_async;
        b.memcpy_async = hip_memcpy_async;
        b.memcpy_h2d = hip_memcpy_h2d;
        b.memcpy_d2h = hip_memcpy_d2h;
        b.stream_sync = hip_stream_sync;
        b.stream_create = hip_stream_create;
        b.stream_destroy = hip_stream_destroy;
        b.stream_wait_event = hip_stream_wait_event;
        b.evolve_b_guard_layer = [](const wxa_field_view* E, const wxa_field_view* B, double dt, const double* dinv,
                                    const int32_t* grow, void* st) -> int {
            return wxa_evolve_b_guard_layer(E, B, dt, dinv, grow, st); };
        b.event_create = hip_event_create;
        b.event_destroy = hip_event_destroy;
        b.event_record = hip_event_record;
        b.event_elapsed_ms = hip_event_elapsed;
        return b;
    }();
    return &be;
}

void set_err(const char* msg) { wxa::set_last_error("%s", msg); }

}

extern "C" wxa_status wxa_nci_godfrey_stencil(double cdtodz, int32_t nodal_gather, int32_t coeff_set, double stencil_z[5]) {
    if (!stencil_z || (coeff_set != WXA_NCI_EX_EY_BZ && coeff_set != WXA_NCI_BX_BY_EZ)) {
        wxa::set_last_error("wxa_nci_godfrey_stencil: bad argument");
        return WXA_ERR_INVALID_ARG;
    }
    wxa::host::NCIGodfreyFilter f(coeff_set == WXA_NCI_EX_EY_BZ ? wxa::host::godfrey_coeff_set::Ex_Ey_Bz
                                                                  : wxa::host::godfrey_coeff_set::Bx_By_Ez,
                                  cdtodz, nodal_gather != 0);
    f.ComputeStencils();
    for (int i = 0; i < 5; ++i) stencil_z[i] = f.stencil_z[i];
    return WXA_OK;
}

struct wxa_sim {};
WXA_SIM_CAPI(wxa_, wxa_status, wxa_sim, hip_backend, set_err)
WXA_INPUTS_CAPI(wxa_, wxa_status, wxa_sim, hip_backend, set_err)
```

### warpx_amd/sim.py

```python
from __future__ import annotations

import ctypes as C

import numpy as np

from . import _capi
from .containers import ParticleArrays, particles_to_numpy, view_to_numpy


class WarpXSim:
    def __init__(self, lib: _capi.CLib, n_cell, prob_lo, prob_hi, nox=1, galerkin=None,
                 particle_pusher=_capi.PUSHER_BORIS, current_deposition=_capi.DEPOSIT_ESIRKEPOV,
                 use_filter=0, cfl=1.0, sort_interval=-1, nbricks=(1, 1, 1), coord=(0, 0, 0),
                 comm: _capi.Comm | None = None, field_boundary_lo=(0, 0, 0), field_boundary_hi=(0, 0, 0),
                 particle_boundary_lo=(0, 0, 0), particle_boundary_hi=(0, 0, 0),
                 grid_type=_capi.GRID_STAGGERED, overlap_halo=0, maxwell_solver=_capi.SOLVER_YEE,
                 use_fdtd_nci_corr=0, gamma_boost=0.0):
        self.lib = lib
        self.on_device = lib.prefix == "wxa_"
        cfg = _capi.SimConfig()
        for d in range(3):
            cfg.n_cell[d] = int(n_cell[d])
            cfg.prob_lo[d] = float(prob_lo[d])
            cfg.prob_hi[d] = float(prob_hi[d])
# ... 28 lines not shown
    @classmethod
    def from_inputs(cls, lib: _capi.CLib, inputs_path, overrides=(), nbricks=None, coord=None,
                    comm: _capi.Comm | None = None, diagnostics: bool = False):
        overrides = ([] if diagnostics else ["warpx_amd.write_diagnostics=0"]) + list(overrides)
        self = cls.__new__(cls)
        self.lib = lib
        self.on_device = lib.prefix == "wxa_"
        self.cfg = None
        self._comm = comm
        self._h = C.c_void_p()
        ov = (C.c_char_p * max(len(overrides), 1))(*[o.encode() for o in overrides])
        nb = (C.c_int32 * 3)(*nbricks) if nbricks is not None else None
        co = (C.c_int32 * 3)(*coord) if coord is not None else None
        lib.sim_create_from_inputs(str(inputs_path).encode(), len(overrides), ov,
                                   C.byref(comm) if comm is not None else None, nb, co, C.byref(self._h))
        self.max_step = lib.sim_max_step(self._h)
        self.species_names = [lib.sim_species_name(self._h, i).decode() for i in range(lib.sim_num_species(self._h))]
        self.species = [None] * len(self.species_names)
        self.dx = None
        return self

    def write_plotfile(self, path: str):
        self.lib.sim_write_plotfile(self._h, str(path).encode())

    BTD_COMPONENTS = ("Ex", "Ey", "Ez", "Bx", "By", "Bz", "jx", "jy", "jz", "rho")

    def add_btd(self, num_snapshots: int, dt_snapshots_lab: float, buffer_size: int = 256, write_species: bool = True):
        self.lib.sim_add_btd(self._h, int(num_snapshots), float(dt_snapshots_lab), int(buffer_size), 1 if write_species else 0)

    def btd_particles(self, i: int, sid: int) -> np.ndarray:
        n = C.c_int64()
        self.lib.sim_btd_num_particles(self._h, int(i), int(sid), C.byref(n))
        out = np.zeros((7, n.value), dtype=np.float64)
        if n.value:
            self.lib.sim_btd_particles(self._h, int(i), int(sid), out.ctypes.data_as(C.POINTER(C.c_double)))
        return out

    def btd_info(self, i: int) -> dict:
        n = (C.c_int32 * 3)()
        z = (C.c_double * 2)()
        t = C.c_double()
        filled, full = C.c_int32(), C.c_int32()
        self.lib.sim_btd_info(self._h, int(i), n, z, C.byref(t), C.byref(filled), C.byref(full))
        return {"n": tuple(n), "z_lab": tuple(z), "t_lab": t.value, "slices": filled.value, "full": bool(full.value)}

    def btd_set_flush(self, file_prefix: str, file_min_digits: int = 6):
        self.lib.sim_btd_set_flush(self._h, str(file_prefix).encode(), int(file_min_digits))

    def btd_flush(self):
        self.lib.sim_btd_flush(self._h)

    def btd_box(self, i: int):
        lo, hi = (C.c_int32 * 3)(), (C.c_int32 * 3)()
        self.lib.sim_btd_box(self._h, int(i), lo, hi)
        return tuple(lo), tuple(hi)

    def btd_snapshot(self, i: int, name: str) -> np.ndarray:
        n = self.btd_info(i)["n"]
        out = np.zeros(n[0] * n[1] * n[2], dtype=np.float64)
        self.lib.sim_btd_data(self._h, int(i), self.BTD_COMPONENTS.index(name), out.ctypes.data_as(C.POINTER(C.c_double)))
        return np.ascontiguousarray(out.reshape(n[2], n[1], n[0]).transpose(2, 1, 0))

    def btd_write_plotfile(self, i: int, path: str):
        self.lib.sim_btd_write_plotfile(self._h, int(i), str(path).encode())

    def add_full_diag(self, name: str, intervals: str, file_prefix: str | None = None, file_min_digits: int = 6,
                      fields=None, write_species: bool = True, dump_last_timestep: bool = True):
        self.lib.sim_add_full_diag(self._h, name.encode(), str(intervals).encode(),
                                   None if file_prefix is None else str(file_prefix).encode(), int(file_min_digits),
                                   None if fields is None else " ".join(fields).encode(), 1 if write_species else 0,
                                   1 if dump_last_timestep else 0)

    def flush_diags_last_timestep(self):
        self.lib.sim_flush_diags_last_timestep(self._h)

    def add_reduced_diag(self, name: str, rd_type: str, intervals: str = "1", path: str | None = None):
        self.lib.sim_add_reduced_diag(self._h, name.encode(), rd_type.encode(), str(intervals).encode(),
                                      None if path is None else str(path).encode())

    def reduced_diag(self, name: str, compute_now: bool = False) -> np.ndarray:
        n = C.c_int32()
        self.lib.sim_reduced_diag_data(self._h, name.encode(), 1 if compute_now else 0, None, 0, C.byref(n))
        out = np.zeros(n.value, dtype=np.float64)
        if n.value:
            self.lib.sim_reduced_diag_data(self._h, name.encode(), 0, out.ctypes.data_as(C.POINTER(C.c_double)),
                                           n.value, C.byref(n))
        return out

    def checksum(self) -> dict:
        import json
        cap = 4096
        while True:
            buf = C.create_string_buffer(cap)
            n = self.lib.sim_checksum_json(self._h, buf, cap)
            if n < 0:
                raise _capi.WxaError("sim_checksum_json failed")
            if n < cap:
                return json.loads(buf.value.decode())
            cap = n + 256

    def close(self):
        if self._h:
            self.lib.sim_destroy(self._h)
            self._h = C.c_void_p()

    def __del__(self):
        try:
            self.close()
        except Exception:
            pass

    def add_species(self, charge, mass, particles):
        if not isinstance(particles, ParticleArrays):
            particles = ParticleArrays.from_numpy(particles, self.lib.memory)
        sid = C.c_int32(-1)
        v = particles.view
        if str(self.lib.memory).startswith("cuda"):
            import torch
            torch.cuda.synchronize()
        self.lib.sim_add_species(self._h, float(charge), float(mass), C.byref(v), C.byref(sid))
        self.species.append((float(charge), float(mass)))
        return sid.value

    def set_external_particle_fields(self, sid: int, E, B):
        self.lib.sim_set_external_particle_fields(self._h, int(sid), (C.c_double * 3)(*map(float, E)),
                                                  (C.c_double * 3)(*map(float, B)))

    def set_deposit_accumulator(self, sid: int, acc: int):
        self.lib.sim_set_deposit_accumulator(self._h, int(sid), int(acc))

    def set_radiation_reaction(self, sid: int, on=True):
        self.lib.sim_set_radiation_reaction(self._h, int(sid), 1 if on else 0)

    def set_synchronize_at_end(self, on: bool):
        self.lib.sim_set_synchronize_at_end(self._h, 1 if on else 0)

    def synchronize(self):
        self.lib.sim_synchronize(self._h)

    def set_safe_guard_cells(self, on: bool = True):
        self.lib.sim_set_safe_guard_cells(self._h, 1 if on else 0)

    def set_single_precision_comms(self, on: bool = True):
        self.lib.sim_set_single_precision_comms(self._h, 1 if on else 0)

    def evolve(self, numsteps: int):
        self.lib.sim_evolve(self._h, int(numsteps))

    @property
    def halo_overlap(self) -> bool:
        return bool(self.lib.sim_halo_overlap(self._h))

    @property
    def dt(self) -> float:
        return self.lib.sim_dt(self._h)

    @property
    def istep(self) -> int:
        return self.lib.sim_istep(self._h)

    def _d2h(self):
        return self.lib.copy_to_host if self.on_device else None

    def compute_rho(self):
        self.lib.sim_compute_rho(self._h)

    def field_view(self, name: str) -> _capi.FieldView:
        v = _capi.FieldView()
        self.lib.sim_get_field(self._h, name.encode(), C.byref(v))
        return v

    def field(self, name: str) -> np.ndarray:
        return view_to_numpy(self.field_view(name), self._d2h())

    def set_field(self, name: str, values: np.ndarray):
        v = self.field_view(name)
        n = tuple(v.n)
        assert values.shape == n, (values.shape, n)
        buf = np.zeros((n[2], n[1], int(v.jstride)), dtype=np.float64)
        buf[:, :, : n[0]] = np.transpose(values, (2, 1, 0))
        buf = np.ascontiguousarray(buf).reshape(-1)[: int(v.kstride) * n[2]]
        if self.on_device:
            self.lib.copy_to_device(v.p, buf.ctypes.data, 8 * buf.size)
        else:
            C.memmove(v.p, buf.ctypes.data, 8 * buf.size)

    def field_valid(self, name: str) -> np.ndarray:
        v = self.field_view(name)
        a = view_to_numpy(v, self._d2h())
        g = v.ng
        return a[g[0]: v.n[0] - g[0], g[1]: v.n[1] - g[1], g[2]: v.n[2] - g[2]]

    def particle_view(self, sid: int) -> _capi.ParticleView:
        v = _capi.ParticleView()
        self.lib.sim_get_particles(self._h, int(sid), C.byref(v))
        return v

    def particles(self, sid: int) -> np.ndarray:
        return particles_to_numpy(self.particle_view(sid), self._d2h())

    def enable_timers(self, on=True):
        self.lib.sim_enable_timers(self._h, 1 if on else 0)

    def dry_comm(self, reps=10):
        ms = (C.c_double * 4)()
        self.lib.sim_dry_comm(self._h, int(reps), ms)
        return {"FillBoundaryEB": ms[0], "SumBoundaryJ": ms[1], "Redistribute": ms[2], "all_three": ms[3]}

    def timers(self, reset=False):
        ms = (C.c_double * 8)()
        cnt = (C.c_int64 * 8)()
        self.lib.sim_get_timers(self._h, ms, cnt, 1 if reset else 0)
        names = ["GatherAndPush", "CurrentDeposition", "SyncCurrent", "EvolveB", "EvolveE",
                 "FillBoundary", "Redistribute", "other"]
        return {n: (ms[i], cnt[i]) for i, n in enumerate(names)}



def field_energy(sim: WarpXSim):
    from .plasma import EP0, MU0
    dV = sim.dx[0] * sim.dx[1] * sim.dx[2]

    def sumsq(name):
        v = sim.field_view(name)
        a = view_to_numpy(v, sim._d2h())
        g = v.ng
        sl = tuple(slice(g[d], v.n[d] - g[d] - v.stag[d]) for d in range(3))
        x = a[sl].astype(np.longdouble)
        return float(np.sum(x * x))

    Es = sumsq("Ex") + sumsq("Ey") + sumsq("Ez")
    Bs = sumsq("Bx") + sumsq("By") + sumsq("Bz")
    return 0.5 * Es * EP0 * dV, 0.5 * Bs / MU0 * dV


def particle_moments(sim: WarpXSim, sid: int):
    from .plasma import C_LIGHT
    q, m = sim.species[sid]
    p = sim.particles(sid).astype(np.longdouble)
    w, ux, uy, uz = p[3], p[4], p[5], p[6]
    u2 = ux * ux + uy * uy + uz * uz
    gamma = np.sqrt(1.0 + u2 / (np.longdouble(C_LIGHT) ** 2))
    ekin = float(np.sum(w * (m * u2 / (1.0 + gamma))))
    mom = [float(np.sum(w * m * c)) for c in (ux, uy, uz)]
    absmom = [float(np.sum(np.abs(m * c))) for c in (ux, uy, uz)]
    abspos = [float(np.sum(np.abs(p[i]))) for i in range(3)]
    return {"ekin": ekin, "momentum": mom, "abs_momentum": absmom, "abs_position": abspos,
            "weight": float(np.sum(w))}
```

Before: 10.77 billion particle-steps/s.

## Fuse second-half and next first-half B updates into one pass with a half-step buffer

Adds a kernel that reads E and B once and writes both the end-of-step B (second half) and the next step's half-advanced B into a separate buffer. The next step then evolves only the guard layer into that buffer and runs EvolveE from it, which removes one full-grid B sweep per step. The cost is an extra B-sized allocation and more state carried across steps, plus first/last-step special cases. It is enabled by default only when the Yee solver, grown B, no safe guard cells, no moving window and no overlap all hold.

```diff
diff --git a/include/warpx_amd.h b/include/warpx_amd.h
--- a/include/warpx_amd.h
+++ b/include/warpx_amd.h
@@ -79,6 +79,12 @@
 
 wxa_status wxa_evolve_b_guard_layer(const wxa_field_view E[3], const wxa_field_view B[3], double dt,
                                     const double inv_dx[3], const int32_t grow[3], void* stream);
+wxa_status wxa_evolve_b_guard_layer_to(const wxa_field_view E[3], const wxa_field_view B[3], const wxa_field_view Bout[3],
+                                       double dt, const double inv_dx[3], const int32_t grow[3], void* stream);
+
+wxa_status wxa_evolve_b_two_halves(const wxa_field_view E[3], const wxa_field_view Bin[3],
+                                   const wxa_field_view Bout_first[3], const wxa_field_view* Bout_second,
+                                   double dt_half, const double inv_dx[3], void* stream);
 
 void wxa_ckc_stencil_coefficients(const double cell_size[3], double coefs_x[5], double coefs_y[5], double coefs_z[5]);
 double wxa_ckc_max_dt(const double cell_size[3]);
@@ -377,6 +383,7 @@
                             const double* values, double* out);
 
 int32_t wxa_sim_halo_overlap(const wxa_sim* s);
+int32_t wxa_sim_fused_b(const wxa_sim* s);
 
 wxa_status wxa_sim_compute_rho(wxa_sim* s);
 double     wxa_sim_dt(const wxa_sim* s);
diff --git a/warpx_amd/_capi.py b/warpx_amd/_capi.py
--- a/warpx_amd/_capi.py
+++ b/warpx_amd/_capi.py
@@ -190,6 +190,7 @@
     "sim_create_from_inputs": (C.c_int, [C.c_char_p, C.c_int32, C.POINTER(C.c_char_p), C.POINTER(Comm),
                                         C.POINTER(C.c_int32), C.POINTER(C.c_int32), C.POINTER(C.c_void_p)]),
     "sim_max_step": (C.c_int32, [C.c_void_p]),
+    "sim_fused_b": (C.c_int32, [C.c_void_p]),
     "sim_num_species": (C.c_int32, [C.c_void_p]),
     "sim_species_name": (C.c_char_p, [C.c_void_p, C.c_int32]),
     "sim_checksum_json": (C.c_int64, [C.c_void_p, C.c_char_p, C.c_int64]),
@@ -279,6 +280,8 @@
     "workspace_set_deposit_accumulator": (C.c_int, [C.c_void_p, C.c_int32]),
     "workspace_set_streaming_plasma": (C.c_int, [C.c_void_p, C.c_int32]),
     "sim_set_deposit_accumulator": (C.c_int, [C.c_void_p, C.c_int32, C.c_int32]),
+    "evolve_b_two_halves": (C.c_int, [_FV3, _FV3, _FV3, _PFV, C.c_double, _D3, C.c_void_p]),
+    "evolve_b_guard_layer_to": (C.c_int, [_FV3, _FV3, _FV3, C.c_double, _D3, _I32_3, C.c_void_p]),
 }
 ACC_FP64, ACC_FP32 = 0, 1
 PUSH_SORT_COUNT, PUSH_SORT_SCATTER = 1, 2
@@ -319,7 +322,8 @@
     pass
 
 
-_RETURNS_A_VALUE = {"sim_max_step", "sim_num_species", "num_threads", "set_num_threads", "sim_halo_overlap", "push_sort_pending"}
+_RETURNS_A_VALUE = {"sim_max_step", "sim_num_species", "num_threads", "set_num_threads", "sim_halo_overlap", "push_sort_pending",
+                    "sim_fused_b"}
 
 
 class CLib:
diff --git a/warpx_amd/csrc/fields.hip b/warpx_amd/csrc/fields.hip
--- a/warpx_amd/csrc/fields.hip
+++ b/warpx_amd/csrc/fields.hip
@@ -119,6 +119,82 @@
             st_once<NT>(bz, ld_once<NT>(bz) + (dt * (idy * (ex_j1 - ex_k)) - dt * (idx * (ey_i1 - ey_k))));
         ex_k = ex_k1; ey_k = ey_k1;
         ex += Ex.ks; ey += Ey.ks; ez += Ez.ks; bx += Bx.ks; by += By.ks; bz += Bz.ks;
+    }
+}
+
+struct BOut {
+    double* x;
+    double* y;
+    double* z;
+};
+template <class CFG, bool SECOND>
+__global__ void __launch_bounds__(CFG::TI* CFG::TJ)
+evolve_b_two_halves_kernel(DevF Ex, DevF Ey, DevF Ez, DevF Bx, DevF By, DevF Bz, BOut O1, BOut O2, Box3 ub, Box3 bbx, Box3 bby,
+                           Box3 bbz, TileGrid tg, double dt, double idx, double idy, double idz) {
+    constexpr int KC = CFG::KC, NT = CFG::NT;
+    const long tile = xcd_tile_id(blockIdx.x, tg.ntiles);
+    if (tile >= tg.ntiles) return;
+    const int ti = (int)(tile % tg.nti);
+    const int tj = (int)((tile / tg.nti) % tg.ntj);
+    const int tk = (int)(tile / ((long)tg.nti * tg.ntj));
+    const int i = ub.lo[0] + ti * CFG::TI + (int)threadIdx.x;
+    const int j = ub.lo[1] + tj * CFG::TJ + (int)threadIdx.y;
+    if (i >= ub.hi[0] || j >= ub.hi[1]) return;
+    const int k0 = ub.lo[2] + tk * KC;
+    const int k1 = min(k0 + KC, ub.hi[2]);
+    const bool px = in_ij(bbx, i, j), py = in_ij(bby, i, j), pz = in_ij(bbz, i, j);
+
+    const double* __restrict__ ex = Ex.p + Ex.off(i, j, k0);
+    const double* __restrict__ ey = Ey.p + Ey.off(i, j, k0);
+    const double* __restrict__ ez = Ez.p + Ez.off(i, j, k0);
+    const long ox = Bx.off(i, j, k0), oy = By.off(i, j, k0), oz = Bz.off(i, j, k0);
+
+    double exv[KC + 1], eyv[KC + 1], ezc[KC], ezj[KC], ezi[KC], exj[KC], eyi[KC], b0[KC], b1[KC], b2[KC];
+    bool d0[KC], d1[KC], d2[KC];
+    exv[0] = ld_shared<NT>(ex); eyv[0] = ld_shared<NT>(ey);
+#pragma unroll
+    for (int n = 0; n < KC; ++n) {
+        const int k = k0 + n;
+        const bool in = k < k1;
+        d0[n] = in && px && k >= bbx.lo[2] && k < bbx.hi[2];
+        d1[n] = in && py && k >= bby.lo[2] && k < bby.hi[2];
+        d2[n] = in && pz && k >= bbz.lo[2] && k < bbz.hi[2];
+        exv[n + 1] = eyv[n + 1] = ezc[n] = ezj[n] = ezi[n] = exj[n] = eyi[n] = b0[n] = b1[n] = b2[n] = 0.0;
+        if (in) {
+            exv[n + 1] = ld_shared<NT>(ex + (n + 1) * Ex.ks); eyv[n + 1] = ld_shared<NT>(ey + (n + 1) * Ey.ks);
+            ezc[n] = ld_shared<NT>(ez + n * Ez.ks); ezj[n] = ld_shared<NT>(ez + n * Ez.ks + Ez.js);
+            ezi[n] = ld_shared<NT>(ez + n * Ez.ks + 1);
+            exj[n] = ld_shared<NT>(ex + n * Ex.ks + Ex.js); eyi[n] = ld_shared<NT>(ey + n * Ey.ks + 1);
+        }
+        if (d0[n]) b0[n] = ld_once<NT>(Bx.p + ox + n * Bx.ks);
+        if (d1[n]) b1[n] = ld_once<NT>(By.p + oy + n * By.ks);
+        if (d2[n]) b2[n] = ld_once<NT>(Bz.p + oz + n * Bz.ks);
+    }
+    asm volatile("" : "+v"(exv[0]), "+v"(eyv[0]));
+#pragma unroll
+    for (int n = 0; n < KC; ++n)
+        asm volatile("" : "+v"(exv[n + 1]), "+v"(eyv[n + 1]), "+v"(ezc[n]), "+v"(ezj[n]), "+v"(ezi[n]), "+v"(exj[n]),
+                          "+v"(eyi[n]), "+v"(b0[n]), "+v"(b1[n]), "+v"(b2[n]));
+#pragma unroll
+    for (int n = 0; n < KC; ++n) {
+        if (d0[n]) {
+            const double t = dt * (idz * (eyv[n + 1] - eyv[n])) - dt * (idy * (ezj[n] - ezc[n]));
+            const double h = b0[n] + t;
+            st_once<NT>(O1.x + ox + n * Bx.ks, h);
+            if constexpr (SECOND) st_once<NT>(O2.x + ox + n * Bx.ks, h + t);
+        }
+        if (d1[n]) {
+            const double t = dt * (idx * (ezi[n] - ezc[n])) - dt * (idz * (exv[n + 1] - exv[n]));
+            const double h = b1[n] + t;
+            st_once<NT>(O1.y + oy + n * By.ks, h);
+            if constexpr (SECOND) st_once<NT>(O2.y + oy + n * By.ks, h + t);
+        }
+        if (d2[n]) {
+            const double t = dt * (idy * (exj[n] - exv[n])) - dt * (idx * (eyi[n] - eyv[n]));
+            const double h = b2[n] + t;
+            st_once<NT>(O1.z + oz + n * Bz.ks, h);
+            if constexpr (SECOND) st_once<NT>(O2.z + oz + n * Bz.ks, h + t);
+        }
     }
 }
 
@@ -215,8 +291,8 @@
     long first[13];
 };
 __global__ void __launch_bounds__(256)
-evolve_b_faces_kernel(DevF Ex, DevF Ey, DevF Ez, DevF Bx, DevF By, DevF Bz, FaceBoxes fb, double dt, double idx, double idy,
-                      double idz) {
+evolve_b_faces_kernel(DevF Ex, DevF Ey, DevF Ez, DevF Bx, DevF By, DevF Bz, BOut O, FaceBoxes fb, double dt, double idx,
+                      double idy, double idz) {
     long t = (long)blockIdx.x * 256 + threadIdx.x;
     if (t >= fb.first[fb.n]) return;
     int f = 0;
@@ -229,18 +305,18 @@
     if (c == 0) {
         const double* ey = Ey.p + Ey.off(i, j, k);
         const double* ez = Ez.p + Ez.off(i, j, k);
-        double* bx = Bx.p + Bx.off(i, j, k);
-        *bx = *bx + (dt * (idz * (ey[Ey.ks] - ey[0])) - dt * (idy * (ez[Ez.js] - ez[0])));
+        const long o = Bx.off(i, j, k);
+        O.x[o] = Bx.p[o] + (dt * (idz * (ey[Ey.ks] - ey[0])) - dt * (idy * (ez[Ez.js] - ez[0])));
     } else if (c == 1) {
         const double* ex = Ex.p + Ex.off(i, j, k);
         const double* ez = Ez.p + Ez.off(i, j, k);
-        double* by = By.p + By.off(i, j, k);
-        *by = *by + (dt * (idx * (ez[1] - ez[0])) - dt * (idz * (ex[Ex.ks] - ex[0])));
+        const long o = By.off(i, j, k);
+        O.y[o] = By.p[o] + (dt * (idx * (ez[1] - ez[0])) - dt * (idz * (ex[Ex.ks] - ex[0])));
     } else {
         const double* ex = Ex.p + Ex.off(i, j, k);
         const double* ey = Ey.p + Ey.off(i, j, k);
-        double* bz = Bz.p + Bz.off(i, j, k);
-        *bz = *bz + (dt * (idy * (ex[Ex.js] - ex[0])) - dt * (idx * (ey[1] - ey[0])));
+        const long o = Bz.off(i, j, k);
+        O.z[o] = Bz.p[o] + (dt * (idy * (ex[Ex.js] - ex[0])) - dt * (idx * (ey[1] - ey[0])));
     }
 }
 
@@ -816,10 +892,61 @@
     return WXA_OK;
 }
 
+static bool same_layout(const wxa_field_view& a, const wxa_field_view& b) {
+    for (int d = 0; d < 3; ++d)
+        if (a.lo[d] != b.lo[d] || a.n[d] != b.n[d] || a.ng[d] != b.ng[d] || a.stag[d] != b.stag[d]) return false;
+    return a.jstride == b.jstride && a.kstride == b.kstride;
+}
+
+wxa_status wxa_evolve_b_two_halves(const wxa_field_view E[3], const wxa_field_view Bin[3], const wxa_field_view Bout_first[3],
+                                   const wxa_field_view* Bout_second, double dt_half, const double dinv[3], void* stream) {
+    WXA_REQUIRE(E && Bin && Bout_first && dinv, "null argument");
+    for (int c = 0; c < 3; ++c) {
+        WXA_REQUIRE(view_ok(E[c]) && view_ok(Bin[c]) && view_ok(Bout_first[c]), "bad field view");
+        WXA_REQUIRE(same_layout(Bin[c], Bout_first[c]), "Bout_first must have Bin's layout");
+        if (Bout_second) {
+            WXA_REQUIRE(view_ok(Bout_second[c]) && same_layout(Bin[c], Bout_second[c]), "Bout_second must have Bin's layout");
+            WXA_REQUIRE(Bout_second[c].p != Bout_first[c].p, "the two outputs must be distinct arrays");
+        }
+    }
+    if (!yee_E(E) || !yee_B(Bin)) {
+        set_last_error("wxa_evolve_b_two_halves: only the Yee staggering is supported");
+        return WXA_ERR_UNSUPPORTED;
+    }
+    for (int c = 0; c < 3; ++c)
+        for (int d = 0; d < 3; ++d) WXA_REQUIRE(E[c].ng[d] >= 1, "EvolveB needs >= 1 guard point on E");
+    const Box3 bx = valid_box(Bin[0]), by = valid_box(Bin[1]), bz = valid_box(Bin[2]);
+    Box3 ub;
+    for (int d = 0; d < 3; ++d) {
+        ub.lo[d] = std::min(bx.lo[d], std::min(by.lo[d], bz.lo[d]));
+        ub.hi[d] = std::max(bx.hi[d], std::max(by.hi[d], bz.hi[d]));
+    }
+    using CFG = StProduction;
+    const TileGrid tg = make_tiles_cfg<CFG>(ub);
+    const BOut o1 = {Bout_first[0].p, Bout_first[1].p, Bout_first[2].p};
+    const BOut o2 = Bout_second ? BOut{Bout_second[0].p, Bout_second[1].p, Bout_second[2].p} : BOut{nullptr, nullptr, nullptr};
+    if (tg.ntiles > 0) {
+        auto kernel = Bout_second ? evolve_b_two_halves_kernel<CFG, true> : evolve_b_two_halves_kernel<CFG, false>;
+        hipLaunchKernelGGL(kernel, dim3((unsigned)xcd_grid_size(tg.ntiles)), dim3(CFG::TI, CFG::TJ), 0, (hipStream_t)stream,
+                           make_devf(E[0]), make_devf(E[1]), make_devf(E[2]), make_devf(Bin[0]), make_devf(Bin[1]),
+                           make_devf(Bin[2]), o1, o2, ub, bx, by, bz, tg, dt_half, dinv[0], dinv[1], dinv[2]);
+    }
+    WXA_LAUNCH_CHECK();
+    return WXA_OK;
+}
+
 wxa_status wxa_evolve_b_guard_layer(const wxa_field_view E[3], const wxa_field_view B[3], double dt,
                                     const double dinv[3], const int32_t grow[3], void* stream) {
-    WXA_REQUIRE(E && B && dinv && grow, "null argument");
-    for (int c = 0; c < 3; ++c) WXA_REQUIRE(view_ok(E[c]) && view_ok(B[c]), "bad field view");
+    return wxa_evolve_b_guard_layer_to(E, B, B, dt, dinv, grow, stream);
+}
+
+wxa_status wxa_evolve_b_guard_layer_to(const wxa_field_view E[3], const wxa_field_view B[3], const wxa_field_view Bout[3],
+                                       double dt, const double dinv[3], const int32_t grow[3], void* stream) {
+    WXA_REQUIRE(E && B && Bout && dinv && grow, "null argument");
+    for (int c = 0; c < 3; ++c) {
+        WXA_REQUIRE(view_ok(E[c]) && view_ok(B[c]) && view_ok(Bout[c]), "bad field view");
+        WXA_REQUIRE(same_layout(B[c], Bout[c]), "Bout must have B's layout");
+    }
     if (!yee_E(E) || !yee_B(B)) {
         set_last_error("wxa_evolve_b_guard_layer: only the Yee staggering is supported");
         return WXA_ERR_UNSUPPORTED;
@@ -848,7 +975,7 @@
     if (fb.n > 0 && fb.first[fb.n] > 0)
         hipLaunchKernelGGL(evolve_b_faces_kernel, dim3((unsigned)((fb.first[fb.n] + 255) / 256)), dim3(256), 0, (hipStream_t)stream,
                            make_devf(E[0]), make_devf(E[1]), make_devf(E[2]), make_devf(B[0]), make_devf(B[1]), make_devf(B[2]),
-                           fb, dt, dinv[0], dinv[1], dinv[2]);
+                           BOut{Bout[0].p, Bout[1].p, Bout[2].p}, fb, dt, dinv[0], dinv[1], dinv[2]);
     WXA_LAUNCH_CHECK();
     return WXA_OK;
 }
diff --git a/warpx_amd/csrc/host/WarpX.hpp b/warpx_amd/csrc/host/WarpX.hpp
--- a/warpx_amd/csrc/host/WarpX.hpp
+++ b/warpx_amd/csrc/host/WarpX.hpp
@@ -76,10 +76,13 @@
             check(m_ctx->be->evolve_b(Ev, Bv, dt, m_stencil_coefs.data(), m_ctx->stream), "evolve_b");
     }
     void EvolveE(ablastr::fields::MultiFabRegister& fields, int lev, PatchType patch_type,
-                 const ablastr::fields::VectorField& Efield, amrex::Real dt) {
+                 const ablastr::fields::VectorField& Efield, amrex::Real dt,
+                 const std::unique_ptr<amrex::MultiFab>* Bsrc = nullptr) {
         using warpx::fields::FieldType;
         if (patch_type != PatchType::fine) throw std::runtime_error("single level: fine patch only");
         auto B = fields.get_alldirs(FieldType::Bfield_fp, lev);
+        if (Bsrc)
+            for (int d = 0; d < 3; ++d) B[d] = Bsrc[d].get();
         auto J = fields.get_alldirs(FieldType::current_fp, lev);
         const wxa_field_view Ev[3] = {Efield[0]->view(), Efield[1]->view(), Efield[2]->view()};
         const wxa_field_view Bv[3] = {B[0]->view(), B[1]->view(), B[2]->view()};
@@ -93,6 +96,32 @@
         const wxa_field_view Ev[3] = {E[0]->view(), E[1]->view(), E[2]->view()};
         const wxa_field_view Bv[3] = {B[0]->view(), B[1]->view(), B[2]->view()};
         check(m_ctx->be->evolve_b_guard_layer(Ev, Bv, dt, m_stencil_coefs.data(), grow, m_ctx->stream), "evolve_b_guard_layer");
+    }
+    void EvolveBGuardLayerTo(ablastr::fields::MultiFabRegister& fields, int lev, const std::unique_ptr<amrex::MultiFab>* Bout,
+                             amrex::Real dt, const int32_t grow[3]) {
+        using warpx::fields::FieldType;
+        auto E = fields.get_alldirs(FieldType::Efield_fp, lev);
+        auto B = fields.get_alldirs(FieldType::Bfield_fp, lev);
+        const wxa_field_view Ev[3] = {E[0]->view(), E[1]->view(), E[2]->view()};
+        const wxa_field_view Bv[3] = {B[0]->view(), B[1]->view(), B[2]->view()};
+        const wxa_field_view Ov[3] = {Bout[0]->view(), Bout[1]->view(), Bout[2]->view()};
+        check(m_ctx->be->evolve_b_guard_layer_to(Ev, Bv, Ov, dt, m_stencil_coefs.data(), grow, m_ctx->stream),
+              "evolve_b_guard_layer_to");
+    }
+    void EvolveBTwoHalves(ablastr::fields::MultiFabRegister& fields, int lev, const std::unique_ptr<amrex::MultiFab>* Bin,
+                          const std::unique_ptr<amrex::MultiFab>* Bsecond, amrex::Real dt_half) {
+        using warpx::fields::FieldType;
+        auto E = fields.get_alldirs(FieldType::Efield_fp, lev);
+        auto B = fields.get_alldirs(FieldType::Bfield_fp, lev);
+        const wxa_field_view Ev[3] = {E[0]->view(), E[1]->view(), E[2]->view()};
+        const wxa_field_view Bv[3] = {B[0]->view(), B[1]->view(), B[2]->view()};
+        wxa_field_view Iv[3], Sv[3];
+        for (int d = 0; d < 3; ++d) {
+            Iv[d] = Bin ? Bin[d]->view() : Bv[d];
+            if (Bsecond) Sv[d] = Bsecond[d]->view();
+        }
+        check(m_ctx->be->evolve_b_two_halves(Ev, Iv, Bv, Bsecond ? Sv : nullptr, dt_half, m_stencil_coefs.data(), m_ctx->stream),
+              "evolve_b_two_halves");
     }
 
 private:
@@ -112,6 +141,7 @@
         using ablastr::fields::Direction;
         if (cfg.nox < 1 || cfg.nox > 4) throw std::runtime_error("algo.particle_shape must be 1..4");
         m_env_no_guard_layer = std::getenv("WXA_NO_GUARD_LAYER") != nullptr;
+        if (const char* e = std::getenv("WXA_NO_FUSED_B")) m_env_no_fused_b = std::atoi(e) != 0;
         if (const char* e = std::getenv("WXA_PEC_RHO_FOLD_GUARD_COLUMNS")) m_env_fold_rho_guard_columns = std::atoi(e) != 0;
         m_ctx.be = be;
         m_ctx.nox = cfg.nox;
@@ -263,8 +293,10 @@
         if (!m_switches_verified) {
             m_switches_verified = true;
             m_comm->VerifySwitchesAgree((safe_guard_cells ? 1 : 0) | (m_env_no_guard_layer ? 2 : 0) |
-                                        (m_env_fold_rho_guard_columns ? 4 : 0) | (m_overlap ? 8 : 0));
-        }
+                                        (m_env_fold_rho_guard_columns ? 4 : 0) | (m_overlap ? 8 : 0) |
+                                        (m_env_no_fused_b ? 16 : 0));
+        }
+        SetUpFusedB();
         if (!m_reduced_diags_started) {
             m_reduced_diags_started = true;
             if (diag_hook) diag_hook((int)istep - 1, kDiagFlush);
@@ -276,7 +308,7 @@
             m_ctx.sort_now = sort_intervals > 0 && (istep % sort_intervals == 0);
             m_ctx.count_now = sort_intervals > 0 && ((istep + 1) % sort_intervals == 0);
             m_ctx.steps_to_next_sort = sort_intervals > 0 ? (int32_t)(sort_intervals - istep % sort_intervals) : 0;
-            OneStep_nosub(cur_time);
+            OneStep_nosub(cur_time, step == 0, step == numsteps_max - 1);
             if (step == numsteps_max - 1 && synchronize_at_end) Synchronize();
             ++istep;
             cur_time += dt[0];
@@ -412,9 +444,13 @@
             throw std::runtime_error("shift_field_window failed");
     }
 
-    void OneStep_nosub(amrex::Real a_cur_time) {
+    void OneStep_nosub(amrex::Real a_cur_time, bool first, bool last) {
         PushParticlesandDeposit(a_cur_time);
         SyncCurrentAndRho();
+        if (m_fused_b) {
+            OneStep_FusedB(first, last);
+            return;
+        }
         EvolveB(0.5 * dt[0], DtType::FirstHalf);
         if (!m_grown_b) FillBoundaryB(guard_cells.ng_FieldSolver, WarpX::sync_nodal_points);
         if (m_overlap) order_streams(m_ctx.stream, 1, m_comm_stream);
@@ -424,6 +460,38 @@
         EvolveB(0.5 * dt[0], DtType::SecondHalf);
         if (safe_guard_cells) FillBoundaryB(guard_cells.ng_alloc_EB);
     }
+
+    void OneStep_FusedB(bool first, bool last) {
+        const amrex::Real dt_half = 0.5 * dt[0];
+        if (first) {
+            EvolveB(dt_half, DtType::FirstHalf);
+        } else {
+            PhaseTimer t(&m_ctx, kFillBoundary);
+            const int32_t grow[3] = {1, 1, 1};
+            m_fdtd_solver_fp->EvolveBGuardLayerTo(m_fields, 0, m_Bhalf, dt_half, grow);
+        }
+        {
+            PhaseTimer t(&m_ctx, kEvolveE);
+            m_fdtd_solver_fp->EvolveE(m_fields, 0, PatchType::fine, m_fields.get_alldirs(warpx::fields::FieldType::Efield_fp, 0),
+                                      dt[0], first ? nullptr : m_Bhalf);
+        }
+        PhaseTimer t(&m_ctx, kEvolveB);
+        m_fdtd_solver_fp->EvolveBTwoHalves(m_fields, 0, first ? nullptr : m_Bhalf, last ? nullptr : m_Bhalf, dt_half);
+    }
+    void SetUpFusedB() {
+        m_fused_b = !m_env_no_fused_b && m_cfg.maxwell_solver == WXA_SOLVER_YEE && m_grown_b && !safe_guard_cells &&
+                    !do_moving_window && !m_cfg.use_fdtd_nci_corr && !m_overlap && m_be->evolve_b_two_halves != nullptr &&
+                    m_be->evolve_b_guard_layer_to != nullptr;
+        if (!m_fused_b || m_Bhalf[0]) return;
+        using warpx::fields::FieldType;
+        using ablastr::fields::Direction;
+        for (int d = 0; d < 3; ++d) {
+            const amrex::MultiFab& B = *m_fields.get(FieldType::Bfield_fp, Direction{d}, 0);
+            m_Bhalf[d] = std::make_unique<amrex::MultiFab>(m_be, m_ctx.brick_box, B.ixType(), B.nGrowVect());
+            m_Bhalf[d]->setVal(0.0, m_ctx.stream);
+        }
+    }
+    bool fused_b() const { return m_fused_b; }
 
     void SetSafeGuardCells(bool on) {
         if (istep != 0 && on != safe_guard_cells) throw std::runtime_error("warpx.safe_guard_cells: before the first step");
@@ -748,6 +816,7 @@
     std::unique_ptr<NCIGodfreyFilter> nci_godfrey_filter_exeybz, nci_godfrey_filter_bxbyez;
     std::unique_ptr<amrex::MultiFab> m_nci_E[3], m_nci_B[3];
     std::unique_ptr<amrex::MultiFab> m_filter_tmp[3];
+    std::unique_ptr<amrex::MultiFab> m_Bhalf[3];
     std::unique_ptr<amrex::MultiFab> m_rho, m_rho_tmp;
     DeviceBuffer m_pec_rho_keep;
     std::unique_ptr<BTDiagnostics> m_btd;
@@ -755,6 +824,7 @@
     bool m_reduced_diags_started = false;
     bool m_grown_b = false, m_overlap = false;
     bool m_env_no_guard_layer = false, m_env_fold_rho_guard_columns = false, m_switches_verified = false;
+    bool m_env_no_fused_b = false, m_fused_b = false;
     void* m_comm_stream = nullptr;
     void* m_halo_events[4] = {nullptr, nullptr, nullptr, nullptr};
     bool m_eb_fill_in_flight = false;
diff --git a/warpx_amd/csrc/host/backend.hpp b/warpx_amd/csrc/host/backend.hpp
--- a/warpx_amd/csrc/host/backend.hpp
+++ b/warpx_amd/csrc/host/backend.hpp
@@ -15,6 +15,10 @@
                     const double*, void*);
     int (*evolve_b_guard_layer)(const wxa_field_view*, const wxa_field_view*, double, const double*, const int32_t* grow,
                                 void*);
+    int (*evolve_b_two_halves)(const wxa_field_view* E, const wxa_field_view* Bin, const wxa_field_view* Bout_first,
+                               const wxa_field_view* Bout_second, double dt_half, const double*, void*) = nullptr;
+    int (*evolve_b_guard_layer_to)(const wxa_field_view* E, const wxa_field_view* B, const wxa_field_view* Bout, double,
+                                   const double*, const int32_t* grow, void*) = nullptr;
     void (*ckc_stencil_coefficients)(const double* cell_size, double* cx, double* cy, double* cz);
     double (*ckc_max_dt)(const double* cell_size);
     int (*evolve_b_ckc)(const wxa_field_view*, const wxa_field_view*, double, const double* cx, const double* cy,
diff --git a/warpx_amd/csrc/host/sim_capi.hpp b/warpx_amd/csrc/host/sim_capi.hpp
--- a/warpx_amd/csrc/host/sim_capi.hpp
+++ b/warpx_amd/csrc/host/sim_capi.hpp
@@ -312,6 +312,9 @@
     int32_t PFX##sim_halo_overlap(const SIMTYPE* s) {                                                  \
         return s && reinterpret_cast<const wxa::host::SimHandle*>(s)->warpx->halo_overlap() ? 1 : 0;     \
     }                                                                                                  \
+    int32_t PFX##sim_fused_b(const SIMTYPE* s) {                                                       \
+        return s && reinterpret_cast<const wxa::host::SimHandle*>(s)->warpx->fused_b() ? 1 : 0;          \
+    }                                                                                                  \
     RET PFX##sim_compute_rho(SIMTYPE* s) {                                                             \
         auto* h = reinterpret_cast<wxa::host::SimHandle*>(s);                                          \
         int rc = wxa::host::sim_compute_rho(h);                                                        \
diff --git a/warpx_amd/csrc/host/warpx_host.hip b/warpx_amd/csrc/host/warpx_host.hip
--- a/warpx_amd/csrc/host/warpx_host.hip
+++ b/warpx_amd/csrc/host/warpx_host.hip
@@ -199,6 +199,12 @@
         b.evolve_b_guard_layer = [](const wxa_field_view* E, const wxa_field_view* B, double dt, const double* dinv,
                                     const int32_t* grow, void* st) -> int {
             return wxa_evolve_b_guard_layer(E, B, dt, dinv, grow, st); };
+        b.evolve_b_two_halves = [](const wxa_field_view* E, const wxa_field_view* Bin, const wxa_field_view* B1,
+                                   const wxa_field_view* B2, double dt_half, const double* dinv, void* st) -> int {
+            return wxa_evolve_b_two_halves(E, Bin, B1, B2, dt_half, dinv, st); };
+        b.evolve_b_guard_layer_to = [](const wxa_field_view* E, const wxa_field_view* B, const wxa_field_view* Bout, double dt,
+                                       const double* dinv, const int32_t* grow, void* st) -> int {
+            return wxa_evolve_b_guard_layer_to(E, B, Bout, dt, dinv, grow, st); };
         b.event_create = hip_event_create;
         b.event_destroy = hip_event_destroy;
         b.event_record = hip_event_record;
diff --git a/warpx_amd/sim.py b/warpx_amd/sim.py
--- a/warpx_amd/sim.py
+++ b/warpx_amd/sim.py
@@ -204,6 +204,10 @@
         return bool(self.lib.sim_halo_overlap(self._h))
 
     @property
+    def fused_b(self) -> bool:
+        return bool(self.lib.sim_fused_b(self._h))
+
+    @property
     def dt(self) -> float:
         return self.lib.sim_dt(self._h)
 
```

Result: faster. 10.98 billion particle-steps/s (median of 6 runs) (+1.9%).
